# rimelabs/lambda-labs_distributed-training-guide

Hardware: AMD Instinct MI355X
Metric: tokens/sec/GPU (causal-LM pretrain) at 1/2/4/8 MI355X; FSDP peak-mem (higher is better)
Workload: dtype bf16; 1 GPU; model=meta-llama/Meta-Llama-3-8B, global_batch=16, seq_len=1024, parallelism=dp1-single

## Files before the change

csrc/kernels/flash_attn.hip:

```cpp
#include "flash_attn_plan.h"
#include "rope_common.h"

#include <ATen/hip/HIPGeneratorImpl.h>
#include <ATen/hip/PhiloxUtils.cuh>
#include <ATen/core/DistributionsHelper.h>

#include <climits>
#include <cstdlib>
#include <type_traits>

#include <cmath>

namespace dtg {

namespace fa {

typedef __attribute__((address_space(3))) i16x4 lds_i16x4;

constexpr float kLog2e = 1.4426950408889634f;
constexpr float kLn2 = 0.6931471805599453f;
constexpr float kRescaleThreshold = 8.f;

template <int W>
__device__ __forceinline__ int off(int row, int ch) {
  constexpr int NCH = W / 8;
  static_assert(NCH == 8 || NCH == 16, "head_dim 64 or 128");
  int sw;
  if constexpr (NCH == 16) sw = ((row & 3) << 2) | ((row >> 2) & 3);
  else sw = ((row & 1) << 2) | ((row >> 1) & 3);
  return row * (W * 2) + 16 * (ch ^ sw);
}

__device__ __forceinline__ i16x4 tr_read(const char* p) {
  return __builtin_amdgcn_ds_read_tr16_b64_v4i16((lds_i16x4*)(p));
}

__device__ __forceinline__ bf16x8 tr_frag_at(const char* pa, const char* pb) {
  const i16x4 a = tr_read(pa);
  const i16x4 b = tr_read(pb);
  typedef short i16x8 __attribute__((ext_vector_type(8)));
  const i16x8 ab = __builtin_shufflevector(a, b, 0, 1, 2, 3, 4, 5, 6, 7);
  return __builtin_bit_cast(bf16x8, ab);
}

template <int W>
__device__ __forceinline__ void tr_offsets(int d, int& oa, int& ob) {
  const int lane = threadIdx.x & 63;
  const int i = lane & 15, g = lane >> 4;
  const int q = i >> 2, p = i & 3;
  const int ch = ((32 * d + 16 * (g & 1)) >> 3) + (p >> 1);
  const int half = 8 * (p & 1);
  const int row = 4 * (g >> 1) + q;
  oa = off<W>(row, ch) + half;
  ob = off<W>(row + 8, ch) + half;
}

__device__ __forceinline__ f32x16 mfma(bf16x8 a, bf16x8 b, f32x16 c) {
  return __builtin_amdgcn_mfma_f32_32x32x16_bf16(a, b, c, 0, 0, 0);
}

__device__ __forceinline__ bf16x8 lds_frag(const char* p) { return *reinterpret_cast<const bf16x8*>(p); }

__device__ __forceinline__ bf16x8 pack8(const f32x16& x, int s) {
  bf16x8 r;
#pragma unroll
  for (int j = 0; j < 8; ++j) r[j] = static_cast<__bf16>(x[8 * s + j]);
  return r;
}

__device__ __forceinline__ float fexp2(float x) { return __builtin_amdgcn_exp2f(x); }

__device__ __forceinline__ float pair_max(float x) {
  const auto r = __builtin_amdgcn_permlane32_swap(__float_as_uint(x), __float_as_uint(x), false, false);
  return fmaxf(__uint_as_float(r[0]), __uint_as_float(r[1]));
}
__device__ __forceinline__ float pair_sum(float x) {
  const auto r = __builtin_amdgcn_permlane32_swap(__float_as_uint(x), __float_as_uint(x), false, false);
  return __uint_as_float(r[0]) + __uint_as_float(r[1]);
}

constexpr int kSchedMfma = 0x008, kSchedDsRead = 0x100;
template <int N, int RPM, int AHEAD>
__device__ __forceinline__ void pipeline_reads() {
  __builtin_amdgcn_sched_group_barrier(kSchedDsRead, AHEAD * RPM, 0);
#pragma unroll
  for (int i = 0; i < N - AHEAD; ++i) {
    __builtin_amdgcn_sched_group_barrier(kSchedMfma, 1, 0);
    __builtin_amdgcn_sched_group_barrier(kSchedDsRead, RPM, 0);
  }
  __builtin_amdgcn_sched_group_barrier(kSchedMfma, AHEAD, 0);
}

__device__ __forceinline__ void prio_hi() { __builtin_amdgcn_s_setprio(1); }
__device__ __forceinline__ void prio_lo() { __builtin_amdgcn_s_setprio(0); }

__device__ __forceinline__ int acc_row(int reg, int h) { return (reg & 3) + 8 * (reg >> 2) + 4 * h; }
constexpr int acc_row0(int reg) { return (reg & 3) + 8 * (reg >> 2); }

struct DropCfg {
  uint32_t k0, k1, off;
  int thr;
  float scale;
  const uint32_t* rng;
};

__device__ __forceinline__ DropCfg resolve_drop(const DropCfg& in) {
  DropCfg d = in;
  if (d.rng != nullptr) {
    d.k0 = d.rng[0];
    d.k1 = d.rng[1] ^ d.rng[3];
    d.off = d.rng[2];
  }
  return d;
}

__device__ __forceinline__ void philox4x32_10(uint32_t (&c)[4], uint32_t k0, uint32_t k1) {
#pragma unroll
  for (int r = 0; r < 10; ++r) {
    if (r) {
      k0 += 0x9E3779B9u;
      k1 += 0xBB67AE85u;
    }
    const uint32_t lo0 = 0xD2511F53u * c[0], hi0 = __umulhi(0xD2511F53u, c[0]);
    const uint32_t lo1 = 0xCD9E8D57u * c[2], hi1 = __umulhi(0xCD9E8D57u, c[2]);
    const uint32_t n0 = hi1 ^ c[1] ^ k0, n2 = hi0 ^ c[3] ^ k1;
    c[0] = n0;
    c[1] = lo1;
    c[2] = n2;
    c[3] = lo0;
  }
}

__device__ __forceinline__ void drop_row_half(const DropCfg& dc, int s0, int q, int head, int key0, int h,
                                              f32x16& x) {
#pragma unroll
  for (int g = 0; g < 4; ++g) {
    uint32_t c[4] = {(uint32_t)(key0 + 8 * g + 4 * h), (uint32_t)(s0 + (q & ~3)), (uint32_t)head, dc.off};
    philox4x32_10(c, dc.k0, dc.k1);
    const int ws = q & 3;
    const uint32_t wd = ws == 0 ? c[0] : ws == 1 ? c[1] : ws == 2 ? c[2] : c[3];
#pragma unroll
    for (int e = 0; e < 4; ++e) x[4 * g + e] = (int)((wd >> (8 * e)) & 255u) < dc.thr ? x[4 * g + e] : 0.f;
  }
}

__device__ __forceinline__ __amdgpu_buffer_rsrc_t make_rsrc(const void* p, int bytes) {
  const uint64_t a = reinterpret_cast<uint64_t>(p);
  const uint32_t lo = __builtin_amdgcn_readfirstlane(static_cast<uint32_t>(a));
  const uint32_t hi = __builtin_amdgcn_readfirstlane(static_cast<uint32_t>(a >> 32));
  const int n = __builtin_amdgcn_readfirstlane(bytes);
  return __builtin_amdgcn_make_buffer_rsrc(reinterpret_cast<void*>((static_cast<uint64_t>(hi) << 32) | lo),
                                           (short)0, n, 0x00020000);
}

template <int R, int W, int NT>
struct Stager {
  static constexpr int NCH = W / 8;
  static constexpr int PER = (R * NCH) / NT;
  static constexpr int RSTEP = NT / NCH;
  static_assert((R * NCH) % NT == 0 && NT % NCH == 0 && RSTEP % 16 == 0, "tile split");
  u16x8 regs[PER];
  __device__ __forceinline__ void load(const uint16_t* base, int64_t stride, int nvalid) {
    const int row0 = threadIdx.x / NCH, ch = threadIdx.x % NCH;
    const int bytes = nvalid > 0 ? static_cast<int>((nvalid - 1) * stride * 2 + W * 2) : 0;
    const __amdgpu_buffer_rsrc_t rs = make_rsrc(base, bytes);
    const int s2 = static_cast<int>(stride) * 2;
#pragma unroll
    for (int i = 0; i < PER; ++i) {
      const int voff = (row0 + i * RSTEP) * s2 + ch * 16;
      regs[i] = __builtin_bit_cast(u16x8, __builtin_amdgcn_raw_buffer_load_b128(rs, voff, 0, 0));
    }
  }
  __device__ __forceinline__ void store(char* tile) const {
    const int o = off<W>(threadIdx.x / NCH, threadIdx.x % NCH);
#pragma unroll
    for (int i = 0; i < PER; ++i) *reinterpret_cast<u16x8*>(tile + o + i * RSTEP * W * 2) = regs[i];
  }
};

template <int NC>
__device__ __forceinline__ void load_row_frags(const uint16_t* row, bool ok, int h, bf16x8* out) {
#pragma unroll
  for (int c = 0; c < NC; ++c) {
    const u16x8 z{0, 0, 0, 0, 0, 0, 0, 0};
    const u16x8 v = ok ? *reinterpret_cast<const u16x8*>(row + 16 * c + 8 * h) : z;
    out[c] = __builtin_bit_cast(bf16x8, v);
  }
}

__device__ __forceinline__ int grid_head(int x, int hq, int hkv) {
  const int group = hq / hkv;
  return (x % hkv) * group + x / hkv;
}

template <int ND>
__device__ __forceinline__ void store_rows_wide(const f32x16* acc, float scale, uint16_t* row, bool ok) {
  const int h = (threadIdx.x & 63) >> 5;
#pragma unroll
  for (int d = 0; d < ND; ++d) {
#pragma unroll
    for (int j = 0; j < 2; ++j) {
      uint32_t w[4];
#pragma unroll
      for (int u = 0; u < 2; ++u) {
        const int base = 4 * (2 * j + u);
        w[2 * u + 0] = (uint32_t)f2bf(acc[d][base + 0] * scale) | ((uint32_t)f2bf(acc[d][base + 1] * scale) << 16);
        w[2 * u + 1] = (uint32_t)f2bf(acc[d][base + 2] * scale) | ((uint32_t)f2bf(acc[d][base + 3] * scale) << 16);
      }
#pragma unroll
      for (int x = 0; x < 2; ++x) {
        const auto r = __builtin_amdgcn_permlane32_swap(w[x], w[2 + x], false, false);
        w[x] = r[0];
        w[2 + x] = r[1];
      }
      if (ok) *reinterpret_cast<uint4*>(row + 32 * d + 16 * j + 8 * h) = make_uint4(w[0], w[1], w[2], w[3]);
    }
  }
}

struct KeyRange {
  int start, len, off;
};
__device__ __forceinline__ KeyRange key_range(const int* kstart, const int* klen, int seq, int s0, int seqlen) {
  if (kstart == nullptr) return KeyRange{s0, seqlen, 0};
  const int n = klen[seq];
  return KeyRange{kstart[seq], n, n - seqlen};
}

struct FwdParams {
  const uint16_t *q, *k, *v;
  int64_t sq, sk, sv;
  uint16_t* o;
  float* lse;
  const int* cu;
  int64_t T;
  int hq, hkv;
  float c2;
  long long* stamps;
  const int *kstart, *klen;
  int window;
  DropCfg drop;
};

__device__ __forceinline__ void fa_stamp(long long* st, int slot, int k) {
  if (st != nullptr && threadIdx.x == 0) {
    st[slot * 6 + k] = (long long)__builtin_amdgcn_s_memrealtime();
    if (k == 0) {
      st[slot * 6 + 4] = (long long)__builtin_amdgcn_s_getreg(4 | (31 << 11));
      st[slot * 6 + 5] = (long long)__builtin_amdgcn_s_getreg(20 | (31 << 11));
    }
  }
}

template <int D, bool CAUSAL, bool WIN = false, bool DROP = false>
__global__ __launch_bounds__(256, 2) void fwd_kernel(FwdParams P) {
  [[maybe_unused]] const DropCfg dcfg = DROP ? resolve_drop(P.drop) : P.drop;
  constexpr int RB = 2 * D;
  constexpr int TILE = kFwdBK * RB;
  constexpr int NC = D / 16;
  constexpr int ND = D / 32;
  extern __shared__ __attribute__((aligned(16))) char smem[];

  fa_stamp(P.stamps, blockIdx.x + gridDim.x * (blockIdx.y + gridDim.y * blockIdx.z), 0);
  const int seq = blockIdx.y, head = grid_head(blockIdx.x, P.hq, P.hkv);
  const int s0 = P.cu[seq];
  const int seqlen = P.cu[seq + 1] - s0;
  const int qb = CAUSAL ? (gridDim.z - 1 - blockIdx.z) : blockIdx.z;
  const int q0 = qb * kFwdBQ;
  if (q0 >= seqlen) return;
  const KeyRange kr = key_range(P.kstart, P.klen, seq, s0, seqlen);
  const int klen = kr.len, koff_c = kr.off;
  const int kvh = head / (P.hq / P.hkv);
  const int lane = threadIdx.x & 63, w = __builtin_amdgcn_readfirstlane(threadIdx.x >> 6);
  const int r = lane & 31, h = lane >> 5;
  const int qrow = q0 + 32 * w + r;

  bf16x8 qf[NC];
  Stager<kFwdBQ, D, 256> sq;
  sq.load(P.q + (int64_t)(s0 + q0) * P.sq + (int64_t)head * D, P.sq, seqlen - q0);
  int koff[NC], toa[ND], tob[ND];
#pragma unroll
  for (int c = 0; c < NC; ++c) koff[c] = off<D>(r, 2 * c + h);
#pragma unroll
  for (int d = 0; d < ND; ++d) tr_offsets<D>(d, toa[d], tob[d]);

  const int kv_end = CAUSAL ? min(klen, q0 + kFwdBQ + koff_c) : klen;
  const int ntiles = (kv_end + kFwdBK - 1) / kFwdBK;
  const int win = (CAUSAL && WIN) ? P.window : 0;
  const int t_begin = win > 0 ? max(0, q0 + koff_c - win + 1) / kFwdBK : 0;
  const uint16_t* kbase = P.k + (int64_t)kr.start * P.sk + (int64_t)kvh * D;
  const uint16_t* vbase = P.v + (int64_t)kr.start * P.sv + (int64_t)kvh * D;

  f32x16 acc[ND];
#pragma unroll
  for (int i = 0; i < ND; ++i) acc[i] = f32x16{};
  float m = -INFINITY, l = 0.f;

  Stager<kFwdBK, D, 256> sk, sv;
  sk.load(kbase + (int64_t)t_begin * kFwdBK * P.sk, P.sk, klen - t_begin * kFwdBK);
  sv.load(vbase + (int64_t)t_begin * kFwdBK * P.sv, P.sv, klen - t_begin * kFwdBK);
  sq.store(smem + 2 * TILE);
  sk.store(smem);
  sv.store(smem + TILE);
  __syncthreads();
#pragma unroll
  for (int c = 0; c < NC; ++c) qf[c] = lds_frag(smem + 2 * TILE + 32 * w * RB + koff[c]);
  __syncthreads();
  fa_stamp(P.stamps, blockIdx.x + gridDim.x * (blockIdx.y + gridDim.y * blockIdx.z), 1);

  const int wave_q0 = q0 + 32 * w, wave_qmax = wave_q0 + 31;
  auto tile_step = [&](int t, auto buf) {
    constexpr int B = decltype(buf)::value;
    const int kt0 = t * kFwdBK;
    const bool more = t + 1 < ntiles;
    if (more) {
      const int nk = kt0 + kFwdBK;
      sk.load(kbase + (int64_t)nk * P.sk, P.sk, klen - nk);
      sv.load(vbase + (int64_t)nk * P.sv, P.sv, klen - nk);
    }
    const char* K = smem + B * 2 * TILE;
    const char* V = K + TILE;
    if ((!CAUSAL || kt0 <= wave_qmax + koff_c) && (win == 0 || kt0 + kFwdBK - 1 >= wave_q0 + koff_c - win + 1)) {
      f32x16 s[2];
      __builtin_amdgcn_sched_barrier(0);
      prio_hi();
#pragma unroll
      for (int kt = 0; kt < 2; ++kt) {
        bf16x8 kf[NC];
#pragma unroll
        for (int c = 0; c < NC; ++c) kf[c] = lds_frag(K + kt * 32 * RB + koff[c]);
        s[kt] = f32x16{};
#pragma unroll
        for (int c = 0; c < NC; ++c) s[kt] = mfma(kf[c], qf[c], s[kt]);
      }
      pipeline_reads<2 * NC, 1, 4>();
      __builtin_amdgcn_sched_barrier(0);
      prio_lo();
      if ((CAUSAL && kt0 + kFwdBK - 1 > wave_q0 + koff_c) || kt0 + kFwdBK > klen ||
          (win > 0 && kt0 < wave_qmax + koff_c - win + 1)) {
#pragma unroll
        for (int kt = 0; kt < 2; ++kt) {
          const int lim = (CAUSAL ? min(qrow + koff_c, klen - 1) : klen - 1) - (kt0 + 32 * kt + 4 * h);
          const int llim = win > 0 ? qrow + koff_c - win + 1 - (kt0 + 32 * kt + 4 * h) : INT_MIN;
#pragma unroll
          for (int i = 0; i < 16; ++i)
            s[kt][i] = (acc_row0(i) > lim || acc_row0(i) < llim) ? -INFINITY : s[kt][i];
        }
      }
      float mx = s[0][0];
#pragma unroll
      for (int kt = 0; kt < 2; ++kt) {
#pragma unroll
        for (int i = 0; i < 16; ++i) mx = fmaxf(mx, s[kt][i]);
      }
      mx = pair_max(mx) * P.c2;
      if (__builtin_amdgcn_ballot_w64(mx > m + kRescaleThreshold) != 0) {
        const float mn = fmaxf(m, mx);
        const float alpha = (mn == -INFINITY) ? 1.f : fexp2(m - mn);
        l *= alpha;
#pragma unroll
        for (int d = 0; d < ND; ++d) acc[d] *= alpha;
        m = mn;
      }
      const float mu = (m == -INFINITY) ? 0.f : m;
      float rs = 0.f;
#pragma unroll
      for (int kt = 0; kt < 2; ++kt) {
#pragma unroll
        for (int i = 0; i < 16; ++i) {
          const float p = fexp2(__builtin_fmaf(s[kt][i], P.c2, -mu));
          s[kt][i] = p;
          rs += p;
        }
      }
      l += rs;
      if constexpr (DROP) {
#pragma unroll
        for (int kt = 0; kt < 2; ++kt) drop_row_half(dcfg, s0, qrow, head, kt0 + 32 * kt, h, s[kt]);
      }
      bf16x8 pf[4];
#pragma unroll
      for (int j = 0; j < 4; ++j) pf[j] = pack8(s[j >> 1], j & 1);
      __builtin_amdgcn_sched_barrier(0);
      prio_hi();
#pragma unroll
      for (int j = 0; j < 4; ++j) {
        const char* vb = V + 16 * j * RB;
        bf16x8 vt[ND];
#pragma unroll
        for (int d = 0; d < ND; ++d) vt[d] = tr_frag_at(vb + toa[d], vb + tob[d]);
#pragma unroll
        for (int d = 0; d < ND; ++d) acc[d] = mfma(vt[d], pf[j], acc[d]);
      }
      pipeline_reads<4 * ND, 2, 3>();
      __builtin_amdgcn_sched_barrier(0);
      prio_lo();
    }
    if (more) {
      char* nb = smem + (1 - B) * 2 * TILE;
      sk.store(nb);
      sv.store(nb + TILE);
    }
    __syncthreads();
  };
  int t = t_begin;
  for (; t + 1 < ntiles; t += 2) {
    tile_step(t, std::integral_constant<int, 0>{});
    tile_step(t + 1, std::integral_constant<int, 1>{});
  }
  if (t < ntiles) tile_step(t, std::integral_constant<int, 0>{});
  fa_stamp(P.stamps, blockIdx.x + gridDim.x * (blockIdx.y + gridDim.y * blockIdx.z), 2);

  const float lt = pair_sum(l);
  const float inv = (lt > 0.f ? 1.f / lt : 0.f) * (DROP ? P.drop.scale : 1.f);
  uint16_t* op = P.o + ((int64_t)(s0 + min(qrow, seqlen - 1)) * P.hq + head) * D;
  store_rows_wide<ND>(acc, inv, op, qrow < seqlen);
  if (qrow < seqlen && h == 0)
    P.lse[(int64_t)head * P.T + s0 + qrow] = (lt > 0.f) ? (m + log2f(lt)) * kLn2 : -INFINITY;
  if (P.stamps != nullptr) {
    asm volatile("s_waitcnt vmcnt(0)" ::: "memory");
    __syncthreads();
    fa_stamp(P.stamps, blockIdx.x + gridDim.x * (blockIdx.y + gridDim.y * blockIdx.z), 3);
  }
}

struct BwdParams {
  const uint16_t *q, *k, *v, *dout, *o;
  int64_t sq, sk, sv;
  const float* lse;
  float* delta;
  uint16_t *dq, *dk, *dv;
  int64_t sdq, sdk, sdv;
  const int* cu;
  int64_t T;
  int hq, hkv;
  float scale, c2;
  const int *kstart, *klen;
  int window;
  float *dk_part, *dv_part;
  int nsplit;
  DropCfg drop;
  const float *rope_cos, *rope_sin;
  const int64_t* rope_pos;
};

template <int ND>
__device__ __forceinline__ void rope_inv_rows(f32x16* acc, const float* cos_t, const float* sin_t, int64_t p) {
  constexpr int HT = ND / 2;
  constexpr int HALF = 16 * ND;
  const int h = (threadIdx.x & 63) >> 5;
  const float* cp = cos_t + p * HALF;
  const float* sp = sin_t + p * HALF;
#pragma unroll
  for (int d = 0; d < HT; ++d) {
#pragma unroll
    for (int g = 0; g < 4; ++g) {
      const int i = 32 * d + 8 * g + 4 * h;
      const float4 c = *reinterpret_cast<const float4*>(cp + i);
      const float4 sn = *reinterpret_cast<const float4*>(sp + i);
      const float cc[4] = {c.x, c.y, c.z, c.w}, ss[4] = {sn.x, sn.y, sn.z, sn.w};
#pragma unroll
      for (int e = 0; e < 4; ++e) {
        const int r = 4 * g + e;
        const float x1 = acc[d][r], x2 = acc[d + HT][r];
        acc[d][r] = x1 * cc[e] + x2 * ss[e];
        acc[d + HT][r] = x2 * cc[e] - x1 * ss[e];
      }
    }
  }
}

template <int D, bool CAUSAL, int OCC, bool WIN = false, bool DROP = false>
__global__ __launch_bounds__(256, OCC) void bwd_dq_kernel(BwdParams P) {
  [[maybe_unused]] const DropCfg dcfg = DROP ? resolve_drop(P.drop) : P.drop;
  constexpr int RB = 2 * D;
  constexpr int TILE = kDqBK * RB;
  constexpr int NC = D / 16;
  constexpr int ND = D / 32;
  extern __shared__ __attribute__((aligned(16))) char smem[];

  const int seq = blockIdx.y, head = grid_head(blockIdx.x, P.hq, P.hkv);
  const int s0 = P.cu[seq];
  const int seqlen = P.cu[seq + 1] - s0;
  const int qb = CAUSAL ? (gridDim.z - 1 - blockIdx.z) : blockIdx.z;
  const int q0 = qb * kDqBQ;
  if (q0 >= seqlen) return;
  const KeyRange kr = key_range(P.kstart, P.klen, seq, s0, seqlen);
  const int klen = kr.len, koff_c = kr.off;
  const int kvh = head / (P.hq / P.hkv);
  const int lane = threadIdx.x & 63, w = __builtin_amdgcn_readfirstlane(threadIdx.x >> 6);
  const int r = lane & 31, h = lane >> 5;
  const int qrow = q0 + 32 * w + r;
  const bool qok = qrow < seqlen;
  const int64_t t_row = s0 + (qok ? qrow : seqlen - 1);

  int koff[NC], toa[ND], tob[ND];
#pragma unroll
  for (int c = 0; c < NC; ++c) koff[c] = off<D>(r, 2 * c + h);
#pragma unroll
  for (int d = 0; d < ND; ++d) tr_offsets<D>(d, toa[d], tob[d]);

  const int kv_end = CAUSAL ? min(klen, q0 + kDqBQ + koff_c) : klen;
  const int ntiles = (kv_end + kDqBK - 1) / kDqBK;
  const int win = (CAUSAL && WIN) ? P.window : 0;
  const int t_begin = win > 0 ? max(0, q0 + koff_c - win + 1) / kDqBK : 0;
  const uint16_t* kbase = P.k + (int64_t)kr.start * P.sk + (int64_t)kvh * D;
  const uint16_t* vbase = P.v + (int64_t)kr.start * P.sv + (int64_t)kvh * D;

  constexpr int QIMG = kDqBQ * RB;
  static_assert(2 * QIMG <= 4 * TILE, "Q + dO images must fit the K/V buffers");
  float* rowd = reinterpret_cast<float*>(smem + 4 * TILE);
  bf16x8 qf[NC], dof[NC];
  float delta;
  Stager<kDqBK, D, 256> sk, sv;
  {
    Stager<kDqBQ, D, 256> sq, sdo, so;
    const int64_t srow = (int64_t)(s0 + q0);
    sq.load(P.q + srow * P.sq + (int64_t)head * D, P.sq, seqlen - q0);
    sdo.load(P.dout + (srow * P.hq + head) * D, (int64_t)P.hq * D, seqlen - q0);
    so.load(P.o + (srow * P.hq + head) * D, (int64_t)P.hq * D, seqlen - q0);
    sk.load(kbase + (int64_t)t_begin * kDqBK * P.sk, P.sk, klen - t_begin * kDqBK);
    sv.load(vbase + (int64_t)t_begin * kDqBK * P.sv, P.sv, klen - t_begin * kDqBK);
    {
      constexpr int NCH = D / 8, RSTEP = 256 / NCH, PER = kDqBQ / RSTEP;
      const int row0 = threadIdx.x / NCH, ch = threadIdx.x % NCH;
#pragma unroll
      for (int i = 0; i < PER; ++i) {
        float part = 0.f;
#pragma unroll
        for (int j = 0; j < 8; ++j) part += bf2f(sdo.regs[i][j]) * bf2f(so.regs[i][j]);
#pragma unroll
        for (int x = 1; x < NCH; x <<= 1) part += __shfl_xor(part, x, 64);
        if (ch == 0) rowd[row0 + i * RSTEP] = part;
      }
    }
    sq.store(smem);
    sdo.store(smem + QIMG);
    __syncthreads();
#pragma unroll
    for (int c = 0; c < NC; ++c) {
      qf[c] = lds_frag(smem + 32 * w * RB + koff[c]);
      dof[c] = lds_frag(smem + QIMG + 32 * w * RB + koff[c]);
    }
    delta = rowd[32 * w + r];
    __syncthreads();
  }
  if (qok && h == 0) P.delta[(int64_t)head * P.T + s0 + qrow] = delta;
  const float lse2 = qok ? P.lse[(int64_t)head * P.T + s0 + qrow] * kLog2e : 0.f;

  f32x16 acc[ND];
#pragma unroll
  for (int i = 0; i < ND; ++i) acc[i] = f32x16{};

  sk.store(smem);
  sv.store(smem + TILE);
  __syncthreads();

  const int wave_q0 = q0 + 32 * w, wave_qmax = wave_q0 + 31;
  auto sd_mfma = [&](const char* K, const char* V, int kt, f32x16& s, f32x16& dp) {
    bf16x8 f[NC], g[NC];
#pragma unroll
    for (int c = 0; c < NC; ++c) f[c] = lds_frag(K + kt * 32 * RB + koff[c]);
#pragma unroll
    for (int c = 0; c < NC; ++c) s = mfma(f[c], qf[c], s);
#pragma unroll
    for (int c = 0; c < NC; ++c) g[c] = lds_frag(V + kt * 32 * RB + koff[c]);
#pragma unroll
    for (int c = 0; c < NC; ++c) dp = mfma(g[c], dof[c], dp);
  };
  auto half_masked = [&](int key0) {
    return (CAUSAL && key0 + 31 > wave_q0 + koff_c) || key0 + 32 > klen ||
           (win > 0 && key0 < wave_qmax + koff_c - win + 1);
  };
  auto softmax_ds = [&](int key0, f32x16& s, const f32x16& dp, bf16x8* dsf) {
#pragma unroll
    for (int i = 0; i < 16; ++i) s[i] = fexp2(__builtin_fmaf(s[i], P.c2, -lse2));
    if (half_masked(key0)) {
      const int lim = (CAUSAL ? min(qrow + koff_c, klen - 1) : klen - 1) - (key0 + 4 * h);
      const int llim = win > 0 ? qrow + koff_c - win + 1 - (key0 + 4 * h) : INT_MIN;
#pragma unroll
      for (int i = 0; i < 16; ++i) s[i] = (acc_row0(i) > lim || acc_row0(i) < llim) ? 0.f : s[i];
    }
    if constexpr (DROP) {
      f32x16 z = dp;
      drop_row_half(dcfg, s0, qrow, head, key0, h, z);
#pragma unroll
      for (int i = 0; i < 16; ++i) s[i] *= z[i] * dcfg.scale - delta;
    } else {
#pragma unroll
      for (int i = 0; i < 16; ++i) s[i] *= dp[i] - delta;
    }
    dsf[0] = pack8(s, 0);
    dsf[1] = pack8(s, 1);
  };
  auto dq_mfma = [&](const char* K, int kt, const bf16x8* dsf) {
#pragma unroll
    for (int st = 0; st < 2; ++st) {
      const char* kb = K + (32 * kt + 16 * st) * RB;
      bf16x8 kt_[ND];
#pragma unroll
      for (int d = 0; d < ND; ++d) kt_[d] = tr_frag_at(kb + toa[d], kb + tob[d]);
#pragma unroll
      for (int d = 0; d < ND; ++d) acc[d] = mfma(kt_[d], dsf[st], acc[d]);
    }
  };
  auto half_live = [&](int key0) {
    return !((CAUSAL && key0 > wave_qmax + koff_c) || key0 >= klen) &&
           !(win > 0 && key0 + 31 < wave_q0 + koff_c - win + 1);
  };
  auto tile_step = [&](int t, auto buf) {
    constexpr int B = decltype(buf)::value;
    const int kt0 = t * kDqBK;
    const bool more = t + 1 < ntiles;
    if (more) {
      const int nk = kt0 + kDqBK;
      sk.load(kbase + (int64_t)nk * P.sk, P.sk, klen - nk);
      sv.load(vbase + (int64_t)nk * P.sv, P.sv, klen - nk);
    }
    const char* K = smem + B * 2 * TILE;
    const char* V = K + TILE;
    const bool live0 = half_live(kt0), live1 = half_live(kt0 + 32);
    {
#pragma unroll
      for (int kt = 0; kt < 2; ++kt) {
        if (!(kt == 0 ? live0 : live1)) continue;
        f32x16 s = f32x16{}, dp = f32x16{};
        __builtin_amdgcn_sched_barrier(0);
        sd_mfma(K, V, kt, s, dp);
        pipeline_reads<2 * NC, 1, 4>();
        __builtin_amdgcn_sched_barrier(0);
        bf16x8 dsf[2];
        softmax_ds(kt0 + 32 * kt, s, dp, dsf);
        __builtin_amdgcn_sched_barrier(0);
        dq_mfma(K, kt, dsf);
        pipeline_reads<2 * ND, 2, 3>();
        __builtin_amdgcn_sched_barrier(0);
      }
    }
    if (more) {
      char* nb = smem + (1 - B) * 2 * TILE;
      sk.store(nb);
      sv.store(nb + TILE);
    }
    __syncthreads();
  };
  int t = t_begin;
  for (; t + 1 < ntiles; t += 2) {
    tile_step(t, std::integral_constant<int, 0>{});
    tile_step(t + 1, std::integral_constant<int, 1>{});
  }
  if (t < ntiles) tile_step(t, std::integral_constant<int, 0>{});

  if (P.rope_cos != nullptr) rope_inv_rows<ND>(acc, P.rope_cos, P.rope_sin, P.rope_pos[s0 + min(qrow, seqlen - 1)]);
  store_rows_wide<ND>(acc, P.scale, P.dq + (int64_t)(s0 + min(qrow, seqlen - 1)) * P.sdq + (int64_t)head * D, qok);
}

template <int D, bool CAUSAL, int PF, bool WIN = false, int QB = kKvBQ, bool DROP = false>
__global__ __launch_bounds__(256, D == 128 ? 1 : 2) void bwd_dkdv_kernel(BwdParams P) {
  [[maybe_unused]] const DropCfg dcfg = DROP ? resolve_drop(P.drop) : P.drop;
  static_assert(QB == 32 || QB == 64, "query rows per item");
  constexpr int RB = 2 * D;
  constexpr int NC = D / 16;
  constexpr int ND = D / 32;
  constexpr int SLICE = QB * RB;
  extern __shared__ __attribute__((aligned(16))) char smem[];
  char* qd = smem;
  float* rowc = reinterpret_cast<float*>(qd + 4 * SLICE);

  const int seq = blockIdx.y, kvh = blockIdx.x;
  const int s0 = P.cu[seq];
  const int seqlen = P.cu[seq + 1] - s0;
  const KeyRange kr = key_range(P.kstart, P.klen, seq, s0, seqlen);
  const int klen = kr.len, koff_c = kr.off;
  const int nsplit = P.nsplit > 1 ? P.nsplit : 1;
  const int split = blockIdx.z % nsplit;
  const int kb = (blockIdx.z / nsplit) * kKvBK;
  if (kb >= klen) return;
  const int group = P.hq / P.hkv;
  const int lane = threadIdx.x & 63, w = __builtin_amdgcn_readfirstlane(threadIdx.x >> 6);
  const int r = lane & 31, h = lane >> 5;
  const int wkey0 = kb + 32 * w;
  const int key = wkey0 + r;

  bf16x8 kf[NC], vf[NC];
  {
    const bool ok = key < klen;
    const int64_t t = kr.start + (ok ? key : klen - 1);
    load_row_frags<NC>(P.k + t * P.sk + (int64_t)kvh * D, ok, h, kf);
    load_row_frags<NC>(P.v + t * P.sv + (int64_t)kvh * D, ok, h, vf);
  }
  int roff[NC], toa[ND], tob[ND];
#pragma unroll
  for (int c = 0; c < NC; ++c) roff[c] = off<D>(r, 2 * c + h);
#pragma unroll
  for (int d = 0; d < ND; ++d) tr_offsets<D>(d, toa[d], tob[d]);

  f32x16 dk[ND], dv[ND];
#pragma unroll
  for (int i = 0; i < ND; ++i) {
    dk[i] = f32x16{};
    dv[i] = f32x16{};
  }

  const int first_slice = CAUSAL ? (max(0, kb - koff_c) / QB) : 0;
  const int win = (CAUSAL && WIN) ? P.window : 0;
  const int end_slice = win > 0 ? min((seqlen + QB - 1) / QB, (kb + kKvBK - 1 - koff_c + win - 1) / QB + 1)
                                : (seqlen + QB - 1) / QB;
  const int per_head = max(0, end_slice - first_slice);
  const int nitems = per_head * group;
  const float inv_scale = 1.f / P.scale;

  struct Item {
    Stager<QB, D, 256> q, dout;
    uint32_t lse, dlt;
  };
  Item ia, ib;
  auto load_item = [&](Item& X, int it) {
    const int hqi = kvh * group + it / per_head;
    const int qs = (first_slice + it % per_head) * QB;
    const int nv = seqlen - qs;
    X.q.load(P.q + (int64_t)(s0 + qs) * P.sq + (int64_t)hqi * D, P.sq, nv);
    X.dout.load(P.dout + ((int64_t)(s0 + qs) * P.hq + hqi) * D, (int64_t)P.hq * D, nv);
    const int nrow = min(QB, seqlen - qs);
    const int64_t ro = (int64_t)hqi * P.T + s0 + qs;
    const int vo = (threadIdx.x & (QB - 1)) * 4;
    X.lse = __builtin_amdgcn_raw_buffer_load_b32(make_rsrc(P.lse + ro, nrow * 4), vo, 0, (int)(1u << 31));
    X.dlt = __builtin_amdgcn_raw_buffer_load_b32(make_rsrc(P.delta + ro, nrow * 4), vo, 0, (int)(1u << 31));
  };
  auto store_item = [&](const Item& X, int buf) {
    X.q.store(qd + buf * 2 * SLICE);
    X.dout.store(qd + buf * 2 * SLICE + SLICE);
    if (threadIdx.x < 2 * QB) {
      const float l = __builtin_bit_cast(float, X.lse), dl = __builtin_bit_cast(float, X.dlt);
      rowc[buf * 2 * QB + threadIdx.x] = (threadIdx.x & QB) ? -dl : -l * inv_scale;
    }
  };
  auto drop_cols = [&](int qsu, int hqi, f32x16& s, f32x16& dp, const float* cnd) {
#pragma unroll
    for (int g = 0; g < 4; ++g) {
      uint32_t c[4] = {(uint32_t)(key & ~3), (uint32_t)(s0 + qsu + 8 * g + 4 * h), (uint32_t)hqi, dcfg.off};
      philox4x32_10(c, dcfg.k0, dcfg.k1);
      const int sh = 8 * (key & 3);
#pragma unroll
      for (int e = 0; e < 4; ++e) {
        const int i = 4 * g + e;
        const bool keep = (int)((c[e] >> sh) & 255u) < dcfg.thr;
        const float p = s[i];
        dp[i] = p * ((keep ? dp[i] * dcfg.scale : 0.f) + cnd[acc_row(i, h)]);
        s[i] = keep ? p * dcfg.scale : 0.f;
      }
    }
  };
  auto compute = [&](int it, int buf) {
    const int qs = (first_slice + it % per_head) * QB;
    {
      const char* Ql = qd + buf * 2 * SLICE;
      const char* dOl = Ql + SLICE;
      const float* c0 = rowc + buf * 2 * QB;
      f32x16 s, dp;
#pragma unroll
      for (int i = 0; i < 16; ++i) {
        s[i] = c0[acc_row(i, h)];
        dp[i] = DROP ? 0.f : c0[QB + acc_row(i, h)];
      }
      __builtin_amdgcn_sched_barrier(0);
      {
        bf16x8 f[NC], g[NC];
#pragma unroll
        for (int c = 0; c < NC; ++c) f[c] = lds_frag(Ql + roff[c]);
#pragma unroll
        for (int c = 0; c < NC; ++c) s = mfma(f[c], kf[c], s);
#pragma unroll
        for (int c = 0; c < NC; ++c) g[c] = lds_frag(dOl + roff[c]);
#pragma unroll
        for (int c = 0; c < NC; ++c) dp = mfma(g[c], vf[c], dp);
      }
      pipeline_reads<2 * NC, 1, 4>();
      __builtin_amdgcn_sched_barrier(0);
#pragma unroll
      for (int i = 0; i < 16; ++i) s[i] = fexp2(s[i] * P.c2);
      if ((CAUSAL && wkey0 + 31 > qs + koff_c) || (win > 0 && qs + kKvBQ - 1 > wkey0 - koff_c + win - 1)) {
        const int lim = key - koff_c - qs - 4 * h;
        const int ulim = win > 0 ? key - koff_c + win - 1 - qs - 4 * h : INT_MAX;
#pragma unroll
        for (int i = 0; i < 16; ++i) s[i] = (acc_row0(i) < lim || acc_row0(i) > ulim) ? 0.f : s[i];
      }
      if constexpr (DROP) {
        drop_cols(qs, kvh * group + it / per_head, s, dp, c0 + QB);
      } else {
#pragma unroll
        for (int i = 0; i < 16; ++i) dp[i] *= s[i];
      }
      const bf16x8 pf[2] = {pack8(s, 0), pack8(s, 1)};
      const bf16x8 dsf[2] = {pack8(dp, 0), pack8(dp, 1)};
      __builtin_amdgcn_sched_barrier(0);
#pragma unroll
      for (int st = 0; st < 2; ++st) {
        const char* ob = dOl + 16 * st * RB;
        const char* qb = Ql + 16 * st * RB;
        bf16x8 a[ND], b[ND];
#pragma unroll
        for (int d = 0; d < ND; ++d) a[d] = tr_frag_at(ob + toa[d], ob + tob[d]);
#pragma unroll
        for (int d = 0; d < ND; ++d) dv[d] = mfma(a[d], pf[st], dv[d]);
#pragma unroll
        for (int d = 0; d < ND; ++d) b[d] = tr_frag_at(qb + toa[d], qb + tob[d]);
#pragma unroll
        for (int d = 0; d < ND; ++d) dk[d] = mfma(b[d], dsf[st], dk[d]);
      }
      pipeline_reads<4 * ND, 2, 3>();
      __builtin_amdgcn_sched_barrier(0);
    }
  };

  auto sd_mfma = [&](const char* Ql, const char* dOl, f32x16& s, f32x16& dp) {
    bf16x8 f[NC], g[NC];
#pragma unroll
    for (int c = 0; c < NC; ++c) f[c] = lds_frag(Ql + roff[c]);
#pragma unroll
    for (int c = 0; c < NC; ++c) s = mfma(f[c], kf[c], s);
#pragma unroll
    for (int c = 0; c < NC; ++c) g[c] = lds_frag(dOl + roff[c]);
#pragma unroll
    for (int c = 0; c < NC; ++c) dp = mfma(g[c], vf[c], dp);
  };
  auto softmax_half = [&](int qsu, int hqi, const float* cnd, f32x16& s, f32x16& dp, bf16x8 (&pf)[2],
                          bf16x8 (&dsf)[2]) {
#pragma unroll
    for (int i = 0; i < 16; ++i) s[i] = fexp2(s[i] * P.c2);
    if constexpr (CAUSAL) {
      const int lim = key - koff_c - qsu - 4 * h;
#pragma unroll
      for (int i = 0; i < 16; ++i) s[i] = acc_row0(i) < lim ? 0.f : s[i];
    }
    if constexpr (DROP) {
      drop_cols(qsu, hqi, s, dp, cnd);
    } else {
#pragma unroll
      for (int i = 0; i < 16; ++i) dp[i] *= s[i];
    }
    pf[0] = pack8(s, 0);
    pf[1] = pack8(s, 1);
    dsf[0] = pack8(dp, 0);
    dsf[1] = pack8(dp, 1);
  };
  auto kv_mfma = [&](const char* Ql, const char* dOl, const bf16x8 (&pf)[2], const bf16x8 (&dsf)[2]) {
#pragma unroll
    for (int st = 0; st < 2; ++st) {
      const char* ob = dOl + 16 * st * RB;
      const char* qb = Ql + 16 * st * RB;
      bf16x8 a[ND], b[ND];
#pragma unroll
      for (int d = 0; d < ND; ++d) a[d] = tr_frag_at(ob + toa[d], ob + tob[d]);
#pragma unroll
      for (int d = 0; d < ND; ++d) dv[d] = mfma(a[d], pf[st], dv[d]);
#pragma unroll
      for (int d = 0; d < ND; ++d) b[d] = tr_frag_at(qb + toa[d], qb + tob[d]);
#pragma unroll
      for (int d = 0; d < ND; ++d) dk[d] = mfma(b[d], dsf[st], dk[d]);
    }
  };
  auto compute64 = [&](int it, int buf) {
    const int qs = (first_slice + it % per_head) * QB;
    const char* Ql = qd + buf * 2 * SLICE;
    const char* dOl = Ql + SLICE;
    const float* c0 = rowc + buf * 2 * QB;
    f32x16 s0, dp0, s1, dp1;
#pragma unroll
    for (int i = 0; i < 16; ++i) {
      s0[i] = c0[acc_row(i, h)];
      dp0[i] = DROP ? 0.f : c0[QB + acc_row(i, h)];
      s1[i] = c0[32 + acc_row(i, h)];
      dp1[i] = DROP ? 0.f : c0[QB + 32 + acc_row(i, h)];
    }
    __builtin_amdgcn_sched_barrier(0);
    sd_mfma(Ql, dOl, s0, dp0);
    pipeline_reads<2 * NC, 1, 4>();
    __builtin_amdgcn_sched_barrier(0);
    bf16x8 pf0[2], dsf0[2], pf1[2], dsf1[2];
    sd_mfma(Ql + 32 * RB, dOl + 32 * RB, s1, dp1);
    const int hqi = kvh * group + it / per_head;
    softmax_half(qs, hqi, c0 + QB, s0, dp0, pf0, dsf0);
    __builtin_amdgcn_sched_barrier(0);
    kv_mfma(Ql, dOl, pf0, dsf0);
    softmax_half(qs + 32, hqi, c0 + QB + 32, s1, dp1, pf1, dsf1);
    __builtin_amdgcn_sched_barrier(0);
    kv_mfma(Ql + 32 * RB, dOl + 32 * RB, pf1, dsf1);
    pipeline_reads<4 * ND, 2, 3>();
    __builtin_amdgcn_sched_barrier(0);
  };

  auto run_item = [&](int it, int buf) {
    if constexpr (QB == 64) compute64(it, buf);
    else compute(it, buf);
  };

  __builtin_amdgcn_s_waitcnt(0x0f70);

  static_assert(PF == 1 || QB == 32, "two-item prefetch only with 32-row items");
  if constexpr (PF == 2) {
    load_item(ia, 0);
    load_item(ib, min(1, nitems - 1));
    store_item(ia, 0);
    __syncthreads();
    auto step = [&](int it, auto par) {
      constexpr int S = decltype(par)::value;
      Item& cur = S == 0 ? ia : ib;
      Item& nxt = S == 0 ? ib : ia;
      load_item(cur, min(it + 2, nitems - 1));
      compute(it, S);
      if (it + 1 < nitems) store_item(nxt, S ^ 1);
      __syncthreads();
    };
    int it = 0;
    for (; it + 1 < nitems; it += 2) {
      step(it, std::integral_constant<int, 0>{});
      step(it + 1, std::integral_constant<int, 1>{});
    }
    if (it < nitems) step(it, std::integral_constant<int, 0>{});
  } else {
    const int it0 = (int)((int64_t)split * nitems / nsplit), it1 = (int)((int64_t)(split + 1) * nitems / nsplit);
    if (it0 < it1) {
      load_item(ia, it0);
      store_item(ia, it0 & 1);
    }
    __syncthreads();
    for (int it = it0; it < it1; ++it) {
      const int buf = it & 1;
      const bool more = it + 1 < it1;
      if (more) load_item(ia, it + 1);
      run_item(it, buf);
      if (more) store_item(ia, buf ^ 1);
      __syncthreads();
    }
  }

  const int64_t krow = kr.start + min(key, klen - 1);
  if (nsplit > 1) {
    if (key < klen) {
      const int64_t o = (((int64_t)split * P.T + krow) * P.hkv + kvh) * D + 4 * h;
      float* pk = P.dk_part + o;
      float* pv = P.dv_part + o;
#pragma unroll
      for (int d = 0; d < ND; ++d) {
#pragma unroll
        for (int g = 0; g < 4; ++g) {
          *reinterpret_cast<f32x4*>(pk + 32 * d + 8 * g) = f32x4{dk[d][4 * g], dk[d][4 * g + 1], dk[d][4 * g + 2], dk[d][4 * g + 3]};
          *reinterpret_cast<f32x4*>(pv + 32 * d + 8 * g) = f32x4{dv[d][4 * g], dv[d][4 * g + 1], dv[d][4 * g + 2], dv[d][4 * g + 3]};
        }
      }
    }
    return;
  }
  if (P.rope_cos != nullptr) rope_inv_rows<ND>(dk, P.rope_cos, P.rope_sin, P.rope_pos[krow]);
  store_rows_wide<ND>(dk, P.scale, P.dk + krow * P.sdk + (int64_t)kvh * D, key < klen);
  store_rows_wide<ND>(dv, 1.f, P.dv + krow * P.sdv + (int64_t)kvh * D, key < klen);
}

template <int D>
__global__ __launch_bounds__(256) void bwd_kv_combine_kernel(const float* __restrict__ dk_part,
                                                             const float* __restrict__ dv_part, int nsplit,
                                                             int64_t T, int hkv, float scale, uint16_t* __restrict__ dk,
                                                             int64_t sdk, uint16_t* __restrict__ dv, int64_t sdv) {
  constexpr int V = D / 8;
  const int64_t i = (int64_t)blockIdx.x * blockDim.x + threadIdx.x;
  const int64_t rows = T * hkv;
  if (i >= rows * V) return;
  const int64_t row = i / V;
  const int c = (int)(i % V) * 8;
  const int64_t t = row / hkv;
  const int hh = (int)(row % hkv);
  float a[8], b[8];
#pragma unroll
  for (int j = 0; j < 8; ++j) a[j] = b[j] = 0.f;
  for (int sp = 0; sp < nsplit; ++sp) {
    const int64_t o = ((int64_t)sp * rows + row) * D + c;
    const f32x4 k0 = *reinterpret_cast<const f32x4*>(dk_part + o), k1 = *reinterpret_cast<const f32x4*>(dk_part + o + 4);
    const f32x4 v0 = *reinterpret_cast<const f32x4*>(dv_part + o), v1 = *reinterpret_cast<const f32x4*>(dv_part + o + 4);
#pragma unroll
    for (int j = 0; j < 4; ++j) {
      a[j] += k0[j];
      a[4 + j] += k1[j];
      b[j] += v0[j];
      b[4 + j] += v1[j];
    }
  }
#pragma unroll
  for (int j = 0; j < 8; ++j) a[j] *= scale;
  store8(dk + t * sdk + (int64_t)hh * D + c, a);
  store8(dv + t * sdv + (int64_t)hh * D + c, b);
}

}

static int env_int(const char* name, int dflt) {
  const char* e = std::getenv(name);
  return (e != nullptr && e[0] != 0) ? std::atoi(e) : dflt;
}
static fa::Tuning& tuning() {
  static fa::Tuning t{std::max(0, env_int("DTG_FA_KV_SPLIT", 0)), env_int("DTG_FA_KV_QB", 64) == 32 ? 32 : 64,
                      env_int("DTG_FA_OCC", 1) == 2 ? 2 : 1, env_int("DTG_FA_KV_PF", 1) == 2 ? 2 : 1};
  return t;
}
[[maybe_unused]] static const bool kTuningLoaded = (tuning(), true);

std::vector<int64_t> flash_attn_tuning(const at::Tensor& , int64_t kv_split, int64_t kv_qb) {
  fa::Tuning& t = tuning();
  std::vector<int64_t> old{t.kv_split, t.kv_qb};
  if (kv_split >= 0) t.kv_split = (int)kv_split;
  DTG_CHECK(kv_qb < 0 || kv_qb == 32 || kv_qb == 64, "flash_attn_tuning: kv_qb must be 32 or 64");
  if (kv_qb >= 0) t.kv_qb = (int)kv_qb;
  return old;
}

template <typename Params>
static void launch(void (*kernel)(Params), const fa::Plan& pl, size_t lds, hipStream_t st, const Params& P) {
  TORCH_INTERNAL_ASSERT(lds == pl.lds, "flash_attn: launch plan and instantiation disagree");
  if (lds > 65536)
    C10_HIP_CHECK(hipFuncSetAttribute((const void*)kernel, hipFuncAttributeMaxDynamicSharedMemorySize, (int)lds));
  hipLaunchKernelGGL(kernel, dim3(pl.grid.x, pl.grid.y, pl.grid.z), dim3(256), lds, st, P);
  DTG_LAUNCH_CHECK();
}
template <int D, bool C, bool WIN = false, bool DROP = false>
static void fwd_launch(const fa::FwdPlan& pl, const fa::FwdParams& P, hipStream_t st) {
  launch(fa::fwd_kernel<D, C, WIN, DROP>, pl, fa::fwd_lds_bytes(D), st, P);
}
template <int D, bool C, int OCC, bool WIN = false, bool DROP = false>
static void dq_launch(const fa::DqPlan& pl, const fa::BwdParams& P, hipStream_t st) {
  TORCH_INTERNAL_ASSERT(pl.occ == OCC);
  launch(fa::bwd_dq_kernel<D, C, OCC, WIN, DROP>, pl, fa::dq_lds_bytes(D), st, P);
}
template <int D, bool C, int PF, bool WIN = false, int QB = fa::kKvBQ, bool DROP = false>
static void kv_launch(const fa::KvPlan& pl, const fa::BwdParams& P, hipStream_t st) {
  TORCH_INTERNAL_ASSERT(pl.pf == PF && pl.qb == QB);
  launch(fa::bwd_dkdv_kernel<D, C, PF, WIN, QB, DROP>, pl, fa::kv_lds_bytes(D, QB), st, P);
}

template <int D>
static void launch_fwd(const fa::FwdPlan& pl, const fa::FwdParams& P, hipStream_t st) {
  if (pl.var == fa::Variant::DROP)
    pl.causal ? fwd_launch<D, true, false, true>(pl, P, st) : fwd_launch<D, false, false, true>(pl, P, st);
  else if (pl.var == fa::Variant::WIN) fwd_launch<D, true, true>(pl, P, st);
  else pl.causal ? fwd_launch<D, true>(pl, P, st) : fwd_launch<D, false>(pl, P, st);
}
template <int D>
static void launch_bwd_dq(const fa::DqPlan& pl, const fa::BwdParams& P, hipStream_t st) {
  constexpr int kOcc = D == 64 ? 2 : 1;
  if (pl.var == fa::Variant::DROP)
    pl.causal ? dq_launch<D, true, kOcc, false, true>(pl, P, st) : dq_launch<D, false, kOcc, false, true>(pl, P, st);
  else if (pl.var == fa::Variant::WIN) dq_launch<D, true, kOcc, true>(pl, P, st);
  else if (pl.occ == 2) pl.causal ? dq_launch<D, true, 2>(pl, P, st) : dq_launch<D, false, 2>(pl, P, st);
  else pl.causal ? dq_launch<D, true, kOcc>(pl, P, st) : dq_launch<D, false, kOcc>(pl, P, st);
}
template <int D>
static void launch_bwd_dkdv(const fa::KvPlan& pl, fa::BwdParams P, hipStream_t st, const at::TensorOptions& opts) {
  at::Tensor dk_part, dv_part;
  P.nsplit = pl.nsplit;
  if (pl.nsplit > 1) {
    dk_part = at::empty({pl.nsplit, P.T, P.hkv, D}, opts.dtype(at::kFloat));
    dv_part = at::empty({pl.nsplit, P.T, P.hkv, D}, opts.dtype(at::kFloat));
    P.dk_part = dk_part.data_ptr<float>();
    P.dv_part = dv_part.data_ptr<float>();
  }
  if (pl.var == fa::Variant::DROP)
    pl.causal ? kv_launch<D, true, 1, false, 64, true>(pl, P, st) : kv_launch<D, false, 1, false, 64, true>(pl, P, st);
  else if (pl.var == fa::Variant::WIN) kv_launch<D, true, 1, true>(pl, P, st);
  else if (pl.pf == 2) pl.causal ? kv_launch<D, true, 2>(pl, P, st) : kv_launch<D, false, 2>(pl, P, st);
  else if (pl.qb == 64)
    pl.causal ? kv_launch<D, true, 1, false, 64>(pl, P, st) : kv_launch<D, false, 1, false, 64>(pl, P, st);
  else pl.causal ? kv_launch<D, true, 1>(pl, P, st) : kv_launch<D, false, 1>(pl, P, st);
  if (pl.nsplit > 1) {
    const int64_t nv = P.T * P.hkv * (D / 8);
    fa::bwd_kv_combine_kernel<D><<<(nv + 255) / 256, 256, 0, st>>>(P.dk_part, P.dv_part, pl.nsplit, P.T, P.hkv, P.scale,
                                                                  P.dk, P.sdk, P.dv, P.sdv);
    DTG_LAUNCH_CHECK();
    if (P.rope_cos != nullptr) rope_rows_launch(P.dk, P.sdk, P.hkv, D, P.rope_cos, P.rope_sin, P.rope_pos, P.T, true, st);
  }
}

struct AttnOpts {
  const at::Tensor *k_start = nullptr, *k_len = nullptr;
  int64_t max_seqlen_k = -1;
  int64_t window = 0;
  const fa::DropCfg* drop = nullptr;
  const at::Tensor *rope_cos = nullptr, *rope_sin = nullptr, *rope_pos = nullptr;
  at::Tensor* stamps = nullptr;
};

static void check_qkv(const at::Tensor& t, const char* name, int64_t heads, int64_t d) {
  DTG_CHECK_CUDA_BF16(t);
  DTG_CHECK(t.dim() == 3 && t.size(1) == heads && t.size(2) == d && t.stride(2) == 1 &&
                t.stride(1) == d && t.stride(0) % 8 == 0,
            name, " must be [T, H, D] with contiguous heads and 16-B aligned token stride");
}

static void check_inputs(const at::Tensor& q, const at::Tensor& k, const at::Tensor& v, const at::Tensor& cu_seqlens) {
  const int64_t D = q.size(2);
  check_qkv(q, "q", q.size(1), D);
  check_qkv(k, "k", k.size(1), D);
  check_qkv(v, "v", k.size(1), D);
  DTG_CHECK(D == 64 || D == 128, "flash_attn: head_dim must be 64 or 128");
  DTG_CHECK(cu_seqlens.scalar_type() == at::kInt && cu_seqlens.is_cuda() && cu_seqlens.is_contiguous(),
            "flash_attn: cu_seqlens must be int32 on the GPU");
}
static fa::Call checked_call(const at::Tensor& q, int64_t hkv, int nseq, int64_t max_seqlen, bool causal,
                             const AttnOpts& op, const int** ks, const int** kl) {
  DTG_CHECK(nseq <= 65535, "flash_attn: at most 65535 sequences per call");
  if (op.k_start != nullptr) {
    for (const at::Tensor* t : {op.k_start, op.k_len})
      DTG_CHECK(t->scalar_type() == at::kInt && t->is_cuda() && t->is_contiguous() && t->numel() == nseq,
                "flash_attn: k_start / k_len must be int32 [nseq] on the GPU");
    *ks = op.k_start->data_ptr<int>();
    *kl = op.k_len->data_ptr<int>();
  }
  DTG_CHECK(op.window >= 0 && op.window < (1ll << 30), "flash_attn: window must be >= 0 (0 = full causal)");
  return fa::Call{(int)q.size(2), causal, op.window, op.drop != nullptr, op.k_start != nullptr, op.rope_cos != nullptr,
                  (int)q.size(1), (int)hkv, nseq, max_seqlen, op.max_seqlen_k < 0 ? max_seqlen : op.max_seqlen_k};
}

static std::tuple<at::Tensor, at::Tensor> flash_attn_fwd_impl(
    const at::Tensor& q, const at::Tensor& k, const at::Tensor& v, const at::Tensor& cu_seqlens, int64_t max_seqlen,
    double scale, bool causal, const AttnOpts& op) {
  const int64_t T = q.size(0), hq = q.size(1), D = q.size(2), hkv = k.size(1);
  check_inputs(q, k, v, cu_seqlens);
  DTG_CHECK(v.size(0) == k.size(0) && (op.k_start != nullptr || k.size(0) == T), "flash_attn: q/k/v token counts differ");
  DTG_CHECK(hq % hkv == 0, "flash_attn: Hq must be a multiple of Hkv");
  const c10::DeviceGuard g(q.device());
  auto o = at::empty({T, hq, D}, q.options());
  auto lse = at::empty({hq, T}, q.options().dtype(at::kFloat));
  const int nseq = cu_seqlens.numel() - 1;
  if (T == 0 || nseq <= 0 || max_seqlen <= 0) return {o, lse};
  fa::FwdParams P{bf16_ptr(q), bf16_ptr(k), bf16_ptr(v), q.stride(0), k.stride(0), v.stride(0),
                  bf16_mut(o), lse.data_ptr<float>(), cu_seqlens.data_ptr<int>(), T, (int)hq, (int)hkv,
                  (float)(scale * fa::kLog2e), nullptr, nullptr, nullptr, 0};
  const fa::Call c = checked_call(q, hkv, nseq, max_seqlen, causal, op, &P.kstart, &P.klen);
  P.window = fa::window_eff(c);
  const fa::FwdPlan pl = fa::plan_fwd(c);
  if (op.stamps != nullptr) {
    *op.stamps = at::zeros({(int64_t)pl.grid.x * pl.grid.y * pl.grid.z, 6}, q.options().dtype(at::kLong));
    P.stamps = reinterpret_cast<long long*>(op.stamps->data_ptr<int64_t>());
  }
  if (const char* why = fa::conflict(c)) DTG_CHECK(false, why);
  if (op.drop != nullptr) P.drop = *op.drop;
  D == 128 ? launch_fwd<128>(pl, P, stream()) : launch_fwd<64>(pl, P, stream());
  return {o, lse};
}

std::tuple<at::Tensor, at::Tensor> flash_attn_fwd(const at::Tensor& q, const at::Tensor& k, const at::Tensor& v,
                                                  const at::Tensor& cu_seqlens, int64_t max_seqlen, double scale,
                                                  bool causal, int64_t window) {
  return flash_attn_fwd_impl(q, k, v, cu_seqlens, max_seqlen, scale, causal, {.window = window});
}

std::tuple<at::Tensor, at::Tensor, at::Tensor> flash_attn_fwd_stamped(
    const at::Tensor& q, const at::Tensor& k, const at::Tensor& v, const at::Tensor& cu_seqlens, int64_t max_seqlen,
    double scale, bool causal) {
  at::Tensor st;
  auto [o, lse] = flash_attn_fwd_impl(q, k, v, cu_seqlens, max_seqlen, scale, causal, {.stamps = &st});
  return {o, lse, st};
}

static void flash_attn_bwd_impl(const at::Tensor& dout_, const at::Tensor& q, const at::Tensor& k, const at::Tensor& v,
                                const at::Tensor& o, const at::Tensor& lse, const at::Tensor& cu_seqlens,
                                int64_t max_seqlen, double scale, bool causal, const at::Tensor& dq,
                                const at::Tensor& dk, const at::Tensor& dv, const AttnOpts& op) {
  auto dout = dout_.contiguous();
  const int64_t T = q.size(0), hq = q.size(1), D = q.size(2), hkv = k.size(1);
  check_inputs(q, k, v, cu_seqlens);
  check_qkv(dq, "dq", hq, D);
  check_qkv(dk, "dk", hkv, D);
  check_qkv(dv, "dv", hkv, D);
  DTG_CHECK_CUDA_BF16(dout);
  DTG_CHECK(o.is_contiguous() && dout.sizes() == o.sizes() && o.size(0) == T, "flash_attn_bwd: o/dout");
  DTG_CHECK(lse.scalar_type() == at::kFloat && lse.is_contiguous() && lse.size(0) == hq && lse.size(1) == T,
            "flash_attn_bwd: lse must be f32 [Hq, T]");
  const c10::DeviceGuard g(q.device());
  const int nseq = cu_seqlens.numel() - 1;
  if (T == 0 || nseq <= 0 || max_seqlen <= 0) {
    for (const at::Tensor& t : {dq, dk, dv}) t.zero_();
    return;
  }
  auto delta = at::empty({hq, T}, q.options().dtype(at::kFloat));
  fa::BwdParams P{bf16_ptr(q), bf16_ptr(k), bf16_ptr(v), bf16_ptr(dout), bf16_ptr(o), q.stride(0), k.stride(0),
                  v.stride(0), lse.data_ptr<float>(), delta.data_ptr<float>(), bf16_mut(dq), bf16_mut(dk),
                  bf16_mut(dv), dq.stride(0), dk.stride(0), dv.stride(0), cu_seqlens.data_ptr<int>(), T, (int)hq,
                  (int)hkv, (float)scale, (float)(scale * fa::kLog2e), nullptr, nullptr, 0};
  const fa::Call c = checked_call(q, hkv, nseq, max_seqlen, causal, op, &P.kstart, &P.klen);
  P.window = fa::window_eff(c);
  if (op.rope_cos != nullptr) {
    P.rope_cos = op.rope_cos->data_ptr<float>();
    P.rope_sin = op.rope_sin->data_ptr<float>();
    P.rope_pos = op.rope_pos->data_ptr<int64_t>();
  }
  if (const char* why = fa::conflict(c)) DTG_CHECK(false, why);
  if (op.drop != nullptr) P.drop = *op.drop;
  const fa::DqPlan dqp = fa::plan_dq(c, tuning());
  const fa::KvPlan kvp = fa::plan_kv(c, tuning());
  D == 128 ? launch_bwd_dq<128>(dqp, P, stream()) : launch_bwd_dq<64>(dqp, P, stream());
  D == 128 ? launch_bwd_dkdv<128>(kvp, P, stream(), q.options()) : launch_bwd_dkdv<64>(kvp, P, stream(), q.options());
}

static std::tuple<at::Tensor, at::Tensor, at::Tensor> flash_attn_bwd_alloc(
    const at::Tensor& dout, const at::Tensor& q, const at::Tensor& k, const at::Tensor& v, const at::Tensor& o,
    const at::Tensor& lse, const at::Tensor& cu_seqlens, int64_t max_seqlen, double scale, bool causal,
    const AttnOpts& op) {
  auto dq = at::empty(q.sizes(), q.options());
  auto dk = op.k_start != nullptr ? at::zeros(k.sizes(), k.options()) : at::empty(k.sizes(), k.options());
  auto dv = op.k_start != nullptr ? at::zeros(v.sizes(), v.options()) : at::empty(v.sizes(), v.options());
  flash_attn_bwd_impl(dout, q, k, v, o, lse, cu_seqlens, max_seqlen, scale, causal, dq, dk, dv, op);
  return {dq, dk, dv};
}

static at::Tensor flash_attn_bwd_fused(const char* name, const at::Tensor& dout, const at::Tensor& qkv, int64_t nq,
                                       int64_t nkv, int64_t D, const at::Tensor& o, const at::Tensor& lse,
                                       const at::Tensor& cu_seqlens, int64_t max_seqlen, double scale, bool causal,
                                       const AttnOpts& op) {
  rope::check_qkv(qkv, nq + 2 * nkv, D, name);
  const int64_t T = qkv.size(0);
  DTG_CHECK(qkv.size(1) == (nq + 2 * nkv) * D, name, ": qkv must be [T, (nq + 2 nkv) * D]");
  if (op.rope_cos != nullptr) {
    rope::check_tables(*op.rope_cos, *op.rope_sin, D, name);
    rope::check_pos(*op.rope_pos, T, name);
  }
  auto dqkv = at::empty({T, (nq + 2 * nkv) * D}, qkv.options());
  auto view3 = [&](const at::Tensor& t, int64_t h0, int64_t nh) {
    return t.as_strided({T, nh, D}, {t.stride(0), D, 1}, t.storage_offset() + h0 * D);
  };
  flash_attn_bwd_impl(dout, view3(qkv, 0, nq), view3(qkv, nq, nkv), view3(qkv, nq + nkv, nkv), o, lse, cu_seqlens,
                      max_seqlen, scale, causal, view3(dqkv, 0, nq), view3(dqkv, nq, nkv), view3(dqkv, nq + nkv, nkv), op);
  return dqkv;
}

std::tuple<at::Tensor, at::Tensor, at::Tensor> flash_attn_bwd(
    const at::Tensor& dout, const at::Tensor& q, const at::Tensor& k, const at::Tensor& v, const at::Tensor& o,
    const at::Tensor& lse, const at::Tensor& cu_seqlens, int64_t max_seqlen, double scale, bool causal, int64_t window) {
  return flash_attn_bwd_alloc(dout, q, k, v, o, lse, cu_seqlens, max_seqlen, scale, causal, {.window = window});
}

at::Tensor flash_attn_bwd_qkv(const at::Tensor& dout, const at::Tensor& qkv, int64_t nq, int64_t nkv, int64_t head_dim,
                              const at::Tensor& o, const at::Tensor& lse, const at::Tensor& cu_seqlens,
                              int64_t max_seqlen, double scale, bool causal, int64_t window) {
  return flash_attn_bwd_fused("flash_attn_bwd_qkv", dout, qkv, nq, nkv, head_dim, o, lse, cu_seqlens, max_seqlen, scale,
                              causal, {.window = window});
}

at::Tensor flash_attn_bwd_qkv_rope(const at::Tensor& dout, const at::Tensor& qkv, int64_t nq, int64_t nkv, int64_t head_dim,
                                   const at::Tensor& o, const at::Tensor& lse, const at::Tensor& cu_seqlens,
                                   int64_t max_seqlen, double scale, bool causal, const at::Tensor& cos_t,
                                   const at::Tensor& sin_t, const at::Tensor& pos, int64_t window) {
  return flash_attn_bwd_fused("flash_attn_bwd_qkv_rope", dout, qkv, nq, nkv, head_dim, o, lse, cu_seqlens, max_seqlen,
                              scale, causal, {.window = window, .rope_cos = &cos_t, .rope_sin = &sin_t, .rope_pos = &pos});
}

std::tuple<at::Tensor, at::Tensor> flash_attn_varlen_fwd(
    const at::Tensor& q, const at::Tensor& k, const at::Tensor& v, const at::Tensor& cu_seqlens_q,
    const at::Tensor& k_start, const at::Tensor& k_len, int64_t max_seqlen_q,
    int64_t , double scale, bool causal) {
  return flash_attn_fwd_impl(q, k, v, cu_seqlens_q, max_seqlen_q, scale, causal, {.k_start = &k_start, .k_len = &k_len});
}

std::tuple<at::Tensor, at::Tensor, at::Tensor> flash_attn_varlen_bwd(
    const at::Tensor& dout, const at::Tensor& q, const at::Tensor& k, const at::Tensor& v, const at::Tensor& o,
    const at::Tensor& lse, const at::Tensor& cu_seqlens_q, const at::Tensor& k_start, const at::Tensor& k_len,
    int64_t max_seqlen_q, int64_t max_seqlen_k, double scale, bool causal) {
  return flash_attn_bwd_alloc(dout, q, k, v, o, lse, cu_seqlens_q, max_seqlen_q, scale, causal,
                              {.k_start = &k_start, .k_len = &k_len, .max_seqlen_k = max_seqlen_k});
}

static fa::DropCfg make_drop_dev(double p, const at::Tensor& rng, const at::Tensor& like) {
  DTG_CHECK(p >= 0.0 && p < 1.0, "flash_attn dropout: p must be in [0, 1)");
  DTG_CHECK(rng.is_cuda() && rng.scalar_type() == at::kLong && rng.numel() == 2 && rng.is_contiguous() &&
                rng.device() == like.device(),
            "flash_attn dropout: rng must be a contiguous int64 [2] tensor {seed, offset} on the inputs' device");
  fa::DropCfg d{};
  d.thr = std::max(1, std::min(256, (int)std::lround((1.0 - p) * 256.0)));
  d.scale = 256.f / (float)d.thr;
  d.rng = reinterpret_cast<const uint32_t*>(rng.data_ptr<int64_t>());
  return d;
}

std::tuple<at::Tensor, at::Tensor> flash_attn_fwd_drop(const at::Tensor& q, const at::Tensor& k, const at::Tensor& v,
                                                       const at::Tensor& cu_seqlens, int64_t max_seqlen, double scale,
                                                       bool causal, double p, const at::Tensor& rng) {
  const fa::DropCfg d = make_drop_dev(p, rng, q);
  return flash_attn_fwd_impl(q, k, v, cu_seqlens, max_seqlen, scale, causal, {.drop = &d});
}

std::tuple<at::Tensor, at::Tensor, at::Tensor> flash_attn_bwd_drop(
    const at::Tensor& dout, const at::Tensor& q, const at::Tensor& k, const at::Tensor& v, const at::Tensor& o,
    const at::Tensor& lse, const at::Tensor& cu_seqlens, int64_t max_seqlen, double scale, bool causal, double p,
    const at::Tensor& rng) {
  const fa::DropCfg d = make_drop_dev(p, rng, q);
  return flash_attn_bwd_alloc(dout, q, k, v, o, lse, cu_seqlens, max_seqlen, scale, causal, {.drop = &d});
}

at::Tensor flash_attn_bwd_qkv_drop(const at::Tensor& dout, const at::Tensor& qkv, int64_t nq, int64_t nkv, int64_t head_dim,
                                   const at::Tensor& o, const at::Tensor& lse, const at::Tensor& cu_seqlens,
                                   int64_t max_seqlen, double scale, bool causal, double p, const at::Tensor& rng) {
  const fa::DropCfg d = make_drop_dev(p, rng, qkv);
  return flash_attn_bwd_fused("flash_attn_bwd_qkv_drop", dout, qkv, nq, nkv, head_dim, o, lse, cu_seqlens, max_seqlen,
                              scale, causal, {.drop = &d});
}

__global__ void philox_rng_kernel(at::PhiloxCudaState st, int64_t* out) {
  if (threadIdx.x == 0) {
    const auto so = at::cuda::philox::unpack(st);
    out[0] = static_cast<int64_t>(std::get<0>(so));
    out[1] = static_cast<int64_t>(std::get<1>(so));
  }
}

at::Tensor philox_rng(const at::Tensor& like, int64_t increment) {
  DTG_CHECK(like.is_cuda(), "philox_rng: needs a GPU tensor");
  const c10::DeviceGuard g(like.device());
  auto gen = at::get_generator_or_default<at::CUDAGeneratorImpl>(
      std::nullopt, at::cuda::detail::getDefaultCUDAGenerator(like.device().index()));
  at::PhiloxCudaState st;
  {
    std::lock_guard<std::mutex> lock(gen->mutex_);
    st = gen->philox_cuda_state(static_cast<uint64_t>(std::max<int64_t>(4, increment)));
  }
  auto out = at::empty({2}, like.options().dtype(at::kLong));
  philox_rng_kernel<<<1, 64, 0, stream()>>>(st, out.data_ptr<int64_t>());
  DTG_LAUNCH_CHECK();
  return out;
}

TORCH_LIBRARY_IMPL(dtg, CUDA, m) {
  m.impl("flash_attn_fwd_drop", &flash_attn_fwd_drop);
  m.impl("flash_attn_bwd_drop", &flash_attn_bwd_drop);
  m.impl("flash_attn_bwd_qkv_drop", &flash_attn_bwd_qkv_drop);
  m.impl("philox_rng", &philox_rng);
  m.impl("flash_attn_varlen_fwd", &flash_attn_varlen_fwd);
  m.impl("flash_attn_varlen_bwd", &flash_attn_varlen_bwd);
  m.impl("flash_attn_fwd", &flash_attn_fwd);
  m.impl("flash_attn_fwd_stamped", &flash_attn_fwd_stamped);
  m.impl("flash_attn_bwd", &flash_attn_bwd);
  m.impl("flash_attn_bwd_qkv", &flash_attn_bwd_qkv);
  m.impl("flash_attn_bwd_qkv_rope", &flash_attn_bwd_qkv_rope);
  m.impl("flash_attn_tuning", &flash_attn_tuning);
}

}
```

csrc/kernels/flash_attn_plan.h:

```cpp
#pragma once

#include <algorithm>
#include <cstddef>
#include <cstdint>

namespace dtg {
namespace fa {

constexpr int kFwdBQ = 128;
constexpr int kFwdBK = 64;
constexpr int kDqBQ = 128;
constexpr int kDqBK = 64;
constexpr int kKvBK = 128;
constexpr int kKvBQ = 32;

constexpr size_t fwd_lds_bytes(int D) { return 4 * (size_t)kFwdBK * D * 2; }
constexpr size_t dq_lds_bytes(int D) { return 4 * (size_t)kDqBK * D * 2 + kDqBQ * 4; }
constexpr size_t kv_lds_bytes(int D, int qb) { return 4 * (size_t)qb * D * 2 + 2 * 2 * qb * 4; }

struct Tuning {
  int kv_split, kv_qb, dq_occ, kv_pf;
};
struct Call {
  int D;
  bool causal;
  int64_t window;
  bool drop, key_ranges, rope;
  int hq, hkv, nseq;
  int64_t max_seqlen, max_seqlen_k;
};
enum class Variant { PLAIN, WIN, DROP };
struct Grid {
  unsigned x, y, z;
};
struct Plan {
  Variant var;
  bool causal;
  Grid grid;
  size_t lds;
};
using FwdPlan = Plan;
struct DqPlan : Plan {
  int occ;
};
struct KvPlan : Plan {
  int pf, qb, nsplit;
};

inline int window_eff(const Call& c) { return c.causal ? (int)c.window : 0; }
inline Variant variant(const Call& c) {
  return c.drop ? Variant::DROP : window_eff(c) > 0 ? Variant::WIN : Variant::PLAIN;
}
inline const char* conflict(const Call& c) {
  if (c.rope && (c.key_ranges || c.drop)) return "flash_attn rope: self-attention without dropout only";
  if (c.drop && (window_eff(c) != 0 || c.key_ranges)) return "flash_attn dropout: no sliding window / key ranges";
  return nullptr;
}
inline unsigned nblocks(int64_t n, int per) { return (unsigned)((n + per - 1) / per); }

inline FwdPlan plan_fwd(const Call& c) {
  return {variant(c), c.causal, {(unsigned)c.hq, (unsigned)c.nseq, nblocks(c.max_seqlen, kFwdBQ)}, fwd_lds_bytes(c.D)};
}
inline DqPlan plan_dq(const Call& c, const Tuning& t) {
  const Variant var = variant(c);
  const int occ = c.D == 64 || (var == Variant::PLAIN && t.dq_occ == 2) ? 2 : 1;
  return {{var, c.causal, {(unsigned)c.hq, (unsigned)c.nseq, nblocks(c.max_seqlen, kDqBQ)}, dq_lds_bytes(c.D)}, occ};
}

inline KvPlan plan_kv(const Call& c, const Tuning& t) {
  const Variant var = variant(c);
  const int pf = var == Variant::PLAIN ? t.kv_pf : 1;
  const int qb = c.drop || (t.kv_qb != 32 && window_eff(c) == 0 && t.kv_pf == 1) ? 64 : 32;
  const unsigned nkb = nblocks(c.max_seqlen_k, kKvBK);
  const int64_t wgs = (int64_t)c.hkv * c.nseq * nkb;
  int nsplit = 1;
  if (t.kv_split > 0) nsplit = std::min(8, t.kv_split);
  else if (wgs > 0 && wgs < 512) nsplit = (int)std::min<int64_t>(4, (512 + wgs - 1) / wgs);
  if (c.key_ranges || window_eff(c) != 0 || (c.drop ? 1 : t.kv_pf) != 1) nsplit = 1;
  return {{var, c.causal, {(unsigned)c.hkv, (unsigned)c.nseq, nkb * nsplit}, kv_lds_bytes(c.D, qb)}, pf, qb, nsplit};
}

}
}
```

lambda-labs_distributed-training-guide_amd/models/llama.py:

```python
from __future__ import annotations

import dataclasses
import weakref
from typing import Optional

import torch
import torch.distributed as dist
import torch.nn as nn

from .. import ops
from ..parallel import async_tp, tp_comm
from .config import LlamaConfig


@dataclasses.dataclass
class CausalLMOutput:
    loss: Optional[torch.Tensor] = None
    logits: Optional[torch.Tensor] = None


class Weight(nn.Module):

    _dtg_param_holder = True

    def __init__(self, *shape, device=None, dtype=torch.bfloat16):
        super().__init__()
        self.weight = nn.Parameter(torch.empty(*shape, device=device, dtype=dtype))


class TPInfo:
    def __init__(self, group=None):
        self.group = group
        self.size = dist.get_world_size(group) if group is not None else 1
        self.rank = dist.get_rank(group) if group is not None else 0
        self.overlap_chunks = async_tp.DEFAULT_CHUNKS
        self.sp_regather = False

    @property
    def enabled(self):
        return self.size > 1


class RunCtx:

    __slots__ = ("cos", "sin", "pos", "cu_seqlens", "max_seqlen", "cp_group", "rows", "sp_group", "cp_ranges")

    def __init__(self, cos, sin, pos, cu_seqlens, max_seqlen, cp_group=None, rows=0, sp_group=None, cp_ranges=None):
        self.cos, self.sin, self.pos, self.cu_seqlens, self.max_seqlen = cos, sin, pos, cu_seqlens, max_seqlen
        self.cp_group, self.rows, self.sp_group = cp_group, rows, sp_group
        self.cp_ranges = cp_ranges


class LlamaAttention(nn.Module):
    def __init__(self, cfg: LlamaConfig, tp: TPInfo, device=None, dtype=torch.bfloat16):
        super().__init__()
        assert cfg.num_attention_heads % tp.size == 0 and cfg.num_key_value_heads % tp.size == 0, \
            "tensor-parallel degree must divide the number of query and key/value heads"
        self.nq = cfg.num_attention_heads // tp.size
        self.nkv = cfg.num_key_value_heads // tp.size
        self.d = cfg.head_dim
        h = cfg.hidden_size
        self.qkv_proj = Weight((self.nq + 2 * self.nkv) * self.d, h, device=device, dtype=dtype)
        if cfg.attention_bias:
            self.qkv_proj.bias = nn.Parameter(torch.empty((self.nq + 2 * self.nkv) * self.d, 1, device=device,
                                                          dtype=dtype))
        self.o_proj = Weight(h, self.nq * self.d, device=device, dtype=dtype)
        self.window = int(cfg.sliding_window or 0)
        self.qk_norm = bool(cfg.qk_norm)
        if self.qk_norm:
            self.eps = cfg.rms_norm_eps
            self.q_norm = Weight(self.d, device=device, dtype=dtype)
            self.k_norm = Weight(self.d, device=device, dtype=dtype)
            for p in (self.q_norm.weight, self.k_norm.weight):
                p._dtg_sequence_parallel = tp.enabled

    def _forward_qk_norm(self, qkv, rc: RunCtx):
        wq, wk, d = self.q_norm.weight, self.k_norm.weight, self.d
        if rc.cp_group is not None:
            from ..parallel.context_parallel import cp_attention

            T = qkv.shape[0]
            qkv = ops.qk_norm_rope(qkv, wq, wk, self.eps, self.nq, self.nkv, d, rc.cos, rc.sin, rc.pos)
            q = qkv[:, :self.nq * d].reshape(T, self.nq, d)
            k = qkv[:, self.nq * d:(self.nq + self.nkv) * d].reshape(T, self.nkv, d)
            v = qkv[:, (self.nq + self.nkv) * d:].reshape(T, self.nkv, d)
            return cp_attention(q, k, v, rc.cp_group, rc.rows, ranges=rc.cp_ranges).reshape(T, self.nq * d)
        if rc.sp_group is not None:
            from ..parallel.ulysses import ulysses_attention

            qkv = ops.qk_norm_rope(qkv, wq, wk, self.eps, self.nq, self.nkv, d)
            return ulysses_attention(qkv, self.nq, self.nkv, d, rc.sp_group, rc.rows, rc.cu_seqlens,
                                     rc.max_seqlen, rc.cos, rc.sin, rc.pos)
        qkv = ops.qk_norm_rope(qkv, wq, wk, self.eps, self.nq, self.nkv, d, rc.cos, rc.sin, rc.pos,
                               grad_inplace=True)
        return ops.attention(qkv, self.nq, self.nkv, d, rc.cu_seqlens, rc.max_seqlen, window=self.window)

    def forward(self, x, rc: RunCtx, out=None):
        b = getattr(self.qkv_proj, "bias", None)
        qkv = ops.linear(x, self.qkv_proj.weight, None if b is None else b.view(-1))
        if self.qk_norm:
            return ops.linear(self._forward_qk_norm(qkv, rc), self.o_proj.weight, out=out)
        if rc.cp_group is not None:
            from ..parallel.context_parallel import cp_attention

            T, d = qkv.shape[0], self.d
            qkv = ops.rope(qkv, rc.cos, rc.sin, rc.pos, self.nq + self.nkv, d)
            q = qkv[:, :self.nq * d].reshape(T, self.nq, d)
            k = qkv[:, self.nq * d:(self.nq + self.nkv) * d].reshape(T, self.nkv, d)
            v = qkv[:, (self.nq + self.nkv) * d:].reshape(T, self.nkv, d)
            o = cp_attention(q, k, v, rc.cp_group, rc.rows, ranges=rc.cp_ranges).reshape(T, self.nq * d)
        elif rc.sp_group is not None:
            from ..parallel.ulysses import ulysses_attention

            o = ulysses_attention(qkv, self.nq, self.nkv, self.d, rc.sp_group, rc.rows, rc.cu_seqlens,
                                  rc.max_seqlen, rc.cos, rc.sin, rc.pos)
        else:
            o = ops.attention(qkv, self.nq, self.nkv, self.d, rc.cu_seqlens, rc.max_seqlen, rc.cos, rc.sin, rc.pos,
                              window=self.window)
        return ops.linear(o, self.o_proj.weight, out=out)


class LlamaMLP(nn.Module):
    def __init__(self, cfg: LlamaConfig, tp: TPInfo, device=None, dtype=torch.bfloat16):
        super().__init__()
        assert cfg.intermediate_size % tp.size == 0
        self.inter = cfg.intermediate_size // tp.size
        self.gate_up_proj = Weight(2 * self.inter, cfg.hidden_size, device=device, dtype=dtype)
        self.down_proj = Weight(cfg.hidden_size, self.inter, device=device, dtype=dtype)

    def forward(self, x, out=None):
        return ops.swiglu_mlp(x, self.gate_up_proj.weight, self.down_proj.weight, out=out)


class LlamaDecoderLayer(nn.Module):
    def __init__(self, cfg: LlamaConfig, tp: TPInfo, device=None, dtype=torch.bfloat16):
        super().__init__()
        self.eps = cfg.rms_norm_eps
        self.tp = tp
        self.input_layernorm = Weight(cfg.hidden_size, device=device, dtype=dtype)
        self.post_attention_layernorm = Weight(cfg.hidden_size, device=device, dtype=dtype)
        self.self_attn = LlamaAttention(cfg, tp, device, dtype)
        self.mlp = LlamaMLP(cfg, tp, device, dtype)
        for p in (self.input_layernorm.weight, self.post_attention_layernorm.weight):
            p._dtg_sequence_parallel = tp.enabled

    def forward(self, x, res, rc: RunCtx):
        g = self.tp.group if self.tp.enabled else None
        if res is None:
            n, res = ops.rms_norm(x, self.input_layernorm.weight, self.eps), x
        else:
            n, res = ops.add_rms_norm(x, res, self.input_layernorm.weight, self.eps)
        ka, km = self._overlap_chunks(n.shape[0], rc) if g is not None else (1, 1)
        regather = g is not None and self._regather()
        if ka > 1:
            a = async_tp.sp_region(n, lambda xg, j, out=None: self.self_attn(xg, _chunk_ctx(rc, xg.shape[0]), out=out), g, ka,
                                   tuple(p for p in self.self_attn.parameters()), regather=regather)
        elif g is not None:
            a = self._sp_block(n, lambda xg: self.self_attn(xg, rc), g, regather)
        else:
            a = self.self_attn(n, rc)
        n2, res = ops.add_rms_norm(a, res, self.post_attention_layernorm.weight, self.eps)
        if km > 1:
            m = async_tp.sp_region(n2, lambda xg, j, out=None: self.mlp(xg, out=out), g, km,
                                   (self.mlp.gate_up_proj.weight, self.mlp.down_proj.weight), regather=regather)
        elif g is not None:
            m = self._sp_block(n2, self.mlp, g, regather)
        else:
            m = self.mlp(n2)
        return m, res

    def _regather(self):
        return self.tp.sp_regather and torch.is_grad_enabled() and not getattr(self, "_dtg_checkpointed", False)

    @staticmethod
    def _sp_block(n, fn, g, regather):
        full = tp_comm.gather_seq(n, g)
        if not regather:
            return tp_comm.scatter_seq(fn(full), g)
        with async_tp.regathered(full, n, g) as h:
            y = fn(full)
        if y.requires_grad:
            ref = weakref.ref(h)
            y.register_hook(lambda grad: None if ref() is None else ref().prefetch())
        return tp_comm.scatter_seq(y, g)

    def _overlap_chunks(self, rows_local, rc: RunCtx):
        k = self.tp.overlap_chunks
        if k <= 1 or getattr(self, "_dtg_checkpointed", False) or not torch.is_grad_enabled():
            return 1, 1
        km = async_tp.region_chunks(rows_local, k)
        dense = (rc.cp_group is None and rc.sp_group is None and rc.cu_seqlens is not None
                 and rc.cu_seqlens.numel() == rc.rows + 1 and rc.max_seqlen > 0)
        ka = async_tp.region_chunks(rows_local, k, rc.max_seqlen) if dense else 1
        return ka, km


def tp_seed_offset(tp_rank: int) -> int:
    return 1_000_003 * int(tp_rank)


def _chunk_ctx(rc: RunCtx, rows: int) -> RunCtx:
    S = rc.max_seqlen
    b = rows // S
    return RunCtx(rc.cos, rc.sin, rc.pos[:rows], rc.cu_seqlens[:b + 1], S, None, b, None)


class _VocabParallelEmbedding(torch.autograd.Function):
    @staticmethod
    def forward(ctx, ids, w, vstart):
        from ..utils.comm import _FAKE

        local = ids - vstart
        if _FAKE:
            local = torch.remainder(local, w.shape[0])
        mask = (local < 0) | (local >= w.shape[0])
        local = local.masked_fill(mask, 0)
        out = torch.nn.functional.embedding(local, w)
        out.masked_fill_(mask[:, None], 0)
        ctx.save_for_backward(local, mask)
        ctx.w = w
        return out

    @staticmethod
    def backward(ctx, dy):
        local, mask = ctx.saved_tensors
        from ..ops.grad_routing import route_embedding_grad

        return None, route_embedding_grad(ctx.w, local.masked_fill(mask, -1), dy.contiguous(), ctx.w.shape[0]), None


class LlamaForCausalLM(nn.Module):
    def __init__(self, cfg: LlamaConfig, tp_group=None, device=None, dtype=torch.bfloat16, cp_group=None,
                 sp_group=None):
        super().__init__()
        self.config = cfg
        self.tp = TPInfo(tp_group)
        self.cp_group = cp_group
        self.sp_group = sp_group
        assert sum(g is not None for g in (cp_group, tp_group, sp_group)) <= 1, \
            "context, Ulysses and tensor parallelism are not combined"
        tp = self.tp
        assert cfg.vocab_size % tp.size == 0 or not tp.enabled, "vocab must divide by the TP degree"
        self.vocab_local = cfg.vocab_size // tp.size
        self.vocab_start = tp.rank * self.vocab_local
        self.embed_tokens = Weight(self.vocab_local, cfg.hidden_size, device=device, dtype=dtype)
        self.layers = nn.ModuleList([LlamaDecoderLayer(cfg, tp, device, dtype) for _ in range(cfg.num_hidden_layers)])
        self.norm = Weight(cfg.hidden_size, device=device, dtype=dtype)
        self.norm.weight._dtg_sequence_parallel = tp.enabled
        self.lm_head = None if cfg.tie_word_embeddings else Weight(self.vocab_local, cfg.hidden_size, device=device, dtype=dtype)
        if cfg.tie_word_embeddings:
            self.embed_tokens.weight._dtg_uses = 2
        self._rope = None
        self._dense_cache = {}

    @torch.no_grad()
    def init_param(self, name: str, t: torch.Tensor):
        if name.endswith("layernorm.weight") or name == "norm.weight" or name.endswith(("q_norm.weight", "k_norm.weight")):
            t.fill_(1.0)
        elif name.endswith(".bias"):
            t.zero_()
        else:
            t.normal_(0.0, self.config.initializer_range)

    @torch.no_grad()
    def init_weights(self):
        off = tp_seed_offset(self.tp.rank) if self.tp.enabled else 0
        for name, p in self.named_parameters():
            if p.device.type == "meta":
                continue
            if off:
                state = torch.random.get_rng_state()
                torch.manual_seed((int(torch.randint(0, 2**62, (1,)).item()) + off) % 2**63)
                self.init_param(name, p)
                torch.random.set_rng_state(state)
                torch.randint(0, 2**62, (1,))
            else:
                self.init_param(name, p)

    def lm_head_weight(self):
        return self.embed_tokens.weight if self.lm_head is None else self.lm_head.weight

    def _rope_tables(self, need: int, device):
        if self._rope is None or self._rope[0].shape[0] < need or self._rope[0].device != device:
            n = max(need, 4096)
            n = (n + 4095) // 4096 * 4096
            c = self.config
            self._rope = ops.rope_tables(c.head_dim, c.rope_theta, n, c.rope_scaling, device=device)
        return self._rope

    def _dense_meta(self, B, S, device):
        key = (B, S, str(device))
        v = self._dense_cache.get(key)
        if v is None:
            pos = torch.arange(S, device=device, dtype=torch.long).repeat(B)
            cu = torch.arange(0, (B + 1) * S, S, device=device, dtype=torch.int32)
            v = (pos, cu)
            self._dense_cache = {key: v}
        return v

    def forward(self, input_ids, labels=None, position_ids=None, cu_seqlens=None, max_seqlen=None,
                num_valid=None, return_logits=False, attention_mask=None):
        rc = self.run_context(input_ids, position_ids, cu_seqlens, max_seqlen)
        x, res = self.embed(input_ids), None
        for layer in self.layers:
            x, res = layer(x, res, rc)
        return self.head(x, res, labels, num_valid, return_logits, input_ids.shape[0])

    def run_context(self, input_ids, position_ids=None, cu_seqlens=None, max_seqlen=None) -> RunCtx:
        B, S = input_ids.shape
        T = B * S
        dev = input_ids.device
        sw = self.config.sliding_window
        if sw is not None and (self.cp_group is not None or self.sp_group is not None) and S > sw:
            raise ValueError(f"{self.config.model_type}: context / Ulysses parallelism with rows longer than the "
                             f"sliding window ({sw}) is not supported; the single-rank and TP paths are")
        sp = self.sp_group is not None
        if sp:
            from ..parallel.ulysses import sp_world

            n = sp_world(self.sp_group)
            if position_ids is not None:
                from ..utils import comm

                loc = position_ids.to(device=dev, dtype=torch.long).contiguous()
                position_ids = comm.all_gather_dim0(loc.t().contiguous(), self.sp_group).t()
                cu_seqlens = None
            S = S * n
            T = B * S
        cp_ranges = None
        if self.cp_group is not None:
            if cu_seqlens is not None:
                from ..parallel.context_parallel import cp_ranges as _cp_ranges
                from ..utils import comm

                n = comm.world(self.cp_group)
                cp_ranges = _cp_ranges(comm.rank(self.cp_group), n, B, S // 2, dev, cu_seqlens=cu_seqlens)
            pos, cu, max_seqlen = position_ids.reshape(-1).to(torch.long), None, 0
        elif position_ids is None:
            pos, cu = self._dense_meta(B, S, dev)
            max_seqlen = S
        else:
            pos = position_ids.reshape(-1).to(torch.long)
            if cu_seqlens is None:
                starts = torch.nonzero(pos == 0).flatten()
                row_starts = torch.arange(0, T, S, device=dev)
                starts = torch.unique(torch.cat([starts, row_starts]))
                cu = torch.cat([starts, torch.tensor([T], device=dev)]).to(torch.int32)
                max_seqlen = int((cu[1:] - cu[:-1]).max().item())
            else:
                cu = cu_seqlens.to(device=dev, dtype=torch.int32)
                if max_seqlen is None:
                    max_seqlen = int((cu[1:] - cu[:-1]).max().item())
        cp = self.cp_group is not None
        if cp:
            assert position_ids is not None, "context parallel needs the global position_ids (cp_batch)"
            cos, sin = self._rope_tables(int(position_ids.max()) + 1, dev)
        else:
            cos, sin = self._rope_tables(S, dev)
        return RunCtx(cos, sin, pos, cu, int(max_seqlen), self.cp_group if cp else None, B,
                      self.sp_group if sp else None, cp_ranges)

    def embed(self, input_ids):
        ids = input_ids.reshape(-1)
        tp = self.tp
        if tp.enabled:
            x = _VocabParallelEmbedding.apply(ids, self.embed_tokens.weight, self.vocab_start)
            return tp_comm.scatter_seq(x, tp.group)
        return ops.embedding(ids, self.embed_tokens.weight)

    def head(self, x, res, labels=None, num_valid=None, return_logits=False, batch_rows=1):
        tp = self.tp
        h, _ = ops.add_rms_norm(x, res, self.norm.weight, self.config.rms_norm_eps)
        if tp.enabled:
            h = tp_comm.gather_seq(h, tp.group)
        out = CausalLMOutput()
        w = self.lm_head_weight()
        if labels is not None:
            cp, sp = self.cp_group is not None, self.sp_group is not None
            if cp or sp:
                shifted = labels.reshape(-1)
            else:
                shifted = torch.full_like(labels, -100)
                shifted[:, :-1] = labels[:, 1:]
                shifted = shifted.reshape(-1)
            if num_valid is None:
                num_valid = int((shifted != -100).sum().item())
                if cp or sp:
                    import torch.distributed as dist

                    t = torch.tensor([num_valid], device=h.device)
                    dist.all_reduce(t, group=self.cp_group if cp else self.sp_group)
                    num_valid = int(t.item())
            if tp.enabled:
                out.loss = ops.vocab_parallel_fused_linear_cross_entropy(
                    h, w, shifted, self.vocab_start, tp.group, num_valid=num_valid)
            else:
                out.loss = ops.fused_linear_cross_entropy(h, w, shifted, num_valid=num_valid)
        if return_logits or labels is None:
            logits = ops.linear(h, w)
            if tp.enabled:
                logits = tp_comm.gather_seq(logits.t().contiguous(), tp.group).t()
            out.logits = logits.view(batch_rows, -1, logits.shape[-1])
        return out


def count_valid_labels(labels: torch.Tensor, ignore_index: int = -100) -> int:
    return int((labels[:, 1:] != ignore_index).sum())
```

lambda-labs_distributed-training-guide_amd/ops/__init__.py:

```python
from . import _schema
from . import _cpu
from . import _native

_native.load()
if not _native.LOADED:
    _schema.LIB.impl("adamw_cpu_", lambda p, g, m, v, lr, b1, b2, eps, wd, step, gs: _cpu.adamw_(
        p, None, g, m, v, lr, b1, b2, eps, wd, step, gs), "CPU")

from .functional import (
    add_rms_norm,
    attention,
    check_sample_scalar,
    decode_attention,
    dropout_add_layer_norm,
    embedding,
    fused_linear_cross_entropy,
    gelu_mlp,
    kv_cache_append,
    layer_norm,
    linear,
    qk_norm_rope,
    rms_norm,
    rope,
    rope_tables,
    sample_logits,
    skinny_linear,
    swiglu,
    swiglu_mlp,
    vocab_parallel_fused_linear_cross_entropy,
)
from .grad_routing import route_param_grad
from .adamw import adamw_step

import contextlib as _contextlib

import torch as _torch


@_contextlib.contextmanager
def fa_tuning(device="cuda", kv_split: int = -1, kv_qb: int = -1):
    like = _torch.empty(0, device=device)
    old = _torch.ops.dtg.flash_attn_tuning(like, kv_split, kv_qb)
    try:
        yield
    finally:
        _torch.ops.dtg.flash_attn_tuning(like, old[0], old[1])

__all__ = [
    "add_rms_norm", "attention", "rope", "embedding", "fused_linear_cross_entropy", "linear", "rms_norm",
    "rope_tables", "swiglu", "swiglu_mlp", "vocab_parallel_fused_linear_cross_entropy", "route_param_grad", "adamw_step",
    "fa_tuning", "layer_norm", "dropout_add_layer_norm", "gelu_mlp", "qk_norm_rope", "kv_cache_append", "decode_attention",
    "sample_logits", "skinny_linear",
]
```

lambda-labs_distributed-training-guide_amd/ops/_cpu.py:

```python
import math

import torch
import torch.nn.functional as F

from ._schema import LIB

_LOG2E = 1.4426950408889634


def rmsnorm_fwd(x, w, eps):
    xf = x.float()
    rstd = torch.rsqrt(xf.pow(2).mean(-1) + eps)
    n = (xf * rstd[:, None]).to(x.dtype)
    y = (w.float() * n.float()).to(x.dtype)
    return y, rstd


def add_rmsnorm_fwd(x, res, w, eps):
    h = (x.float() + res.float()).to(x.dtype)
    y, rstd = rmsnorm_fwd(h, w, eps)
    return y, h, rstd


def rmsnorm_bwd(dy, x, w, rstd, dres):
    xf, dyf, wf = x.float(), dy.float(), w.float()
    n = xf * rstd[:, None]
    g = dyf * wf
    dot = (g * n).mean(-1, keepdim=True)
    dx = rstd[:, None] * (g - n * dot)
    if dres is not None:
        dx = dx + dres.float()
    dw = (dyf * n.to(x.dtype).float()).sum(0)
    return dx.to(x.dtype), dw.to(w.dtype)


def rope_(qkv, cos, sin, pos, nheads, head_dim, inverse):
    T = qkv.shape[0]
    half = head_dim // 2
    view = qkv[:, : nheads * head_dim].reshape(T, nheads, head_dim)
    x1 = view[..., :half].float()
    x2 = view[..., half:].float()
    c = cos[pos][:, None, :]
    s = sin[pos][:, None, :]
    if inverse:
        s = -s
    o1 = x1 * c - x2 * s
    o2 = x2 * c + x1 * s
    qkv[:, : nheads * head_dim] = torch.cat([o1, o2], dim=-1).to(qkv.dtype).reshape(T, nheads * head_dim)


def _qk_weights(wq, wk, nq, nkv):
    return torch.cat([wq.float()[None].expand(nq, -1), wk.float()[None].expand(nkv, -1)], 0)


def _qk_rotate(y, cos, sin, pos, inverse):
    if cos.numel() == 0:
        return y
    half = y.shape[-1] // 2
    c = cos[pos][:, None, :]
    s = sin[pos][:, None, :]
    if inverse:
        s = -s
    y1, y2 = y[..., :half], y[..., half:]
    return torch.cat([y1 * c - y2 * s, y2 * c + y1 * s], -1)


def qk_norm_rope_fwd_(qkv, wq, wk, cos, sin, pos, nq, nkv, head_dim, eps):
    T, nh, d = qkv.shape[0], nq + nkv, head_dim
    xqk = qkv[:, : nh * d].clone()
    x = xqk.float().reshape(T, nh, d)
    rstd = torch.rsqrt(x.pow(2).mean(-1) + eps)
    y = _qk_weights(wq, wk, nq, nkv) * (x * rstd[..., None])
    qkv[:, : nh * d] = _qk_rotate(y, cos, sin, pos, False).reshape(T, nh * d).to(qkv.dtype)
    return xqk, rstd


def qk_norm_rope_bwd_(dqkv, xqk, rstd, wq, wk, cos, sin, pos, nq, nkv, head_dim):
    T, nh, d = dqkv.shape[0], nq + nkv, head_dim
    dy = _qk_rotate(dqkv[:, : nh * d].float().reshape(T, nh, d), cos, sin, pos, True)
    xh = xqk.float().reshape(T, nh, d) * rstd.reshape(T, nh, 1)
    g = _qk_weights(wq, wk, nq, nkv) * dy
    dx = rstd.reshape(T, nh, 1) * (g - xh * (g * xh).mean(-1, keepdim=True))
    dw = dy * xh
    dqkv[:, : nh * d] = dx.reshape(T, nh * d).to(dqkv.dtype)
    return dw[:, :nq].sum((0, 1)).to(wq.dtype), dw[:, nq:].sum((0, 1)).to(wk.dtype)


def kv_cache_append_(qkv, k_cache, v_cache, cos, sin, pos, rows, nq, nkv, head_dim):
    T, d = qkv.shape[0], head_dim
    if not (k_cache.dim() == 4 and k_cache.shape == v_cache.shape and k_cache.shape[1] == nkv and k_cache.shape[3] == d):
        raise RuntimeError("dtg: kv_cache_append_: caches must be contiguous bf16 [rows_max, nkv, S_max, head_dim]")
    if not (qkv.dim() == 2 and qkv.shape[1] >= (nq + 2 * nkv) * d and pos.numel() == T and rows.numel() == T):
        raise RuntimeError("dtg: kv_cache_append_: qkv must be [T, (nq + 2 nkv) * head_dim] with one pos and row per token")
    pos, rows = pos.long(), rows.long()
    ok = (pos >= 0) & (pos < k_cache.shape[2]) & (rows >= 0) & (rows < k_cache.shape[0])
    if cos.numel():
        ok &= pos < cos.shape[0]
        sel = qkv[ok]
        rope_(sel, cos, sin, pos[ok], nq + nkv, d, False)
        qkv[ok] = sel
    k = qkv[:, nq * d:(nq + nkv) * d].reshape(T, nkv, d)
    v = qkv[:, (nq + nkv) * d:(nq + 2 * nkv) * d].reshape(T, nkv, d)
    k_cache[rows[ok], :, pos[ok]] = k[ok]
    v_cache[rows[ok], :, pos[ok]] = v[ok]


def decode_attn(qkv, k_cache, v_cache, rows, lens, nq, nkv, head_dim, scale, max_len, window=0, splits=0):
    B, d, g = qkv.shape[0], head_dim, nq // nkv
    if nq % nkv or not (k_cache.dim() == 4 and k_cache.shape == v_cache.shape and k_cache.shape[1] == nkv
                        and k_cache.shape[3] == d):
        raise RuntimeError("dtg: decode_attn: caches must be contiguous bf16 [rows_max, nkv, S_max, head_dim]")
    if not 0 <= max_len <= k_cache.shape[2]:
        raise RuntimeError("dtg: decode_attn: max_len must lie in [0, S_max]")
    out = torch.zeros(B, nq * d, dtype=qkv.dtype)
    for b in range(B):
        n, r = int(lens[b]), int(rows[b])
        if not 0 <= r < k_cache.shape[0]:
            continue
        n = min(n, k_cache.shape[2])
        lo = max(0, n - window) if window > 0 else 0
        if n <= lo:
            continue
        q = qkv[b, : nq * d].float().reshape(nkv, g, d)
        k, v = k_cache[r, :, lo:n].float(), v_cache[r, :, lo:n].float()
        p = torch.softmax(torch.einsum("hgd,hsd->hgs", q, k) * scale, -1)
        out[b] = torch.einsum("hgs,hsd->hgd", p, v).reshape(nq * d).to(qkv.dtype)
    return out


def swiglu_fwd(gu):
    inter = gu.shape[1] // 2
    g, u = gu[:, :inter].float(), gu[:, inter:].float()
    return (F.silu(g) * u).to(gu.dtype)


SKINNY_MAX_M = 16


def skinny_linear(x, w, bias, act=0):
    name = "dtg: skinny_linear"
    if x.dtype != torch.bfloat16 or w.dtype != torch.bfloat16:
        raise RuntimeError(f"{name}: x and w must be bf16 tensors")
    if act not in (0, 1):
        raise RuntimeError(f"{name}: act must be 0 (none) or 1 (SwiGLU)")
    if x.dim() != 2 or not 1 <= x.shape[0] <= SKINNY_MAX_M:
        raise RuntimeError(f"{name}: x must be [M, K] with 1 <= M <= {SKINNY_MAX_M}")
    K = x.shape[1]
    if K % 8:
        raise RuntimeError(f"{name}: K must be a multiple of 8")
    if x.stride(1) != 1 or x.stride(0) % 8 or x.data_ptr() % 16:
        raise RuntimeError(f"{name}: x must have unit inner stride and 16-B aligned rows")
    if w.dim() != 2 or w.shape[1] != K or w.shape[0] < 1 or not w.is_contiguous():
        raise RuntimeError(f"{name}: w must be a contiguous [N, K] on x's device")
    N = w.shape[0]
    if act and N % 2:
        raise RuntimeError(f"{name}: the SwiGLU epilogue needs an even N (gate rows, then up rows)")
    y = x.float() @ w.float().t()
    if bias is not None:
        if bias.dtype != torch.bfloat16 or bias.dim() != 1 or bias.shape[0] != N or not bias.is_contiguous():
            raise RuntimeError(f"{name}: bias must be a contiguous bf16 [N]")
        y = y + bias.float()
    y = y.to(x.dtype)
    return swiglu_fwd(y) if act else y


def swiglu_bwd(dh, gu):
    inter = gu.shape[1] // 2
    g, u, d = gu[:, :inter].float(), gu[:, inter:].float(), dh.float()
    s = torch.sigmoid(g)
    du = d * g * s
    dg = d * u * s * (1 + g * (1 - s))
    return torch.cat([dg, du], dim=1).to(gu.dtype)


def ce_fwd_bwd_(logits, labels, ignore_index, grad_scale, compute_grad):
    x = logits.float()
    lse = torch.logsumexp(x, dim=-1)
    valid = labels != ignore_index
    safe = torch.where(valid, labels, torch.zeros_like(labels))
    xl = x.gather(1, safe[:, None])[:, 0]
    loss = torch.where(valid, lse - xl, torch.zeros_like(lse))
    if compute_grad:
        g = torch.exp(x - lse[:, None])
        g.scatter_add_(1, safe[:, None], -torch.ones_like(g[:, :1]))
        g = g * grad_scale
        g[~valid] = 0
        logits.copy_(g.to(logits.dtype))
    return loss


def ce_stats(logits, labels, vocab_start):
    x = logits.float()
    m = x.max(-1).values
    s = torch.exp(x - m[:, None]).sum(-1)
    local = labels - vocab_start
    inside = (local >= 0) & (local < x.shape[1])
    xl = x.gather(1, local.clamp(0, x.shape[1] - 1)[:, None])[:, 0]
    return m, s, torch.where(inside, xl, torch.zeros_like(xl))


def ce_grad_(logits, labels, lse, vocab_start, ignore_index, grad_scale):
    x = logits.float()
    g = torch.exp(x - lse[:, None])
    local = labels - vocab_start
    inside = (local >= 0) & (local < x.shape[1])
    onehot = torch.zeros_like(g)
    rows = torch.nonzero(inside).flatten()
    onehot[rows, local[rows]] = 1.0
    g = (g - onehot) * grad_scale
    g[labels == ignore_index] = 0
    logits.copy_(g.to(logits.dtype))


def adamw_t_(p, master, g, m, v, pt, mats, ntiles, lr, beta1, beta2, eps, wd, step, grad_scale, hyper=None,
             tile_cols=64, gscale=None):
    for off, rows, cols, toff, _ in mats.tolist():
        n = rows * cols
        sl = slice(off, off + n)
        adamw_(p[sl], None if master is None else master[sl], g[sl], m[sl], v[sl], lr, beta1, beta2, eps, wd,
               step, grad_scale, hyper, gscale)
        if toff >= 0:
            pt[toff:toff + n].copy_(p[sl].view(rows, cols).t().reshape(-1))


def adamw_(p, master, g, m, v, lr, beta1, beta2, eps, wd, step, grad_scale, hyper=None, gscale=None):
    bc1 = 1 - beta1**step
    bc2 = math.sqrt(1 - beta2**step)
    if hyper is not None:
        lr, bc1, bc2 = (float(x) for x in hyper[:3].tolist())
    if gscale is not None:
        grad_scale = float(torch.tensor(grad_scale, dtype=torch.float32) * gscale.float().reshape(-1)[0])
    pf = master if master is not None else p.float()
    gf = g.float() * grad_scale
    mf, vf = m.float(), v.float()
    pf = pf * (1 - lr * wd)
    mf = mf + (gf - mf) * (1 - beta1)
    vf = vf * beta2 + (1 - beta2) * gf * gf
    pf = pf - (lr / bc1) * mf / (vf.sqrt() / bc2 + eps)
    m.copy_(mf)
    v.copy_(vf)
    if master is not None:
        master.copy_(pf)
    p.copy_(pf)


_SUMSQ_CHUNK = 1 << 20


def grad_sumsq_(g, acc, slot):
    assert g.dim() == 1 and acc.dtype == torch.float32
    for i in range(0, g.numel(), _SUMSQ_CHUNK):
        acc[slot] += g[i:i + _SUMSQ_CHUNK].float().square().sum()


def _key_ranges(cu_seqlens, k_start=None, k_len=None):
    cu = cu_seqlens.tolist()
    out = []
    for i in range(len(cu) - 1):
        a, b = cu[i], cu[i + 1]
        if k_start is None:
            out.append((a, b, a, b))
        else:
            ks, kl = int(k_start[i]), int(k_len[i])
            out.append((a, b, ks, ks + kl))
    return out


def _mask(nq, nk, window=0):
    i = torch.arange(nq)[:, None]
    j = torch.arange(nk)[None, :]
    m = j > i + (nk - nq)
    if window > 0:
        m = m | (j <= i + (nk - nq) - window)
    return m


def _attn_ref(q, k, v, cu_seqlens, scale, causal, k_start=None, k_len=None, window=0):
    T, hq, d = q.shape
    hkv = k.shape[1]
    rep = hq // hkv
    o = torch.zeros(T, hq, d, dtype=torch.float32)
    lse = torch.full((hq, T), float("-inf"), dtype=torch.float32)
    for a, b, ka, kb in _key_ranges(cu_seqlens, k_start, k_len):
        if b <= a:
            continue
        qs = q[a:b].float().transpose(0, 1)
        ks = k[ka:kb].float().transpose(0, 1).repeat_interleave(rep, 0)
        vs = v[ka:kb].float().transpose(0, 1).repeat_interleave(rep, 0)
        sc = qs @ ks.transpose(1, 2) * scale
        if causal:
            sc = sc.masked_fill(_mask(b - a, kb - ka, window), float("-inf"))
        l_ = torch.logsumexp(sc, -1)
        p = torch.exp(sc - l_[..., None])
        o[a:b] = (p @ vs).transpose(0, 1)
        lse[:, a:b] = l_
    return o, lse


def _check_qkv(t, name, heads, d):
    if not (t.dim() == 3 and t.shape[1] == heads and t.shape[2] == d and t.stride(2) == 1 and t.stride(1) == d
            and t.stride(0) % 8 == 0):
        raise RuntimeError(f"dtg: {name} must be [T, H, D] with contiguous heads and 16-B aligned token stride")


def _check_attn_inputs(q, k, v):
    _check_qkv(q, "q", q.shape[1], q.shape[2])
    _check_qkv(k, "k", k.shape[1], q.shape[2])
    _check_qkv(v, "v", k.shape[1], q.shape[2])


def flash_attn_fwd(q, k, v, cu_seqlens, max_seqlen, scale, causal, window=0):
    _check_attn_inputs(q, k, v)
    o, lse = _attn_ref(q, k, v, cu_seqlens, scale, causal, window=window)
    return o.to(q.dtype), lse


_PHILOX_M = (0xD2511F53, 0xCD9E8D57)
_PHILOX_W = (0x9E3779B9, 0xBB67AE85)


def philox4x32_10(c0, c1, c2, c3, k0, k1):
    import numpy as np

    m32 = np.uint64(0xFFFFFFFF)
    c = [np.asarray(x, dtype=np.uint64) & m32 for x in (c0, c1, c2, c3)]
    k0, k1 = np.uint64(k0) & m32, np.uint64(k1) & m32
    for r in range(10):
        if r:
            k0 = (k0 + np.uint64(_PHILOX_W[0])) & m32
            k1 = (k1 + np.uint64(_PHILOX_W[1])) & m32
        p0 = np.uint64(_PHILOX_M[0]) * c[0]
        p1 = np.uint64(_PHILOX_M[1]) * c[2]
        c = [(p1 >> np.uint64(32)) ^ c[1] ^ k0, p1 & m32, (p0 >> np.uint64(32)) ^ c[3] ^ k1, p0 & m32]
    return c


def dropout_threshold(p):
    thr = max(1, min(256, int(round((1.0 - p) * 256.0))))
    return thr, 256.0 / thr


def dropout_keep(seed, offset, head, s0, nq, nk, p):
    import numpy as np

    thr, _ = dropout_threshold(p)
    q = np.arange(nq, dtype=np.uint64)[:, None]
    k = np.arange(nk, dtype=np.uint64)[None, :]
    seed = int(seed) & 0xFFFFFFFFFFFFFFFF
    offset = int(offset) & 0xFFFFFFFFFFFFFFFF
    w = philox4x32_10(k & ~np.uint64(3), np.uint64(s0) + (q & ~np.uint64(3)), np.full_like(q, head),
                      np.full_like(q, offset & 0xFFFFFFFF), seed & 0xFFFFFFFF, (seed >> 32) ^ (offset >> 32))
    sel = (q & np.uint64(3)).astype(np.int64)
    word = np.choose(np.broadcast_to(sel, (nq, nk)), [np.broadcast_to(x, (nq, nk)) for x in w])
    byte = (word >> (np.uint64(8) * (k & np.uint64(3)))) & np.uint64(255)
    return torch.from_numpy(byte.astype(np.int64) < thr)


def _drop_masks(cu_seqlens, hq, p, seed, offset):
    out = []
    for a, b, _, _ in _key_ranges(cu_seqlens):
        out.append(torch.stack([dropout_keep(seed, offset, h, a, b - a, b - a, p) for h in range(hq)]) if b > a else None)
    return out


def _rng_pair(rng):
    seed, offset = (int(x) for x in rng.reshape(-1).tolist())
    return seed, offset


def philox_rng(like, increment):
    r = torch.randint(0, 2**62, (2,))
    return torch.tensor([int(r[0]), int(r[1] % (2**31))], dtype=torch.int64)


def flash_attn_fwd_drop(q, k, v, cu_seqlens, max_seqlen, scale, causal, p, rng):
    seed, offset = _rng_pair(rng)
    _check_attn_inputs(q, k, v)
    T, hq, d = q.shape
    rep = hq // k.shape[1]
    _, sc_keep = dropout_threshold(p)
    o = torch.zeros(T, hq, d, dtype=torch.float32)
    lse = torch.full((hq, T), float("-inf"), dtype=torch.float32)
    for (a, b, _, _), m in zip(_key_ranges(cu_seqlens), _drop_masks(cu_seqlens, hq, p, seed, offset)):
        if b <= a:
            continue
        qs = q[a:b].float().transpose(0, 1)
        ks = k[a:b].float().transpose(0, 1).repeat_interleave(rep, 0)
        vs = v[a:b].float().transpose(0, 1).repeat_interleave(rep, 0)
        s = qs @ ks.transpose(1, 2) * scale
        if causal:
            s = s.masked_fill(_mask(b - a, b - a), float("-inf"))
        l_ = torch.logsumexp(s, -1)
        pr = torch.exp(s - l_[..., None]) * m * sc_keep
        o[a:b] = (pr @ vs).transpose(0, 1)
        lse[:, a:b] = l_
    return o.to(q.dtype), lse


def flash_attn_bwd_drop(dout, q, k, v, o, lse, cu_seqlens, max_seqlen, scale, causal, p, rng):
    seed, offset = _rng_pair(rng)
    _check_attn_inputs(q, k, v)
    T, hq, d = q.shape
    hkv = k.shape[1]
    rep = hq // hkv
    _, sc_keep = dropout_threshold(p)
    dq = torch.zeros(T, hq, d, dtype=torch.float32)
    dk = torch.zeros(T, hkv, d, dtype=torch.float32)
    dv = torch.zeros(T, hkv, d, dtype=torch.float32)
    for (a, b, _, _), m in zip(_key_ranges(cu_seqlens), _drop_masks(cu_seqlens, hq, p, seed, offset)):
        if b <= a:
            continue
        qs = q[a:b].float().transpose(0, 1)
        ks = k[a:b].float().transpose(0, 1).repeat_interleave(rep, 0)
        vs = v[a:b].float().transpose(0, 1).repeat_interleave(rep, 0)
        dos = dout[a:b].float().transpose(0, 1)
        os_ = o[a:b].float().transpose(0, 1)
        s = qs @ ks.transpose(1, 2) * scale
        if causal:
            s = s.masked_fill(_mask(b - a, b - a), float("-inf"))
        pr = torch.exp(s - lse[:, a:b].float()[..., None])
        z = pr * m * sc_keep
        dvh = z.transpose(1, 2) @ dos
        dpr = (dos @ vs.transpose(1, 2)) * m * sc_keep
        delta = (dos * os_).sum(-1, keepdim=True)
        ds = pr * (dpr - delta)
        dq[a:b] = (ds @ ks * scale).transpose(0, 1)
        dk[a:b] += (ds.transpose(1, 2) @ qs * scale).view(hkv, rep, b - a, d).sum(1).transpose(0, 1)
        dv[a:b] += dvh.view(hkv, rep, b - a, d).sum(1).transpose(0, 1)
    return dq.to(q.dtype), dk.to(k.dtype), dv.to(v.dtype)


_LN_STREAM_TAG = 0x4C4E4452


def ln_dropout_keep(seed, offset, T, H, p):
    import numpy as np

    thr, _ = dropout_threshold(p)
    seed = int(seed) & 0xFFFFFFFFFFFFFFFF
    offset = int(offset) & 0xFFFFFFFFFFFFFFFF
    rows = np.arange(T, dtype=np.uint64)[:, None]
    chunks = np.arange(H // 8, dtype=np.uint64)[None, :]
    shape = (T, H // 8)
    w = philox4x32_10(np.broadcast_to(chunks, shape), np.broadcast_to(rows, shape),
                      np.full(shape, offset & 0xFFFFFFFF, dtype=np.uint64),
                      np.full(shape, _LN_STREAM_TAG, dtype=np.uint64), seed & 0xFFFFFFFF, (seed >> 32) ^ (offset >> 32))
    byte = np.stack([(w[j >> 2] >> np.uint64(8 * (j & 3))) & np.uint64(255) for j in range(8)], axis=-1)
    return torch.from_numpy((byte.astype(np.int64) < thr).reshape(T, H))


def _ln_check_rows(t, name):
    if not (t.dim() == 2 and t.stride(1) == 1 and t.stride(0) % 8 == 0):
        raise RuntimeError(f"dtg: {name} must be 2-D with unit inner stride and 16-byte aligned rows")
    if t.shape[1] % 8:
        raise RuntimeError("dtg: layernorm: bad weight/hidden")
    if t.shape[1] > 16384:
        raise RuntimeError("dtg: layernorm: unsupported hidden size")


def _ln_drop(p, rng):
    if not 0.0 <= p < 1.0:
        raise RuntimeError("dtg: layernorm dropout: p must be in [0, 1)")
    if p == 0.0:
        if rng is not None:
            raise RuntimeError("dtg: layernorm dropout: rng given with p == 0")
        return None
    if rng is None:
        raise RuntimeError("dtg: layernorm dropout: rng must be a contiguous int64 [2] tensor {seed, offset}")
    return _rng_pair(rng)


def _ln_stats(h, eps):
    hf = h.float()
    mean = hf.mean(-1)
    d = hf - mean[:, None]
    return mean, torch.rsqrt((d * d).mean(-1) + eps)


def layernorm_fwd(x, w, b, eps):
    _ln_check_rows(x, "x")
    mean, rstd = _ln_stats(x, eps)
    return F.layer_norm(x, (x.shape[1],), w, b, eps), mean, rstd


def dropout_add_layernorm_fwd(x, res, w, b, eps, p, rng):
    _ln_check_rows(x, "x")
    _ln_check_rows(res, "residual")
    so = _ln_drop(p, rng)
    xf = x.float()
    if so is not None:
        keep = ln_dropout_keep(so[0], so[1], x.shape[0], x.shape[1], p)
        xf = torch.where(keep, xf * dropout_threshold(p)[1], torch.zeros_like(xf))
    h = (res.float() + xf).to(x.dtype)
    y, mean, rstd = layernorm_fwd(h, w, b, eps)
    return y, h, mean, rstd


def layernorm_bwd(dy, h, w, mean, rstd, dres, p, rng):
    _ln_check_rows(h, "h")
    so = _ln_drop(p, rng)
    dyf, wf, r = dy.float(), w.float(), rstd[:, None]
    n = (h.float() - mean[:, None]) * r
    g = dyf * wf
    dhf = r * (g - g.mean(-1, keepdim=True) - n * (g * n).mean(-1, keepdim=True))
    if dres is not None:
        dhf = dhf + dres.float()
    dh = dhf.to(h.dtype)
    dx = dh
    if so is not None:
        keep = ln_dropout_keep(so[0], so[1], h.shape[0], h.shape[1], p)
        dx = torch.where(keep, dhf * dropout_threshold(p)[1], torch.zeros_like(dhf)).to(h.dtype)
    return dh, dx, (dyf * n).sum(0).to(w.dtype), dyf.sum(0).to(w.dtype)


_GELU_C = math.sqrt(2.0 / math.pi)
_GELU_A = 0.044715


def _gelu_check(x, name):
    if not (x.dim() == 2 and x.stride(1) == 1 and x.stride(0) % 8 == 0 and x.shape[1] % 8 == 0):
        raise RuntimeError(f"dtg: {name}: x must be [T, I] with unit inner stride, 16-byte aligned rows and I % 8 == 0")


def gelu_fwd(x):
    _gelu_check(x, "gelu_fwd")
    return F.gelu(x, approximate="tanh").contiguous()


def gelu_bwd(dh, x):
    _gelu_check(x, "gelu_bwd")
    xf = x.float()
    s = torch.sigmoid(2 * _GELU_C * (xf + _GELU_A * xf * xf * xf))
    du2 = 2 * _GELU_C * (1 + 3 * _GELU_A * xf * xf)
    return (dh.float() * (s + xf * s * (1 - s) * du2)).to(x.dtype)


def gelu_bwd_t(dh, x):
    if x.shape[0] % 8:
        raise RuntimeError("dtg: gelu_bwd_t: T must be a multiple of 8")
    dx = gelu_bwd(dh, x)
    return dx, dx.t().contiguous(), gelu_fwd(x).t().contiguous()


def _qkv_heads(qkv, nq, nkv, d):
    T = qkv.shape[0]
    q = qkv[:, : nq * d].reshape(T, nq, d)
    k = qkv[:, nq * d : (nq + nkv) * d].reshape(T, nkv, d)
    v = qkv[:, (nq + nkv) * d :].reshape(T, nkv, d)
    return q, k, v


def flash_attn_bwd_qkv_drop(dout, qkv, nq, nkv, head_dim, o, lse, cu_seqlens, max_seqlen, scale, causal, p, rng):
    T = qkv.shape[0]
    q, k, v = _qkv_heads(qkv, nq, nkv, head_dim)
    dq, dk, dv = flash_attn_bwd_drop(dout, q, k, v, o, lse, cu_seqlens, max_seqlen, scale, causal, p, rng)
    return torch.cat([dq.reshape(T, -1), dk.reshape(T, -1), dv.reshape(T, -1)], dim=1)


def flash_attn_varlen_fwd(q, k, v, cu_seqlens_q, k_start, k_len, max_seqlen_q, max_seqlen_k, scale, causal):
    _check_attn_inputs(q, k, v)
    o, lse = _attn_ref(q, k, v, cu_seqlens_q, scale, causal, k_start, k_len)
    return o.to(q.dtype), lse


def flash_attn_bwd(dout, q, k, v, o, lse, cu_seqlens, max_seqlen, scale, causal, window=0, k_start=None, k_len=None):
    T, hq, d = q.shape
    _check_attn_inputs(q, k, v)
    if not (lse.dtype == torch.float32 and lse.is_contiguous() and tuple(lse.shape) == (hq, T)):
        raise RuntimeError("dtg: flash_attn_bwd: lse must be f32 [Hq, T]")
    if not (o.is_contiguous() and dout.shape == o.shape and o.shape[0] == T):
        raise RuntimeError("dtg: flash_attn_bwd: o/dout")
    hkv = k.shape[1]
    rep = hq // hkv
    dq = torch.zeros(T, hq, d, dtype=torch.float32)
    dk = torch.zeros(k.shape[0], hkv, d, dtype=torch.float32)
    dv = torch.zeros(k.shape[0], hkv, d, dtype=torch.float32)
    for a, b, ka, kb in _key_ranges(cu_seqlens, k_start, k_len):
        if b <= a:
            continue
        qs = q[a:b].float().transpose(0, 1)
        ks = k[ka:kb].float().transpose(0, 1).repeat_interleave(rep, 0)
        vs = v[ka:kb].float().transpose(0, 1).repeat_interleave(rep, 0)
        dos = dout[a:b].float().transpose(0, 1)
        os_ = o[a:b].float().transpose(0, 1)
        sc = qs @ ks.transpose(1, 2) * scale
        if causal:
            sc = sc.masked_fill(_mask(b - a, kb - ka, window), float("-inf"))
        p = torch.exp(sc - lse[:, a:b].float()[..., None])
        dvh = p.transpose(1, 2) @ dos
        dp = dos @ vs.transpose(1, 2)
        delta = (dos * os_).sum(-1, keepdim=True)
        ds = p * (dp - delta)
        dqh = ds @ ks * scale
        dkh = ds.transpose(1, 2) @ qs * scale
        dq[a:b] = dqh.transpose(0, 1)
        dk[ka:kb] += dkh.view(hkv, rep, kb - ka, d).sum(1).transpose(0, 1)
        dv[ka:kb] += dvh.view(hkv, rep, kb - ka, d).sum(1).transpose(0, 1)
    return dq.to(q.dtype), dk.to(k.dtype), dv.to(v.dtype)


def flash_attn_varlen_bwd(dout, q, k, v, o, lse, cu_seqlens_q, k_start, k_len, max_seqlen_q, max_seqlen_k, scale,
                          causal):
    return flash_attn_bwd(dout, q, k, v, o, lse, cu_seqlens_q, max_seqlen_q, scale, causal, 0, k_start, k_len)


def flash_attn_bwd_qkv(dout, qkv, nq, nkv, head_dim, o, lse, cu_seqlens, max_seqlen, scale, causal, window=0):
    T = qkv.shape[0]
    q, k, v = _qkv_heads(qkv, nq, nkv, head_dim)
    dq, dk, dv = flash_attn_bwd(dout, q, k, v, o, lse, cu_seqlens, max_seqlen, scale, causal, window)
    return torch.cat([dq.reshape(T, -1), dk.reshape(T, -1), dv.reshape(T, -1)], dim=1)


def flash_attn_bwd_qkv_rope(dout, qkv, nq, nkv, head_dim, o, lse, cu_seqlens, max_seqlen, scale, causal, cos, sin,
                            pos, window=0):
    dqkv = flash_attn_bwd_qkv(dout, qkv, nq, nkv, head_dim, o, lse, cu_seqlens, max_seqlen, scale, causal, window)
    rope_(dqkv, cos, sin, pos, nq + nkv, head_dim, True)
    return dqkv


def swiglu_bwd_t(dh, gu):
    if not (gu.dim() == 2 and gu.stride(1) == 1 and gu.stride(0) % 8 == 0 and gu.shape[1] % 16 == 0):
        raise RuntimeError("dtg: swiglu_bwd_t: the pre-activation must be [T, 2 * I] with unit inner stride, "
                           "16-byte aligned rows and I % 8 == 0")
    if not (dh.dim() == 2 and dh.shape[0] == gu.shape[0] and dh.shape[1] == gu.shape[1] // 2):
        raise RuntimeError("dtg: swiglu_bwd_t: shape mismatch")
    dgu = swiglu_bwd(dh, gu)
    return dgu, dgu.t().contiguous(), swiglu_fwd(gu).t().contiguous()


def transpose2d(x):
    return x.t().contiguous()


def transpose_mats_(x, out, mats, mats_host, ntiles):
    for so, r, c, do, _t0 in mats_host.tolist():
        out[do:do + r * c].copy_(x[so:so + r * c].view(r, c).t().reshape(-1))


def embedding_bwd_(out, ids, dy):
    acc = torch.zeros(out.shape, dtype=torch.float32)
    ids = ids.reshape(-1)
    keep = (ids >= 0) & (ids < out.shape[0])
    acc.index_add_(0, ids[keep], dy.reshape(-1, dy.shape[-1])[keep].float())
    out.copy_((out.float() + acc).to(out.dtype))


def sample_u(rng):
    import numpy as np

    g = rng.detach().cpu().numpy().astype(np.int64).view(np.uint64).reshape(-1, 3)
    lo, hi = g & np.uint64(0xFFFFFFFF), g >> np.uint64(32)
    w0 = philox4x32_10(lo[:, 2], hi[:, 2], lo[:, 1], hi[:, 1], lo[:, 0], hi[:, 0])[0]
    u = (w0 >> np.uint64(8)).astype(np.float32) * np.float32(2.0 ** -24)
    return torch.from_numpy(u).to(rng.device)


def sample_logits(logits, params, top_k, rng, u=None):
    n, V = logits.shape
    dev = logits.device
    if n == 0:
        return torch.empty(0, dtype=torch.int64, device=dev), torch.empty(0, dtype=torch.int32, device=dev)
    ninf = float("-inf")
    x = logits.to(torch.float64)
    x = torch.where(torch.isnan(x), torch.full_like(x, ninf), x)
    T, top_p, min_p = (params[:, i].to(torch.float64) for i in range(3))
    k = top_k.to(torch.int64)
    idx = torch.arange(V, device=dev)
    M = x.max(1).values
    first_max = torch.where(x == M[:, None], idx, V).min(1).values
    n_max = (x == M[:, None]).sum(1)
    dead, hot = M == ninf, M == float("inf")
    greedy = ~(T > 0)
    special = dead | hot | greedy
    Ms = torch.where(special, torch.zeros_like(M), M)[:, None]
    Ts = torch.where(special, torch.ones_like(T), T)[:, None]
    xs = torch.where(special[:, None], torch.zeros_like(x), x)
    w = torch.where(xs == Ms, torch.ones_like(xs), torch.exp((xs - Ms) / Ts))
    w = torch.where(xs == ninf, torch.zeros_like(w), w)

    desc, order = xs.sort(1, descending=True)
    asc = desc.flip(1).contiguous()
    kth = desc.gather(1, (k - 1).clamp(0, V - 1)[:, None])[:, 0]
    t_k = torch.where((k > 0) & (k < V), kth, torch.full_like(kth, ninf))
    in_a = xs >= t_k[:, None]
    wa = w * in_a
    z_a = wa.sum(1)
    cs = wa.gather(1, order).cumsum(1)
    n_ge = V - torch.searchsorted(asc, desc.contiguous(), right=False)
    mass_ge = cs.gather(1, n_ge - 1)
    ok = (desc >= t_k[:, None]) & (mass_ge >= (top_p * z_a)[:, None])
    t_p = torch.where(ok, desc, torch.full_like(desc, ninf)).max(1).values
    t_p = torch.where((top_p > 0) & (top_p < 1), t_p, torch.where(top_p <= 0, Ms[:, 0], torch.full_like(t_p, ninf)))
    t_m = torch.where(min_p > 0, Ms[:, 0] + Ts[:, 0] * torch.log(min_p.clamp_min(1e-300)), torch.full_like(M, ninf))
    t_m = torch.where(torch.isnan(t_m), torch.full_like(t_m, ninf), t_m)
    thr = torch.minimum(torch.maximum(torch.maximum(t_k, t_p), t_m), Ms[:, 0])
    in_k = xs >= thr[:, None]
    c = (w * in_k).cumsum(1)
    z_k = c[:, -1]
    if u is None:
        u = sample_u(rng)
    u = u.to(torch.float64)
    u = torch.where(u >= 0, u.clamp(max=1.0), torch.zeros_like(u))
    ids = torch.searchsorted(c, (u * z_k)[:, None], right=True)[:, 0]
    last = torch.where(in_k, idx, -1).max(1).values
    ids = torch.where(ids >= V, last, ids)
    kept = in_k.sum(1)

    ids = torch.where(greedy | hot, first_max, ids)
    kept = torch.where(greedy, torch.ones_like(kept), kept)
    kept = torch.where(hot, n_max, kept)
    ids = torch.where(dead, torch.full_like(ids, -1), ids)
    kept = torch.where(dead, torch.zeros_like(kept), kept)
    return ids.to(torch.int64), kept.to(torch.int32)


_TUNING = [0, 64]


def flash_attn_tuning(like, kv_split, kv_qb):
    old = list(_TUNING)
    if kv_split >= 0:
        _TUNING[0] = int(kv_split)
    if kv_qb >= 0:
        _TUNING[1] = int(kv_qb)
    return old


for _name, _fn in list(globals().items()):
    if _name in (
        "rmsnorm_fwd", "add_rmsnorm_fwd", "rmsnorm_bwd", "rope_", "swiglu_fwd", "swiglu_bwd",
        "ce_fwd_bwd_", "ce_stats", "ce_grad_", "adamw_", "adamw_t_", "grad_sumsq_", "flash_attn_fwd", "flash_attn_bwd",
        "flash_attn_bwd_qkv", "transpose2d", "transpose_mats_", "swiglu_bwd_t", "embedding_bwd_", "flash_attn_varlen_fwd",
        "flash_attn_varlen_bwd", "flash_attn_fwd_drop", "flash_attn_bwd_drop", "flash_attn_bwd_qkv_drop", "philox_rng",
        "flash_attn_bwd_qkv_rope", "flash_attn_tuning", "layernorm_fwd", "dropout_add_layernorm_fwd", "layernorm_bwd",
        "gelu_fwd", "gelu_bwd", "gelu_bwd_t", "qk_norm_rope_fwd_", "qk_norm_rope_bwd_", "kv_cache_append_", "decode_attn",
        "sample_logits", "skinny_linear",
    ):
        LIB.impl(_name, _fn, "CPU")
```

lambda-labs_distributed-training-guide_amd/ops/_schema.py:

```python
import torch

LIB = torch.library.Library("dtg", "DEF")

_DEFS = [
    "rmsnorm_fwd(Tensor x, Tensor w, float eps) -> (Tensor, Tensor)",
    "add_rmsnorm_fwd(Tensor x, Tensor residual, Tensor w, float eps) -> (Tensor, Tensor, Tensor)",
    "rmsnorm_bwd(Tensor dy, Tensor x, Tensor w, Tensor rstd, Tensor? dres) -> (Tensor, Tensor)",
    "layernorm_fwd(Tensor x, Tensor w, Tensor b, float eps) -> (Tensor, Tensor, Tensor)",
    "dropout_add_layernorm_fwd(Tensor x, Tensor residual, Tensor w, Tensor b, float eps, float p, Tensor? rng) "
    "-> (Tensor, Tensor, Tensor, Tensor)",
    "layernorm_bwd(Tensor dy, Tensor h, Tensor w, Tensor mean, Tensor rstd, Tensor? dres, float p, Tensor? rng) "
    "-> (Tensor, Tensor, Tensor, Tensor)",
    "gelu_fwd(Tensor x) -> Tensor",
    "gelu_bwd(Tensor dh, Tensor x) -> Tensor",
    "gelu_bwd_t(Tensor dh, Tensor x) -> (Tensor, Tensor, Tensor)",
    "rope_(Tensor(a!) qkv, Tensor cos, Tensor sin, Tensor pos, int nheads, int head_dim, bool inverse) -> ()",
    "qk_norm_rope_fwd_(Tensor(a!) qkv, Tensor wq, Tensor wk, Tensor cos, Tensor sin, Tensor pos, int nq, int nkv, "
    "int head_dim, float eps) -> (Tensor, Tensor)",
    "qk_norm_rope_bwd_(Tensor(a!) dqkv, Tensor xqk, Tensor rstd, Tensor wq, Tensor wk, Tensor cos, Tensor sin, "
    "Tensor pos, int nq, int nkv, int head_dim) -> (Tensor, Tensor)",
    "kv_cache_append_(Tensor(a!) qkv, Tensor(b!) k_cache, Tensor(c!) v_cache, Tensor cos, Tensor sin, Tensor pos, "
    "Tensor rows, int nq, int nkv, int head_dim) -> ()",
    "decode_attn(Tensor qkv, Tensor k_cache, Tensor v_cache, Tensor rows, Tensor lens, int nq, int nkv, int head_dim, "
    "float scale, int max_len, int window=0, int splits=0) -> Tensor",
    "sample_logits(Tensor logits, Tensor params, Tensor top_k, Tensor rng, Tensor? u=None) -> (Tensor, Tensor)",
    "skinny_linear(Tensor x, Tensor w, Tensor? bias, int act=0) -> Tensor",
    "swiglu_fwd(Tensor gu) -> Tensor",
    "swiglu_bwd(Tensor dh, Tensor gu) -> Tensor",
    "swiglu_bwd_t(Tensor dh, Tensor gu) -> (Tensor, Tensor, Tensor)",
    "ce_fwd_bwd_(Tensor(a!) logits, Tensor labels, int ignore_index, float grad_scale, bool compute_grad) -> Tensor",
    "ce_stats(Tensor logits, Tensor labels, int vocab_start) -> (Tensor, Tensor, Tensor)",
    "ce_grad_(Tensor(a!) logits, Tensor labels, Tensor lse, int vocab_start, int ignore_index, float grad_scale) -> ()",
    "adamw_(Tensor(a!) p, Tensor(b!)? master, Tensor g, Tensor(c!) m, Tensor(d!) v, float lr, float beta1, "
    "float beta2, float eps, float wd, int step, float grad_scale, Tensor? hyper=None, Tensor? gscale=None) -> ()",
    "adamw_t_(Tensor(a!) p, Tensor(b!)? master, Tensor g, Tensor(c!) m, Tensor(d!) v, Tensor(e!) pt, Tensor mats, "
    "int ntiles, float lr, float beta1, float beta2, float eps, float wd, int step, float grad_scale, "
    "Tensor? hyper=None, int tile_cols=64, Tensor? gscale=None) -> ()",
    "grad_sumsq_(Tensor g, Tensor(a!) acc, int slot) -> ()",
    "adamw_cpu_(Tensor(a!) p, Tensor g, Tensor(b!) m, Tensor(c!) v, float lr, float beta1, float beta2, "
    "float eps, float wd, int step, float grad_scale) -> ()",
    "flash_attn_fwd(Tensor q, Tensor k, Tensor v, Tensor cu_seqlens, int max_seqlen, float scale, bool causal, "
    "int window=0) -> (Tensor, Tensor)",
    "flash_attn_bwd(Tensor dout, Tensor q, Tensor k, Tensor v, Tensor o, Tensor lse, Tensor cu_seqlens, "
    "int max_seqlen, float scale, bool causal, int window=0) -> (Tensor, Tensor, Tensor)",
    "flash_attn_bwd_qkv(Tensor dout, Tensor qkv, int nq, int nkv, int head_dim, Tensor o, Tensor lse, "
    "Tensor cu_seqlens, int max_seqlen, float scale, bool causal, int window=0) -> Tensor",
    "flash_attn_bwd_qkv_rope(Tensor dout, Tensor qkv, int nq, int nkv, int head_dim, Tensor o, Tensor lse, "
    "Tensor cu_seqlens, int max_seqlen, float scale, bool causal, Tensor cos, Tensor sin, Tensor pos, "
    "int window=0) -> Tensor",
    "flash_attn_fwd_drop(Tensor q, Tensor k, Tensor v, Tensor cu_seqlens, int max_seqlen, float scale, bool causal, "
    "float p, Tensor rng) -> (Tensor, Tensor)",
    "flash_attn_bwd_drop(Tensor dout, Tensor q, Tensor k, Tensor v, Tensor o, Tensor lse, Tensor cu_seqlens, "
    "int max_seqlen, float scale, bool causal, float p, Tensor rng) -> (Tensor, Tensor, Tensor)",
    "flash_attn_bwd_qkv_drop(Tensor dout, Tensor qkv, int nq, int nkv, int head_dim, Tensor o, Tensor lse, "
    "Tensor cu_seqlens, int max_seqlen, float scale, bool causal, float p, Tensor rng) -> Tensor",
    "philox_rng(Tensor like, int increment) -> Tensor",
    "transpose2d(Tensor x) -> Tensor",
    "transpose_mats_(Tensor x, Tensor(a!) out, Tensor mats, Tensor mats_host, int ntiles) -> ()",
    "embedding_bwd_(Tensor(a!) out, Tensor ids, Tensor dy) -> ()",
    "flash_attn_varlen_fwd(Tensor q, Tensor k, Tensor v, Tensor cu_seqlens_q, Tensor k_start, Tensor k_len, "
    "int max_seqlen_q, int max_seqlen_k, float scale, bool causal) -> (Tensor, Tensor)",
    "flash_attn_varlen_bwd(Tensor dout, Tensor q, Tensor k, Tensor v, Tensor o, Tensor lse, Tensor cu_seqlens_q, "
    "Tensor k_start, Tensor k_len, int max_seqlen_q, int max_seqlen_k, float scale, bool causal) "
    "-> (Tensor, Tensor, Tensor)",
    "flash_attn_fwd_stamped(Tensor q, Tensor k, Tensor v, Tensor cu_seqlens, int max_seqlen, float scale, "
    "bool causal) -> (Tensor, Tensor, Tensor)",
    "flash_attn_tuning(Tensor like, int kv_split, int kv_qb) -> int[]",
]

for _d in _DEFS:
    LIB.define(_d)
```

lambda-labs_distributed-training-guide_amd/ops/functional.py:

```python
import math
import os

import torch
import torch.distributed as dist
import torch.nn.functional as F

from . import grad_routing as _gr
from .grad_routing import route_embedding_grad, route_param_grad, route_weight_grad_mm

ops = torch.ops.dtg


_LINEAR_BWD = os.environ.get("DTG_LINEAR_BWD", "tn")
_TN_MIN_TOKENS = 4096


def _tn_ok(*ts):
    return all(t.is_cuda and t.dtype == torch.bfloat16 and t.shape[0] % 8 == 0 and t.shape[1] % 8 == 0
               and t.stride(1) == 1 for t in ts)


def _wt(w):
    ref = getattr(w, "_dtg_wt", None)
    if ref is not None:
        t = ref[0].weight_t(ref[1])
        if t is not None:
            return t
    return ops.transpose2d(w)


def _bwd_layout(x, w):
    mode = _LINEAR_BWD
    if mode == "native" or x.shape[0] < _TN_MIN_TOKENS or not _tn_ok(x, w):
        return False, False
    if mode == "tn":
        return True, True
    return True, w.shape[0] >= w.shape[1]


def _bias_grad(b, dy):
    return route_param_grad(b, dy.sum(0, dtype=torch.float32).to(dy.dtype))


def _dx_mm(dy, w, tn):
    return torch.mm(dy, _wt(w).t()) if tn else torch.mm(dy, w)


def _dw_mm(w, dy, x, tn, dy_t=None, x_t=None):
    if not (tn and _tn_ok(dy)):
        return route_weight_grad_mm(w, dy, x)
    return route_weight_grad_mm(w, dy, x, a_t=ops.transpose2d(dy) if dy_t is None else dy_t,
                                b_t=ops.transpose2d(x) if x_t is None else x_t)


def _linear_backward(ctx, dy, x, w):
    dx_tn, dw_tn = _bwd_layout(x, w)
    dx = _dx_mm(dy, w, dx_tn) if ctx.needs_input_grad[0] else None
    dw = _dw_mm(w, dy, x, dw_tn) if ctx.needs_input_grad[1] else None
    return dx, dw


class _Linear(torch.autograd.Function):
    @staticmethod
    def forward(ctx, x, w, out=None):
        ctx.save_for_backward(x, w)
        if out is not None:
            return torch.mm(x, w.t(), out=out[0])
        return torch.mm(x, w.t())

    @staticmethod
    def backward(ctx, dy):
        x, w = ctx.saved_tensors
        return (*_linear_backward(ctx, dy, x, w), None)


def linear(x, w, b=None, out=None):
    if b is None:
        return _Linear.apply(x, w, None if out is None else (out,))
    assert out is None, "linear: out= is for the bias-free projections"
    return _LinearBias.apply(x, w, b)


class _LinearBias(torch.autograd.Function):
    @staticmethod
    def forward(ctx, x, w, b):
        ctx.save_for_backward(x, w, b)
        return torch.addmm(b, x, w.t())

    @staticmethod
    def backward(ctx, dy):
        x, w, b = ctx.saved_tensors
        dx, dw = _linear_backward(ctx, dy, x, w)
        return dx, dw, _bias_grad(b, dy) if ctx.needs_input_grad[2] else None


class _RMSNorm(torch.autograd.Function):
    @staticmethod
    def forward(ctx, x, w, eps):
        y, rstd = ops.rmsnorm_fwd(x, w, eps)
        ctx.save_for_backward(x, w, rstd)
        return y

    @staticmethod
    def backward(ctx, dy):
        x, w, rstd = ctx.saved_tensors
        dx, dw = ops.rmsnorm_bwd(dy, x, w, rstd, None)
        return dx, route_param_grad(w, dw), None


class _AddRMSNorm(torch.autograd.Function):
    @staticmethod
    def forward(ctx, x, res, w, eps):
        y, h, rstd = ops.add_rmsnorm_fwd(x, res, w, eps)
        ctx.save_for_backward(h, w, rstd)
        return y, h

    @staticmethod
    def backward(ctx, dy, dh):
        h, w, rstd = ctx.saved_tensors
        if dy is None:
            dy = torch.zeros_like(h)
        dx, dw = ops.rmsnorm_bwd(dy, h, w, rstd, dh)
        return dx, dx, route_param_grad(w, dw), None


def rms_norm(x, w, eps):
    return _RMSNorm.apply(x, w, eps)


def add_rms_norm(x, res, w, eps):
    return _AddRMSNorm.apply(x, res, w, eps)


class _LayerNorm(torch.autograd.Function):
    @staticmethod
    def forward(ctx, x, w, b, eps):
        y, mean, rstd = ops.layernorm_fwd(x, w, b, eps)
        ctx.save_for_backward(x, w, b, mean, rstd)
        return y

    @staticmethod
    def backward(ctx, dy):
        x, w, b, mean, rstd = ctx.saved_tensors
        dx, _, dw, db = ops.layernorm_bwd(dy, x, w, mean, rstd, None, 0.0, None)
        return dx, route_param_grad(w, dw), route_param_grad(b, db), None


class _DropoutAddLayerNorm(torch.autograd.Function):

    @staticmethod
    def forward(ctx, x, res, w, b, eps, p, rng):
        y, h, mean, rstd = ops.dropout_add_layernorm_fwd(x, res, w, b, eps, p, rng)
        saved = (h, w, b, mean, rstd) if rng is None else (h, w, b, mean, rstd, rng)
        ctx.save_for_backward(*saved)
        ctx.p = p
        return y, h

    @staticmethod
    def backward(ctx, dy, dh_in):
        h, w, b, mean, rstd, *rng = ctx.saved_tensors
        if dy is None:
            dy = torch.zeros_like(h)
        dh, dx, dw, db = ops.layernorm_bwd(dy, h, w, mean, rstd, dh_in, ctx.p, rng[0] if rng else None)
        return dx, dh, route_param_grad(w, dw), route_param_grad(b, db), None, None, None


def layer_norm(x, w, b, eps):
    return _LayerNorm.apply(x, w, b, eps)


def dropout_add_layer_norm(x, res, w, b, eps, p=0.0):
    p = float(p)
    return _DropoutAddLayerNorm.apply(x, res, w, b, eps, p, dropout_rng(x) if p > 0.0 else None)


def _llama3_inv_freq(inv_freq, scaling):
    factor = scaling["factor"]
    low = scaling.get("low_freq_factor", 1.0)
    high = scaling.get("high_freq_factor", 4.0)
    old_ctx = scaling["original_max_position_embeddings"]
    low_wl = old_ctx / low
    high_wl = old_ctx / high
    wavelen = 2 * math.pi / inv_freq
    out = torch.where(wavelen > low_wl, inv_freq / factor, inv_freq)
    smooth = (old_ctx / wavelen - low) / (high - low)
    smoothed = (1 - smooth) * out / factor + smooth * out
    is_medium = (wavelen >= high_wl) & (wavelen <= low_wl)
    return torch.where(is_medium, smoothed, out)


def rope_tables(head_dim, theta, max_pos, scaling=None, device=None):
    inv_freq = 1.0 / (theta ** (torch.arange(0, head_dim, 2, dtype=torch.int64).float() / head_dim))
    attn_factor = 1.0
    if scaling is not None:
        kind = scaling.get("rope_type", scaling.get("type"))
        if kind == "llama3":
            inv_freq = _llama3_inv_freq(inv_freq, scaling)
        elif kind in (None, "default"):
            pass
        else:
            raise NotImplementedError(f"rope scaling {kind}")
    t = torch.arange(max_pos, dtype=torch.float32)
    freqs = torch.outer(t, inv_freq)
    cos = (freqs.cos() * attn_factor).contiguous()
    sin = (freqs.sin() * attn_factor).contiguous()
    if device is not None:
        cos, sin = cos.to(device), sin.to(device)
    return cos, sin


_FA_ROPE_FUSED = os.environ.get("DTG_FA_ROPE_FUSED", "1") == "1"


def _qkv_head_views(qkv, nq, nkv, d):
    T = qkv.shape[0]

    def view(h0, nh):
        return qkv.as_strided((T, nh, d), (qkv.stride(0), d, 1), qkv.storage_offset() + h0 * d)

    return view(0, nq), view(nq, nkv), view(nq + nkv, nkv)


class _AttentionQKV(torch.autograd.Function):
    @staticmethod
    def forward(ctx, qkv, cos, sin, pos, cu_seqlens, max_seqlen, nq, nkv, head_dim, scale, causal, rope, window):
        T = qkv.shape[0]
        d = head_dim
        if rope:
            ops.rope_(qkv, cos, sin, pos, nq + nkv, d, False)
        q, k, v = _qkv_head_views(qkv, nq, nkv, d)
        o, lse = ops.flash_attn_fwd(q, k, v, cu_seqlens, max_seqlen, scale, causal, window)
        ctx.save_for_backward(qkv, o, lse, cu_seqlens, cos, sin, pos)
        ctx.meta = (max_seqlen, nq, nkv, d, scale, causal, rope, window)
        return o.view(T, nq * d)

    @staticmethod
    def backward(ctx, do):
        qkv, o, lse, cu, cos, sin, pos = ctx.saved_tensors
        max_seqlen, nq, nkv, d, scale, causal, rope, window = ctx.meta
        T = qkv.shape[0]
        if rope and _FA_ROPE_FUSED:
            dqkv = ops.flash_attn_bwd_qkv_rope(do.contiguous().view(T, nq, d), qkv, nq, nkv, d, o, lse, cu, max_seqlen,
                                               scale, causal, cos, sin, pos, window)
        else:
            dqkv = ops.flash_attn_bwd_qkv(do.contiguous().view(T, nq, d), qkv, nq, nkv, d, o, lse, cu, max_seqlen,
                                          scale, causal, window)
            if rope:
                ops.rope_(dqkv, cos, sin, pos, nq + nkv, d, True)
        return dqkv, None, None, None, None, None, None, None, None, None, None, None, None


class _AttentionQKVDrop(torch.autograd.Function):

    @staticmethod
    def forward(ctx, qkv, cu_seqlens, max_seqlen, nq, nkv, head_dim, scale, causal, p, rng):
        T = qkv.shape[0]
        d = head_dim
        q, k, v = _qkv_head_views(qkv, nq, nkv, d)
        o, lse = ops.flash_attn_fwd_drop(q, k, v, cu_seqlens, max_seqlen, scale, causal, p, rng)
        ctx.save_for_backward(qkv, o, lse, cu_seqlens, rng)
        ctx.meta = (max_seqlen, nq, nkv, d, scale, causal, p)
        return o.view(T, nq * d)

    @staticmethod
    def backward(ctx, do):
        qkv, o, lse, cu, rng = ctx.saved_tensors
        max_seqlen, nq, nkv, d, scale, causal, p = ctx.meta
        T = qkv.shape[0]
        dqkv = ops.flash_attn_bwd_qkv_drop(do.contiguous().view(T, nq, d), qkv, nq, nkv, d, o, lse, cu, max_seqlen,
                                           scale, causal, p, rng)
        return dqkv, None, None, None, None, None, None, None, None, None


def dropout_rng(like):
    return ops.philox_rng(like, 4)


class _Rope(torch.autograd.Function):

    @staticmethod
    def forward(ctx, qkv, cos, sin, pos, nheads, head_dim):
        y = qkv.contiguous().clone()
        ops.rope_(y, cos, sin, pos, nheads, head_dim, False)
        ctx.save_for_backward(cos, sin, pos)
        ctx.meta = (nheads, head_dim)
        return y

    @staticmethod
    def backward(ctx, dy):
        cos, sin, pos = ctx.saved_tensors
        dx = dy.contiguous().clone()
        ops.rope_(dx, cos, sin, pos, ctx.meta[0], ctx.meta[1], True)
        return dx, None, None, None, None, None


def rope(qkv, cos, sin, pos, nheads, head_dim):
    return _Rope.apply(qkv, cos, sin, pos, int(nheads), int(head_dim))


FA_HEAD_DIMS = (64, 128)


_QKNORM_FUSED = os.environ.get("DTG_QKNORM_FUSED", "1") == "1"


class _QKNormRope(torch.autograd.Function):

    @staticmethod
    def forward(ctx, qkv, wq, wk, cos, sin, pos, nq, nkv, head_dim, eps, grad_inplace):
        xqk, rstd = ops.qk_norm_rope_fwd_(qkv, wq, wk, cos, sin, pos, nq, nkv, head_dim, eps)
        ctx.mark_dirty(qkv)
        ctx.save_for_backward(xqk, rstd, wq, wk, cos, sin, pos)
        ctx.meta = (nq, nkv, head_dim, grad_inplace)
        return qkv

    @staticmethod
    def backward(ctx, dqkv):
        xqk, rstd, wq, wk, cos, sin, pos = ctx.saved_tensors
        nq, nkv, d, grad_inplace = ctx.meta
        dense = dqkv.dim() == 2 and dqkv.stride(1) == 1 and dqkv.stride(0) >= dqkv.shape[1] and dqkv.stride(0) % 8 == 0
        if not (grad_inplace and dense):
            dqkv = dqkv.contiguous().clone() if dense else dqkv.contiguous()
        dwq, dwk = ops.qk_norm_rope_bwd_(dqkv, xqk, rstd, wq, wk, cos, sin, pos, nq, nkv, d)
        return (dqkv, route_param_grad(wq, dwq), route_param_grad(wk, dwk), None, None, None, None, None, None, None,
                None)


class _RoutedParam(torch.autograd.Function):

    @staticmethod
    def forward(ctx, w):
        ctx.w = w
        return w.view_as(w)

    @staticmethod
    def backward(ctx, g):
        return route_param_grad(ctx.w, g.to(ctx.w.dtype))


def _qk_norm_rope_composed(qkv, wq, wk, eps, nq, nkv, d, cos, sin, pos):
    T, nh = qkv.shape[0], nq + nkv
    xf = qkv[:, : nh * d].reshape(T, nh, d).float()
    n = xf * torch.rsqrt(xf.pow(2).mean(-1, keepdim=True) + eps)
    wq, wk = _RoutedParam.apply(wq).float(), _RoutedParam.apply(wk).float()
    y = torch.cat([wq * n[:, :nq], wk * n[:, nq:]], 1)
    if cos is not None:
        h = d // 2
        c, s = cos[pos][:, None, :], sin[pos][:, None, :]
        y1, y2 = y[..., :h], y[..., h:]
        y = torch.cat([y1 * c - y2 * s, y2 * c + y1 * s], -1)
    return torch.cat([y.reshape(T, nh * d).to(qkv.dtype), qkv[:, nh * d:]], 1)


def qk_norm_rope(qkv, wq, wk, eps, nq, nkv, head_dim, cos=None, sin=None, pos=None, grad_inplace=False):
    nq, nkv, d = int(nq), int(nkv), int(head_dim)
    if not _QKNORM_FUSED or (qkv.is_cuda and d not in FA_HEAD_DIMS):
        return _qk_norm_rope_composed(qkv, wq, wk, float(eps), nq, nkv, d, cos, sin, pos)
    if cos is None:
        cos = sin = torch.empty(0, device=qkv.device)
        pos = torch.empty(0, dtype=torch.long, device=qkv.device)
    if qkv.is_leaf and qkv.requires_grad:
        qkv = qkv.clone()
    return _QKNormRope.apply(qkv, wq, wk, cos, sin, pos, nq, nkv, d, float(eps), bool(grad_inplace))


def _attention_padded(qkv, nq, nkv, d, cu_seqlens, max_seqlen, cos, sin, pos, causal, scale, window):
    dp = next((x for x in FA_HEAD_DIMS if x >= d), None)
    if dp is None or d % 2:
        raise ValueError(f"attention: head_dim {d} unsupported (kernels: {FA_HEAD_DIMS}; smaller even dims are padded)")
    T = qkv.shape[0]
    x = qkv.reshape(T, nq + 2 * nkv, d)
    if cos is not None:
        h = d // 2
        qk = x[:, : nq + nkv].float()
        c, s = cos[pos][:, None, :], sin[pos][:, None, :]
        x1, x2 = qk[..., :h], qk[..., h:]
        rot = torch.cat([x1 * c - x2 * s, x2 * c + x1 * s], -1).to(x.dtype)
        x = torch.cat([rot, x[:, nq + nkv:]], 1)
    xp = F.pad(x, (0, dp - d)).reshape(T, (nq + 2 * nkv) * dp)
    e = torch.empty(0, device=qkv.device)
    o = _AttentionQKV.apply(xp, e, e, torch.empty(0, dtype=torch.long, device=qkv.device), cu_seqlens, int(max_seqlen),
                            nq, nkv, dp, float(scale), causal, False, int(window or 0))
    return o.view(T, nq, dp)[..., :d].reshape(T, nq * d)


def attention(qkv, nq, nkv, head_dim, cu_seqlens, max_seqlen, cos=None, sin=None, pos=None, causal=True, scale=None,
              window=0, dropout_p=0.0):
    if scale is None:
        scale = 1.0 / math.sqrt(head_dim)
    if dropout_p > 0.0:
        if cos is not None or window:
            raise ValueError("attention dropout is supported without RoPE / sliding windows (GPT-2)")
        if qkv.is_cuda and head_dim not in FA_HEAD_DIMS:
            raise ValueError(f"attention dropout: head_dim {head_dim} needs a kernel instantiation {FA_HEAD_DIMS}")
        return _AttentionQKVDrop.apply(qkv, cu_seqlens, int(max_seqlen), nq, nkv, head_dim, float(scale), causal,
                                       float(dropout_p), dropout_rng(qkv))
    if qkv.is_cuda and head_dim not in FA_HEAD_DIMS:
        return _attention_padded(qkv, nq, nkv, head_dim, cu_seqlens, max_seqlen, cos, sin, pos, causal, scale, window)
    rope = cos is not None
    if not rope:
        cos = sin = torch.empty(0, device=qkv.device)
        pos = torch.empty(0, dtype=torch.long, device=qkv.device)
    return _AttentionQKV.apply(qkv, cos, sin, pos, cu_seqlens, int(max_seqlen), nq, nkv, head_dim, float(scale), causal, rope,
                               int(window or 0))


_DECODE_FUSED = os.environ.get("DTG_DECODE_FUSED", "1") == "1"
DECODE_GROUPS = (1, 2, 3, 4, 7, 8, 16)


def _decode_kernels(qkv, nq, nkv, d):
    if not _DECODE_FUSED:
        return False
    return not qkv.is_cuda or (qkv.dtype == torch.bfloat16 and d in FA_HEAD_DIMS and nq // nkv in DECODE_GROUPS)


def _check_cache_args(name, qkv, k_cache, v_cache, nq, nkv, d, index):
    if nq < 1 or nkv < 1 or nq % nkv:
        raise ValueError(f"{name}: nq ({nq}) must be a positive multiple of nkv ({nkv})")
    if qkv.dim() != 2 or qkv.shape[1] != (nq + 2 * nkv) * d:
        raise ValueError(f"{name}: qkv must be [T, (nq + 2 nkv) * head_dim], got {tuple(qkv.shape)}")
    if k_cache.dim() != 4 or k_cache.shape != v_cache.shape or k_cache.shape[1] != nkv or k_cache.shape[3] != d:
        raise ValueError(f"{name}: caches must be [rows_max, {nkv}, S_max, {d}], got {tuple(k_cache.shape)} / "
                         f"{tuple(v_cache.shape)}")
    if k_cache.dtype != qkv.dtype or v_cache.dtype != qkv.dtype or not (k_cache.is_contiguous() and v_cache.is_contiguous()):
        raise ValueError(f"{name}: caches must be contiguous and of qkv's dtype")
    for what, t in index.items():
        if t.dim() != 1 or t.numel() != qkv.shape[0] or t.dtype not in (torch.int32, torch.int64):
            raise ValueError(f"{name}: {what} must be an integer tensor [{qkv.shape[0]}], got {t.dtype} {tuple(t.shape)}")


@torch.no_grad()
def kv_cache_append(qkv, k_cache, v_cache, pos, rows, nq, nkv, head_dim, cos=None, sin=None, pos_max=None,
                    row_max=None):
    nq, nkv, d = int(nq), int(nkv), int(head_dim)
    _check_cache_args("kv_cache_append", qkv, k_cache, v_cache, nq, nkv, d, {"pos": pos, "rows": rows})
    if (cos is None) != (sin is None):
        raise ValueError("kv_cache_append: pass both cos and sin, or neither")
    if cos is not None and (cos.dim() != 2 or cos.shape[1] != d // 2 or cos.shape != sin.shape):
        raise ValueError(f"kv_cache_append: tables must be [max_pos, {d // 2}]")
    if pos_max is not None and not 0 <= int(pos_max) < min(k_cache.shape[2], cos.shape[0] if cos is not None else 1 << 62):
        raise ValueError(f"kv_cache_append: position {int(pos_max)} outside the cache (S_max = {k_cache.shape[2]}) or the "
                         f"RoPE tables")
    if row_max is not None and not 0 <= int(row_max) < k_cache.shape[0]:
        raise ValueError(f"kv_cache_append: cache row {int(row_max)} outside [0, {k_cache.shape[0]})")
    pos, rows = pos.long(), rows.to(torch.int32)
    if _decode_kernels(qkv, nq, nq, d):
        e = torch.empty(0, device=qkv.device)
        ops.kv_cache_append_(qkv, k_cache, v_cache, e if cos is None else cos, e if sin is None else sin,
                             pos.contiguous(), rows.contiguous(), nq, nkv, d)
        return qkv
    T, h = qkv.shape[0], d // 2
    ok = (pos >= 0) & (pos < k_cache.shape[2]) & (rows >= 0) & (rows < k_cache.shape[0])
    if cos is not None:
        ok &= pos < cos.shape[0]
        p = pos.clamp(0, cos.shape[0] - 1)
        x = qkv[:, : (nq + nkv) * d].reshape(T, nq + nkv, d).float()
        c, s = cos[p][:, None, :], sin[p][:, None, :]
        x1, x2 = x[..., :h], x[..., h:]
        rot = torch.cat([x1 * c - x2 * s, x2 * c + x1 * s], -1).reshape(T, (nq + nkv) * d).to(qkv.dtype)
        qkv[:, : (nq + nkv) * d] = torch.where(ok[:, None], rot, qkv[:, : (nq + nkv) * d])
    r, p = rows.long()[ok], pos[ok]
    k_cache[r, :, p] = qkv[:, nq * d:(nq + nkv) * d].reshape(T, nkv, d)[ok]
    v_cache[r, :, p] = qkv[:, (nq + nkv) * d:].reshape(T, nkv, d)[ok]
    return qkv


@torch.no_grad()
def decode_attention(qkv, k_cache, v_cache, rows, lens, nq, nkv, head_dim, max_len, scale=None, window=0, splits=0):
    nq, nkv, d = int(nq), int(nkv), int(head_dim)
    _check_cache_args("decode_attention", qkv, k_cache, v_cache, nq, nkv, d, {"rows": rows, "lens": lens})
    max_len, window, splits = int(max_len), int(window or 0), int(splits)
    if not 0 <= max_len <= k_cache.shape[2]:
        raise ValueError(f"decode_attention: max_len {max_len} outside [0, S_max = {k_cache.shape[2]}]")
    if window < 0 or splits < 0:
        raise ValueError("decode_attention: window and splits must not be negative")
    if scale is None:
        scale = 1.0 / math.sqrt(d)
    if _decode_kernels(qkv, nq, nkv, d):
        return ops.decode_attn(qkv, k_cache, v_cache, rows.to(torch.int32).contiguous(), lens.to(torch.int32).contiguous(),
                               nq, nkv, d, float(scale), max_len, window, splits)
    B, g = qkv.shape[0], nq // nkv
    n = lens.long().clamp(0, max_len)
    r = rows.long()
    n = torch.where((r >= 0) & (r < k_cache.shape[0]), n, torch.zeros_like(n))
    r = r.clamp(0, k_cache.shape[0] - 1)
    j = torch.arange(max_len, device=qkv.device)
    keep = j[None] < n[:, None]
    if window > 0:
        keep &= j[None] >= (n - window)[:, None]
    q = qkv[:, : nq * d].reshape(B, nkv, g, d).float()
    k = torch.where(keep[:, None, :, None], k_cache[r, :, :max_len].float(), torch.zeros((), device=qkv.device))
    v = torch.where(keep[:, None, :, None], v_cache[r, :, :max_len].float(), torch.zeros((), device=qkv.device))
    s = torch.einsum("bhgd,bhsd->bhgs", q, k) * float(scale)
    s = s.masked_fill(~keep[:, None, None, :], float("-inf"))
    p = torch.softmax(s, -1).masked_fill(~keep[:, None, None, :], 0.0)
    return torch.einsum("bhgs,bhsd->bhgd", p, v).reshape(B, nq * d).to(qkv.dtype)


_SAMPLE_FUSED = os.environ.get("DTG_SAMPLE_FUSED", "1") == "1"

_SAMPLE_RULES = {
    "temperature": (lambda v: v >= 0.0, "temperature >= 0"),
    "top_k": (lambda v: v >= 0, "top_k >= 0"),
    "top_p": (lambda v: 0.0 < v <= 1.0, "0 < top_p <= 1"),
    "min_p": (lambda v: 0.0 <= v <= 1.0, "0 <= min_p <= 1"),
}


def check_sample_scalar(name, v):
    ok, text = _SAMPLE_RULES[name]
    if not ok(v):
        raise ValueError(f"sample_logits: need {text}, got {name} = {v!r}")


def _sample_column(name, v, n, dtype, device):
    if isinstance(v, torch.Tensor):
        if v.dim() != 1 or v.shape[0] != n or v.device != device:
            raise ValueError(f"sample_logits: a tensor {name} must be [{n}] on the logits' device, got "
                             f"{tuple(v.shape)} on {v.device}")
        return v.to(dtype)
    if name in _SAMPLE_RULES:
        check_sample_scalar(name, v)
    if dtype == torch.int64:
        v = (int(v) + 2**63) % 2**64 - 2**63
    return torch.full((n,), v, dtype=dtype, device=device)


@torch.no_grad()
def sample_logits(logits, temperature=0.0, top_k=0, top_p=1.0, min_p=0.0, seed=0, stream=None, step=0, u=None):
    if logits.dim() != 2 or logits.shape[1] < 1:
        raise ValueError(f"sample_logits: logits must be [n, V] with V >= 1, got {tuple(logits.shape)}")
    n, V = logits.shape
    dev = logits.device
    col = lambda name, v, dt: _sample_column(name, v, n, dt, dev)
    params = torch.stack([col("temperature", temperature, torch.float32), col("top_p", top_p, torch.float32),
                          col("min_p", min_p, torch.float32)], 1)
    k = col("top_k", top_k, torch.int32)
    if stream is None:
        stream = torch.arange(n, dtype=torch.int64, device=dev)
    rng = torch.stack([col("seed", seed, torch.int64), col("stream", stream, torch.int64),
                       col("step", step, torch.int64)], 1)
    if u is not None:
        u = col("u", u, torch.float32)
    if n and (logits.stride(1) != 1 or (n > 1 and logits.stride(0) < V)):
        logits = logits.contiguous()
    if logits.is_cuda and not (_SAMPLE_FUSED and logits.dtype in (torch.bfloat16, torch.float32)):
        from . import _cpu

        return _cpu.sample_logits(logits, params, k, rng, u)
    return ops.sample_logits(logits, params, k, rng, u)


class _SwiGLU(torch.autograd.Function):
    @staticmethod
    def forward(ctx, gu):
        ctx.save_for_backward(gu)
        return ops.swiglu_fwd(gu)

    @staticmethod
    def backward(ctx, dh):
        (gu,) = ctx.saved_tensors
        return ops.swiglu_bwd(dh.contiguous(), gu)


def swiglu(gu):
    return _SwiGLU.apply(gu)


_SKINNY_FUSED = os.environ.get("DTG_SKINNY_FUSED", "1") == "1"
SKINNY_MAX_M = 16


@torch.no_grad()
def skinny_linear(x, w, b=None, act=None):
    if act not in (None, 0, 1, "swiglu"):
        raise ValueError(f"skinny_linear: act must be None or 'swiglu', got {act!r}")
    act = 1 if act in (1, "swiglu") else 0
    if x.dim() != 2 or w.dim() != 2 or x.shape[1] != w.shape[1]:
        raise ValueError(f"skinny_linear: x [M, K] and w [N, K] do not match: {tuple(x.shape)}, {tuple(w.shape)}")
    if x.shape[0] > SKINNY_MAX_M:
        raise ValueError(f"skinny_linear: M = {x.shape[0]} rows exceed the kernel's limit of {SKINNY_MAX_M}")
    if act and w.shape[0] % 2:
        raise ValueError(f"skinny_linear: the SwiGLU epilogue needs an even N, got {w.shape[0]}")
    if b is not None:
        b = b.reshape(-1)
    if x.is_cuda and not (_SKINNY_FUSED and x.dtype == torch.bfloat16 and w.dtype == torch.bfloat16):
        y = torch.mm(x, w.t()) if b is None else torch.addmm(b, x, w.t())
        if not act:
            return y
        inter = w.shape[0] // 2
        if inter % 8 == 0:
            return ops.swiglu_fwd(y)
        g, u = y[:, :inter].float(), y[:, inter:].float()
        return (F.silu(g) * u).to(y.dtype)
    return ops.skinny_linear(x, w, b, act)


def _mlp_backward(act, x, w1, w2, a, dy, b1=None, b2=None):
    dy = dy.contiguous()
    dx_tn, dw_tn = _bwd_layout(x, w1)
    fused = dw_tn and _tn_ok(dy, a) and a.stride(0) == a.shape[1]
    db2 = None if b2 is None else _bias_grad(b2, dy)
    dh = _dx_mm(dy, w2, dx_tn)
    if fused:
        da, da_t, h_t = getattr(ops, act + "_bwd_t")(dh, a)
        del dh
        dw2 = _dw_mm(w2, dy, None, True, x_t=h_t)
        del h_t
    else:
        da_t = None
        h = getattr(ops, act + "_fwd")(a)
        da = getattr(ops, act + "_bwd")(dh, a)
        del dh
        dw2 = _dw_mm(w2, dy, h, False)
        del h
    db1 = None if b1 is None else _bias_grad(b1, da)
    dx = _dx_mm(da, w1, dx_tn)
    dw1 = _dw_mm(w1, da, x, fused, dy_t=da_t)
    return dx, dw1, dw2, db1, db2


class _SwiGLUMLP(torch.autograd.Function):

    @staticmethod
    def forward(ctx, x, w_gu, w_down, out=None):
        gu = torch.mm(x, w_gu.t())
        h = ops.swiglu_fwd(gu)
        ctx.save_for_backward(x, w_gu, w_down, gu)
        if out is not None:
            return torch.mm(h, w_down.t(), out=out[0])
        return torch.mm(h, w_down.t())

    @staticmethod
    def backward(ctx, dy):
        x, w_gu, w_down, gu = ctx.saved_tensors
        dx, dw_gu, dw_down, _, _ = _mlp_backward("swiglu", x, w_gu, w_down, gu, dy)
        return dx, dw_gu, dw_down, None


def swiglu_mlp(x, w_gu, w_down, out=None):
    return _SwiGLUMLP.apply(x, w_gu, w_down, None if out is None else (out,))


class _GeluMLP(torch.autograd.Function):

    @staticmethod
    def forward(ctx, x, w_fc, b_fc, w_proj, b_proj):
        a = torch.addmm(b_fc, x, w_fc.t())
        h = ops.gelu_fwd(a)
        ctx.save_for_backward(x, w_fc, b_fc, w_proj, b_proj, a)
        return torch.addmm(b_proj, h, w_proj.t())

    @staticmethod
    def backward(ctx, dy):
        x, w_fc, b_fc, w_proj, b_proj, a = ctx.saved_tensors
        dx, dw_fc, dw_proj, db_fc, db_proj = _mlp_backward("gelu", x, w_fc, w_proj, a, dy, b_fc, b_proj)
        return dx, dw_fc, db_fc, dw_proj, db_proj


def gelu_mlp(x, w_fc, b_fc, w_proj, b_proj):
    return _GeluMLP.apply(x, w_fc, b_fc, w_proj, b_proj)


class _Embedding(torch.autograd.Function):
    @staticmethod
    def forward(ctx, ids, w):
        ctx.save_for_backward(ids)
        ctx.w = w
        return F.embedding(ids, w)

    @staticmethod
    def backward(ctx, dy):
        (ids,) = ctx.saved_tensors
        w = ctx.w
        return None, route_embedding_grad(w, ids, dy.contiguous(), w.shape[0])


def embedding(ids, w):
    return _Embedding.apply(ids, w)


def _default_chunk(vocab, hidden_rows):
    gib = float(os.environ.get("DTG_CE_CHUNK_GIB", "1"))
    n = max(1, -(-hidden_rows * max(vocab, 1) // max(1, int(gib * (1 << 29)))))
    per = -(-hidden_rows // n)
    return max(1024, min(hidden_rows, -(-per // 64) * 64))


def _ce_tn(h, w):
    return _LINEAR_BWD != "native" and _tn_ok(h, w)


def _ce_dx(logits, w, w_t, out):
    if w_t is not None:
        torch.mm(logits, w_t.t(), out=out)
    else:
        torch.mm(logits, w, out=out)


class _FusedLinearCE(torch.autograd.Function):
    @staticmethod
    def forward(ctx, h, w, labels, ignore_index, num_valid, chunk):
        T = h.shape[0]
        need = ctx.needs_input_grad[0] or ctx.needs_input_grad[1]
        scale = 1.0 / max(num_valid, 1)
        loss_sum = torch.zeros((), dtype=torch.float32, device=h.device)
        dh = torch.empty_like(h) if need else None
        want_dw = need and ctx.needs_input_grad[1]
        direct = want_dw and _gr.direct_loss_grad() and getattr(w, "main_grad", None) is not None
        dw = torch.empty(w.shape, dtype=w.dtype, device=h.device) if (want_dw and not direct) else None
        V = w.shape[0]
        pad = (-V) % 8 if (need and h.is_cuda and _LINEAR_BWD != "native" and chunk % 8 == 0
                           and _tn_ok(h)) else 0
        wp = w
        if pad:
            wp = torch.zeros((V + pad, w.shape[1]), dtype=w.dtype, device=w.device)
            wp[:V].copy_(w.detach())
        tn = need and _ce_tn(h, wp) and chunk % 8 == 0
        w_t = (_wt(w) if wp is w else ops.transpose2d(wp)) if (tn and ctx.needs_input_grad[0]) else None
        for s in range(0, T, chunk):
            e = min(T, s + chunk)
            lp = torch.mm(h[s:e], wp.t())
            logits = lp[:, :V] if pad else lp
            rows = ops.ce_fwd_bwd_(logits, labels[s:e], ignore_index, scale, need)
            loss_sum += rows.sum()
            if need:
                _ce_dx(lp, wp, w_t, dh[s:e])
                if direct and tn:
                    _gr.accumulate_mm_into_main_grad(w, logits, h[s:e], a_t=ops.transpose2d(lp)[:V],
                                                     b_t=ops.transpose2d(h[s:e]))
                elif direct:
                    _gr.accumulate_mm_into_main_grad(w, logits, h[s:e])
                elif dw is not None:
                    if s == 0:
                        torch.mm(logits.t(), h[s:e], out=dw)
                    else:
                        dw.addmm_(logits.t(), h[s:e])
        ctx.save_for_backward(dh, dw)
        ctx.w = w
        ctx.direct = direct
        return loss_sum * scale

    @staticmethod
    def backward(ctx, go):
        dh, dw = ctx.saved_tensors
        w = ctx.w
        if ctx.direct:
            _gr.notify_param(w)
            return dh, None, None, None, None, None
        gdh = (dh * go.to(dh.dtype)) if ctx.needs_input_grad[0] else None
        gdw = route_param_grad(w, dw * go.to(dw.dtype)) if dw is not None else None
        return gdh, gdw, None, None, None, None


def fused_linear_cross_entropy(h, w, labels, ignore_index=-100, num_valid=None, chunk=None):
    if num_valid is None:
        num_valid = int((labels != ignore_index).sum().item())
    if chunk is None:
        chunk = _default_chunk(w.shape[0], h.shape[0])
    return _FusedLinearCE.apply(h, w, labels, ignore_index, int(num_valid), int(chunk))


class _VocabParallelFusedLinearCE(torch.autograd.Function):

    @staticmethod
    def forward(ctx, h, w, labels, ignore_index, num_valid, chunk, vocab_start, group):
        from ..utils import comm as _comm

        T = h.shape[0]
        need = ctx.needs_input_grad[0] or ctx.needs_input_grad[1]
        scale = 1.0 / max(num_valid, 1)
        loss_sum = torch.zeros((), dtype=torch.float32, device=h.device)
        dh = torch.empty_like(h) if need else None
        want_dw = need and ctx.needs_input_grad[1]
        direct = want_dw and _gr.direct_loss_grad() and getattr(w, "main_grad", None) is not None
        dw = torch.empty(w.shape, dtype=w.dtype, device=h.device) if (want_dw and not direct) else None
        tn = need and _ce_tn(h, w) and chunk % 8 == 0 and w.shape[0] % 8 == 0
        w_t = _wt(w) if (tn and ctx.needs_input_grad[0]) else None

        def issue(s, e):
            logits = torch.mm(h[s:e], w.t())
            m, sx, xl = ops.ce_stats(logits, labels[s:e], vocab_start)
            stats, work = _comm.all_gather_stack_async(torch.stack([m, sx, xl]), group)
            return s, e, logits, stats, work

        def finish(s, e, logits, stats, work):
            nonlocal loss_sum
            work.wait()
            gm = stats[:, 0].amax(0)
            sx = (stats[:, 1] * torch.exp(stats[:, 0] - gm)).sum(0)
            lse = gm + torch.log(sx)
            lab = labels[s:e]
            valid = lab != ignore_index
            loss_sum += torch.where(valid, lse - stats[:, 2].sum(0), torch.zeros_like(lse)).sum()
            if not need:
                return
            ops.ce_grad_(logits, lab, lse.contiguous(), vocab_start, ignore_index, scale)
            _ce_dx(logits, w, w_t, dh[s:e])
            if not want_dw:
                return
            a_t = ops.transpose2d(logits) if tn else None
            b_t = ops.transpose2d(h[s:e]) if tn else None
            if direct:
                _gr.accumulate_mm_into_main_grad(w, logits, h[s:e], a_t=a_t, b_t=b_t)
            else:
                lhs, rhs = (a_t, b_t.t()) if tn else (logits.t(), h[s:e])
                if s == 0:
                    torch.mm(lhs, rhs, out=dw)
                else:
                    dw.addmm_(lhs, rhs)

        pend = None
        for s in range(0, T, chunk):
            cur = issue(s, min(T, s + chunk))
            if pend is not None:
                finish(*pend)
            pend = cur
        if pend is not None:
            finish(*pend)
        ctx.save_for_backward(dh, dw)
        ctx.w = w
        ctx.direct = direct
        return loss_sum * scale

    @staticmethod
    def backward(ctx, go):
        dh, dw = ctx.saved_tensors
        if ctx.direct:
            _gr.notify_param(ctx.w)
            return dh, None, None, None, None, None, None, None
        gdh = dh * go.to(dh.dtype) if ctx.needs_input_grad[0] else None
        gdw = route_param_grad(ctx.w, dw * go.to(dw.dtype)) if dw is not None else None
        return gdh, gdw, None, None, None, None, None, None


def vocab_parallel_fused_linear_cross_entropy(h, w_local, labels, vocab_start, group, ignore_index=-100,
                                              num_valid=None, chunk=None):
    if num_valid is None:
        num_valid = int((labels != ignore_index).sum().item())
    if chunk is None:
        chunk = _default_chunk(w_local.shape[0], h.shape[0])
    return _VocabParallelFusedLinearCE.apply(h, w_local, labels, ignore_index, int(num_valid), int(chunk),
                                             int(vocab_start), group)
```

Measured before the change: 27590 tokens/s (whole job).

## Emit transposed attention outputs from flash-attention kernels for weight-gradient GEMMs

Forward and backward flash-attention kernels can now also write a feature-major transposed copy of O and of dQKV, using DPP quad shuffles so lanes store packed columns. A new fused attention-block autograd function (QKV projection, RoPE, attention, output projection) passes these transposed tensors to the weight-gradient matmuls, so the TN path does not need its own transpose pass. The cost is an extra strided global write per kernel and extra saved memory for O transposed, and the fused block replaces the layer's old forward path when its eligibility checks pass.

Result: no change. 27650 tokens/s (whole job), median of 4 (+0.2%).

```diff
diff --git a/csrc/kernels/flash_attn.hip b/csrc/kernels/flash_attn.hip
--- a/csrc/kernels/flash_attn.hip
+++ b/csrc/kernels/flash_attn.hip
@@ -214,6 +214,46 @@
         w[2 + x] = r[1];
       }
       if (ok) *reinterpret_cast<uint4*>(row + 32 * d + 16 * j + 8 * h) = make_uint4(w[0], w[1], w[2], w[3]);
+    }
+  }
+}
+
+__device__ __forceinline__ uint32_t quad_xor1(uint32_t x) {
+  return (uint32_t)__builtin_amdgcn_mov_dpp((int)x, 0xB1, 0xF, 0xF, true);
+}
+__device__ __forceinline__ uint32_t quad_xor2(uint32_t x) {
+  return (uint32_t)__builtin_amdgcn_mov_dpp((int)x, 0x4E, 0xF, 0xF, true);
+}
+
+template <int ND>
+__device__ __forceinline__ void store_cols_t(const f32x16* acc, float scale, uint16_t* col0, int64_t ld, bool ok,
+                                             bool wide) {
+  const int lane = threadIdx.x & 63;
+  const int h = lane >> 5, j = lane & 3;
+  if (!wide) {
+    if (ok) {
+#pragma unroll
+      for (int d = 0; d < ND; ++d) {
+#pragma unroll
+        for (int i = 0; i < 16; ++i) col0[(int64_t)(32 * d + 8 * (i >> 2) + 4 * h + (i & 3)) * ld] = f2bf(acc[d][i] * scale);
+      }
+    }
+    return;
+  }
+  const bool odd = (j & 1) != 0, up = (j & 2) != 0;
+  uint16_t* p = col0 + (int64_t)(4 * h + j) * ld - j;
+#pragma unroll
+  for (int d = 0; d < ND; ++d) {
+#pragma unroll
+    for (int g = 0; g < 4; ++g) {
+      const uint32_t w0 = (uint32_t)f2bf(acc[d][4 * g + 0] * scale) | ((uint32_t)f2bf(acc[d][4 * g + 1] * scale) << 16);
+      const uint32_t w1 = (uint32_t)f2bf(acc[d][4 * g + 2] * scale) | ((uint32_t)f2bf(acc[d][4 * g + 3] * scale) << 16);
+      const uint32_t r0 = quad_xor1(w0), r1 = quad_xor1(w1);
+      const uint32_t x = odd ? (r0 >> 16) | (w0 & 0xffff0000u) : (w0 & 0xffffu) | (r0 << 16);
+      const uint32_t y = odd ? (r1 >> 16) | (w1 & 0xffff0000u) : (w1 & 0xffffu) | (r1 << 16);
+      const uint32_t got = quad_xor2(up ? x : y);
+      const uint2 out = up ? make_uint2(got, y) : make_uint2(x, got);
+      if (ok) *reinterpret_cast<uint2*>(p + (int64_t)(32 * d + 8 * g) * ld) = out;
     }
   }
 }
@@ -240,6 +280,7 @@
   const int *kstart, *klen;
   int window;
   DropCfg drop;
+  uint16_t* o_t = nullptr;
 };
 
 __device__ __forceinline__ void fa_stamp(long long* st, int slot, int k) {
@@ -252,7 +293,7 @@
   }
 }
 
-template <int D, bool CAUSAL, bool WIN = false, bool DROP = false>
+template <int D, bool CAUSAL, bool WIN = false, bool DROP = false, bool EMIT_T = false>
 __global__ __launch_bounds__(256, 2) void fwd_kernel(FwdParams P) {
   [[maybe_unused]] const DropCfg dcfg = DROP ? resolve_drop(P.drop) : P.drop;
   constexpr int RB = 2 * D;
@@ -415,6 +456,8 @@
   const float inv = (lt > 0.f ? 1.f / lt : 0.f) * (DROP ? P.drop.scale : 1.f);
   uint16_t* op = P.o + ((int64_t)(s0 + min(qrow, seqlen - 1)) * P.hq + head) * D;
   store_rows_wide<ND>(acc, inv, op, qrow < seqlen);
+  if constexpr (EMIT_T)
+    store_cols_t<ND>(acc, inv, P.o_t + (int64_t)head * D * P.T + s0 + qrow, P.T, qrow < seqlen, ((s0 | seqlen) & 3) == 0);
   if (qrow < seqlen && h == 0)
     P.lse[(int64_t)head * P.T + s0 + qrow] = (lt > 0.f) ? (m + log2f(lt)) * kLn2 : -INFINITY;
   if (P.stamps != nullptr) {
@@ -442,6 +485,7 @@
   DropCfg drop;
   const float *rope_cos, *rope_sin;
   const int64_t* rope_pos;
+  uint16_t* dqkv_t = nullptr;
 };
 
 template <int ND>
@@ -470,7 +514,7 @@
   }
 }
 
-template <int D, bool CAUSAL, int OCC, bool WIN = false, bool DROP = false>
+template <int D, bool CAUSAL, int OCC, bool WIN = false, bool DROP = false, bool EMIT_T = false>
 __global__ __launch_bounds__(256, OCC) void bwd_dq_kernel(BwdParams P) {
   [[maybe_unused]] const DropCfg dcfg = DROP ? resolve_drop(P.drop) : P.drop;
   constexpr int RB = 2 * D;
@@ -653,9 +697,11 @@
 
   if (P.rope_cos != nullptr) rope_inv_rows<ND>(acc, P.rope_cos, P.rope_sin, P.rope_pos[s0 + min(qrow, seqlen - 1)]);
   store_rows_wide<ND>(acc, P.scale, P.dq + (int64_t)(s0 + min(qrow, seqlen - 1)) * P.sdq + (int64_t)head * D, qok);
-}
-
-template <int D, bool CAUSAL, int PF, bool WIN = false, int QB = kKvBQ, bool DROP = false>
+  if constexpr (EMIT_T)
+    store_cols_t<ND>(acc, P.scale, P.dqkv_t + (int64_t)head * D * P.T + s0 + qrow, P.T, qok, ((s0 | seqlen) & 3) == 0);
+}
+
+template <int D, bool CAUSAL, int PF, bool WIN = false, int QB = kKvBQ, bool DROP = false, bool EMIT_T = false>
 __global__ __launch_bounds__(256, D == 128 ? 1 : 2) void bwd_dkdv_kernel(BwdParams P) {
   [[maybe_unused]] const DropCfg dcfg = DROP ? resolve_drop(P.drop) : P.drop;
   static_assert(QB == 32 || QB == 64, "query rows per item");
@@ -955,6 +1001,12 @@
   if (P.rope_cos != nullptr) rope_inv_rows<ND>(dk, P.rope_cos, P.rope_sin, P.rope_pos[krow]);
   store_rows_wide<ND>(dk, P.scale, P.dk + krow * P.sdk + (int64_t)kvh * D, key < klen);
   store_rows_wide<ND>(dv, 1.f, P.dv + krow * P.sdv + (int64_t)kvh * D, key < klen);
+  if constexpr (EMIT_T) {
+    const bool wide = ((s0 | seqlen) & 3) == 0;
+    uint16_t* kt = P.dqkv_t + (int64_t)(P.hq + kvh) * D * P.T + s0 + key;
+    store_cols_t<ND>(dk, P.scale, kt, P.T, key < klen, wide);
+    store_cols_t<ND>(dv, 1.f, kt + (int64_t)P.hkv * D * P.T, P.T, key < klen, wide);
+  }
 }
 
 template <int D>
@@ -1021,24 +1073,27 @@
   hipLaunchKernelGGL(kernel, dim3(pl.grid.x, pl.grid.y, pl.grid.z), dim3(256), lds, st, P);
   DTG_LAUNCH_CHECK();
 }
-template <int D, bool C, bool WIN = false, bool DROP = false>
+template <int D, bool C, bool WIN = false, bool DROP = false, bool EMIT_T = false>
 static void fwd_launch(const fa::FwdPlan& pl, const fa::FwdParams& P, hipStream_t st) {
-  launch(fa::fwd_kernel<D, C, WIN, DROP>, pl, fa::fwd_lds_bytes(D), st, P);
-}
-template <int D, bool C, int OCC, bool WIN = false, bool DROP = false>
+  launch(fa::fwd_kernel<D, C, WIN, DROP, EMIT_T>, pl, fa::fwd_lds_bytes(D), st, P);
+}
+template <int D, bool C, int OCC, bool WIN = false, bool DROP = false, bool EMIT_T = false>
 static void dq_launch(const fa::DqPlan& pl, const fa::BwdParams& P, hipStream_t st) {
   TORCH_INTERNAL_ASSERT(pl.occ == OCC);
-  launch(fa::bwd_dq_kernel<D, C, OCC, WIN, DROP>, pl, fa::dq_lds_bytes(D), st, P);
-}
-template <int D, bool C, int PF, bool WIN = false, int QB = fa::kKvBQ, bool DROP = false>
+  launch(fa::bwd_dq_kernel<D, C, OCC, WIN, DROP, EMIT_T>, pl, fa::dq_lds_bytes(D), st, P);
+}
+template <int D, bool C, int PF, bool WIN = false, int QB = fa::kKvBQ, bool DROP = false, bool EMIT_T = false>
 static void kv_launch(const fa::KvPlan& pl, const fa::BwdParams& P, hipStream_t st) {
   TORCH_INTERNAL_ASSERT(pl.pf == PF && pl.qb == QB);
-  launch(fa::bwd_dkdv_kernel<D, C, PF, WIN, QB, DROP>, pl, fa::kv_lds_bytes(D, QB), st, P);
+  launch(fa::bwd_dkdv_kernel<D, C, PF, WIN, QB, DROP, EMIT_T>, pl, fa::kv_lds_bytes(D, QB), st, P);
 }
 
 template <int D>
 static void launch_fwd(const fa::FwdPlan& pl, const fa::FwdParams& P, hipStream_t st) {
-  if (pl.var == fa::Variant::DROP)
+  if (P.o_t != nullptr) {
+    TORCH_INTERNAL_ASSERT(pl.var == fa::Variant::PLAIN);
+    pl.causal ? fwd_launch<D, true, false, false, true>(pl, P, st) : fwd_launch<D, false, false, false, true>(pl, P, st);
+  } else if (pl.var == fa::Variant::DROP)
     pl.causal ? fwd_launch<D, true, false, true>(pl, P, st) : fwd_launch<D, false, false, true>(pl, P, st);
   else if (pl.var == fa::Variant::WIN) fwd_launch<D, true, true>(pl, P, st);
   else pl.causal ? fwd_launch<D, true>(pl, P, st) : fwd_launch<D, false>(pl, P, st);
@@ -1046,7 +1101,11 @@
 template <int D>
 static void launch_bwd_dq(const fa::DqPlan& pl, const fa::BwdParams& P, hipStream_t st) {
   constexpr int kOcc = D == 64 ? 2 : 1;
-  if (pl.var == fa::Variant::DROP)
+  if (P.dqkv_t != nullptr) {
+    TORCH_INTERNAL_ASSERT(pl.var == fa::Variant::PLAIN && pl.occ == kOcc);
+    pl.causal ? dq_launch<D, true, kOcc, false, false, true>(pl, P, st)
+              : dq_launch<D, false, kOcc, false, false, true>(pl, P, st);
+  } else if (pl.var == fa::Variant::DROP)
     pl.causal ? dq_launch<D, true, kOcc, false, true>(pl, P, st) : dq_launch<D, false, kOcc, false, true>(pl, P, st);
   else if (pl.var == fa::Variant::WIN) dq_launch<D, true, kOcc, true>(pl, P, st);
   else if (pl.occ == 2) pl.causal ? dq_launch<D, true, 2>(pl, P, st) : dq_launch<D, false, 2>(pl, P, st);
@@ -1062,7 +1121,15 @@
     P.dk_part = dk_part.data_ptr<float>();
     P.dv_part = dv_part.data_ptr<float>();
   }
-  if (pl.var == fa::Variant::DROP)
+  if (P.dqkv_t != nullptr) {
+    TORCH_INTERNAL_ASSERT(pl.var == fa::Variant::PLAIN && pl.pf == 1 && pl.nsplit == 1);
+    if (pl.qb == 64)
+      pl.causal ? kv_launch<D, true, 1, false, 64, false, true>(pl, P, st)
+                : kv_launch<D, false, 1, false, 64, false, true>(pl, P, st);
+    else
+      pl.causal ? kv_launch<D, true, 1, false, 32, false, true>(pl, P, st)
+                : kv_launch<D, false, 1, false, 32, false, true>(pl, P, st);
+  } else if (pl.var == fa::Variant::DROP)
     pl.causal ? kv_launch<D, true, 1, false, 64, true>(pl, P, st) : kv_launch<D, false, 1, false, 64, true>(pl, P, st);
   else if (pl.var == fa::Variant::WIN) kv_launch<D, true, 1, true>(pl, P, st);
   else if (pl.pf == 2) pl.causal ? kv_launch<D, true, 2>(pl, P, st) : kv_launch<D, false, 2>(pl, P, st);
@@ -1085,7 +1152,14 @@
   const fa::DropCfg* drop = nullptr;
   const at::Tensor *rope_cos = nullptr, *rope_sin = nullptr, *rope_pos = nullptr;
   at::Tensor* stamps = nullptr;
+  at::Tensor* o_t = nullptr;
+  at::Tensor* dqkv_t = nullptr;
 };
+
+static void check_t_out(const char* name, int64_t T, int64_t features) {
+  DTG_CHECK(T % 8 == 0 && features % 8 == 0, name, ": the transposed output needs T and the feature count to be "
+            "multiples of 8, got T = ", T, ", features = ", features);
+}
 
 static void check_qkv(const at::Tensor& t, const char* name, int64_t heads, int64_t d) {
   DTG_CHECK_CUDA_BF16(t);
@@ -1142,6 +1216,10 @@
   }
   if (const char* why = fa::conflict(c)) DTG_CHECK(false, why);
   if (op.drop != nullptr) P.drop = *op.drop;
+  if (op.o_t != nullptr && fa::fwd_emits_t(c)) {
+    *op.o_t = at::empty({hq * D, T}, q.options());
+    P.o_t = bf16_mut(*op.o_t);
+  }
   D == 128 ? launch_fwd<128>(pl, P, stream()) : launch_fwd<64>(pl, P, stream());
   return {o, lse};
 }
@@ -1196,6 +1274,10 @@
   if (op.drop != nullptr) P.drop = *op.drop;
   const fa::DqPlan dqp = fa::plan_dq(c, tuning());
   const fa::KvPlan kvp = fa::plan_kv(c, tuning());
+  if (op.dqkv_t != nullptr && fa::bwd_emits_t(c, tuning())) {
+    *op.dqkv_t = at::empty({(hq + 2 * hkv) * D, T}, q.options());
+    P.dqkv_t = bf16_mut(*op.dqkv_t);
+  }
   D == 128 ? launch_bwd_dq<128>(dqp, P, stream()) : launch_bwd_dq<64>(dqp, P, stream());
   D == 128 ? launch_bwd_dkdv<128>(kvp, P, stream(), q.options()) : launch_bwd_dkdv<64>(kvp, P, stream(), q.options());
 }
@@ -1250,6 +1332,38 @@
                                    const at::Tensor& sin_t, const at::Tensor& pos, int64_t window) {
   return flash_attn_bwd_fused("flash_attn_bwd_qkv_rope", dout, qkv, nq, nkv, head_dim, o, lse, cu_seqlens, max_seqlen,
                               scale, causal, {.window = window, .rope_cos = &cos_t, .rope_sin = &sin_t, .rope_pos = &pos});
+}
+
+std::tuple<at::Tensor, at::Tensor, at::Tensor> flash_attn_fwd_t(const at::Tensor& q, const at::Tensor& k,
+                                                                const at::Tensor& v, const at::Tensor& cu_seqlens,
+                                                                int64_t max_seqlen, double scale, bool causal,
+                                                                int64_t window) {
+  DTG_CHECK(q.dim() == 3, "flash_attn_fwd_t: q must be [T, H, D]");
+  check_t_out("flash_attn_fwd_t", q.size(0), q.size(1) * q.size(2));
+  at::Tensor o_t;
+  auto [o, lse] = flash_attn_fwd_impl(q, k, v, cu_seqlens, max_seqlen, scale, causal, {.window = window, .o_t = &o_t});
+  return {o, lse, o_t};
+}
+
+std::tuple<at::Tensor, at::Tensor> flash_attn_bwd_qkv_t(
+    const at::Tensor& dout, const at::Tensor& qkv, int64_t nq, int64_t nkv, int64_t head_dim, const at::Tensor& o,
+    const at::Tensor& lse, const at::Tensor& cu_seqlens, int64_t max_seqlen, double scale, bool causal,
+    const std::optional<at::Tensor>& cos_t, const std::optional<at::Tensor>& sin_t,
+    const std::optional<at::Tensor>& pos, int64_t window) {
+  const bool rope = cos_t.has_value();
+  DTG_CHECK(sin_t.has_value() == rope && pos.has_value() == rope, "flash_attn_bwd_qkv_t: pass cos, sin and pos, or none");
+  DTG_CHECK(qkv.dim() == 2, "flash_attn_bwd_qkv_t: qkv must be [T, (nq + 2 nkv) * D]");
+  check_t_out("flash_attn_bwd_qkv_t", qkv.size(0), qkv.size(1));
+  at::Tensor dqkv_t;
+  AttnOpts op{.window = window, .dqkv_t = &dqkv_t};
+  if (rope) {
+    op.rope_cos = &*cos_t;
+    op.rope_sin = &*sin_t;
+    op.rope_pos = &*pos;
+  }
+  auto dqkv = flash_attn_bwd_fused("flash_attn_bwd_qkv_t", dout, qkv, nq, nkv, head_dim, o, lse, cu_seqlens, max_seqlen,
+                                   scale, causal, op);
+  return {dqkv, dqkv_t};
 }
 
 std::tuple<at::Tensor, at::Tensor> flash_attn_varlen_fwd(
@@ -1339,6 +1453,8 @@
   m.impl("flash_attn_bwd_qkv", &flash_attn_bwd_qkv);
   m.impl("flash_attn_bwd_qkv_rope", &flash_attn_bwd_qkv_rope);
   m.impl("flash_attn_tuning", &flash_attn_tuning);
-}
-
-}
+  m.impl("flash_attn_fwd_t", &flash_attn_fwd_t);
+  m.impl("flash_attn_bwd_qkv_t", &flash_attn_bwd_qkv_t);
+}
+
+}
diff --git a/csrc/kernels/flash_attn_plan.h b/csrc/kernels/flash_attn_plan.h
--- a/csrc/kernels/flash_attn_plan.h
+++ b/csrc/kernels/flash_attn_plan.h
@@ -80,5 +80,12 @@
   return {{var, c.causal, {(unsigned)c.hkv, (unsigned)c.nseq, nkb * nsplit}, kv_lds_bytes(c.D, qb)}, pf, qb, nsplit};
 }
 
+inline bool fwd_emits_t(const Call& c) { return variant(c) == Variant::PLAIN && !c.key_ranges; }
+inline bool bwd_emits_t(const Call& c, const Tuning& t) {
+  if (variant(c) != Variant::PLAIN || c.key_ranges) return false;
+  const KvPlan kv = plan_kv(c, t);
+  return kv.pf == 1 && kv.nsplit == 1 && plan_dq(c, t).occ == (c.D == 64 ? 2 : 1);
+}
+
 }
 }
diff --git a/lambda-labs_distributed-training-guide_amd/models/llama.py b/lambda-labs_distributed-training-guide_amd/models/llama.py
--- a/lambda-labs_distributed-training-guide_amd/models/llama.py
+++ b/lambda-labs_distributed-training-guide_amd/models/llama.py
@@ -59,6 +59,7 @@
         self.nq = cfg.num_attention_heads // tp.size
         self.nkv = cfg.num_key_value_heads // tp.size
         self.d = cfg.head_dim
+        self.tp_region = tp.enabled
         h = cfg.hidden_size
         self.qkv_proj = Weight((self.nq + 2 * self.nkv) * self.d, h, device=device, dtype=dtype)
         if cfg.attention_bias:
@@ -95,8 +96,15 @@
                                grad_inplace=True)
         return ops.attention(qkv, self.nq, self.nkv, d, rc.cu_seqlens, rc.max_seqlen, window=self.window)
 
+    def _plain(self, rc: RunCtx, b, out):
+        return (b is None and out is None and not self.qk_norm and not self.window and rc.cp_group is None
+                and rc.sp_group is None and rc.cos is not None and not self.tp_region)
+
     def forward(self, x, rc: RunCtx, out=None):
         b = getattr(self.qkv_proj, "bias", None)
+        if self._plain(rc, b, out) and ops.attention_block_ok(x, self.qkv_proj.weight, self.o_proj.weight, self.d):
+            return ops.attention_block(x, self.qkv_proj.weight, self.o_proj.weight, self.nq, self.nkv, self.d,
+                                       rc.cu_seqlens, rc.max_seqlen, rc.cos, rc.sin, rc.pos)
         qkv = ops.linear(x, self.qkv_proj.weight, None if b is None else b.view(-1))
         if self.qk_norm:
             return ops.linear(self._forward_qk_norm(qkv, rc), self.o_proj.weight, out=out)
diff --git a/lambda-labs_distributed-training-guide_amd/ops/__init__.py b/lambda-labs_distributed-training-guide_amd/ops/__init__.py
--- a/lambda-labs_distributed-training-guide_amd/ops/__init__.py
+++ b/lambda-labs_distributed-training-guide_amd/ops/__init__.py
@@ -10,6 +10,8 @@
 from .functional import (
     add_rms_norm,
     attention,
+    attention_block,
+    attention_block_ok,
     check_sample_scalar,
     decode_attention,
     dropout_add_layer_norm,
@@ -50,5 +52,5 @@
     "add_rms_norm", "attention", "rope", "embedding", "fused_linear_cross_entropy", "linear", "rms_norm",
     "rope_tables", "swiglu", "swiglu_mlp", "vocab_parallel_fused_linear_cross_entropy", "route_param_grad", "adamw_step",
     "fa_tuning", "layer_norm", "dropout_add_layer_norm", "gelu_mlp", "qk_norm_rope", "kv_cache_append", "decode_attention",
-    "sample_logits", "skinny_linear",
+    "sample_logits", "skinny_linear", "attention_block", "attention_block_ok",
 ]
diff --git a/lambda-labs_distributed-training-guide_amd/ops/_cpu.py b/lambda-labs_distributed-training-guide_amd/ops/_cpu.py
--- a/lambda-labs_distributed-training-guide_amd/ops/_cpu.py
+++ b/lambda-labs_distributed-training-guide_amd/ops/_cpu.py
@@ -618,6 +618,35 @@
     return dqkv
 
 
+def _check_t_out(name, T, features):
+    if T % 8 or features % 8:
+        raise RuntimeError(f"dtg: {name}: the transposed output needs T and the feature count to be multiples of 8, "
+                           f"got T = {T}, features = {features}")
+
+
+def flash_attn_fwd_t(q, k, v, cu_seqlens, max_seqlen, scale, causal, window=0):
+    if q.dim() != 3:
+        raise RuntimeError("dtg: flash_attn_fwd_t: q must be [T, H, D]")
+    _check_t_out("flash_attn_fwd_t", q.shape[0], q.shape[1] * q.shape[2])
+    o, lse = flash_attn_fwd(q, k, v, cu_seqlens, max_seqlen, scale, causal, window)
+    return o, lse, o.reshape(o.shape[0], -1).t().contiguous()
+
+
+def flash_attn_bwd_qkv_t(dout, qkv, nq, nkv, head_dim, o, lse, cu_seqlens, max_seqlen, scale, causal, cos, sin, pos,
+                         window=0):
+    if (cos is None) != (sin is None) or (cos is None) != (pos is None):
+        raise RuntimeError("dtg: flash_attn_bwd_qkv_t: pass cos, sin and pos, or none")
+    if qkv.dim() != 2:
+        raise RuntimeError("dtg: flash_attn_bwd_qkv_t: qkv must be [T, (nq + 2 nkv) * D]")
+    _check_t_out("flash_attn_bwd_qkv_t", qkv.shape[0], qkv.shape[1])
+    if cos is None:
+        dqkv = flash_attn_bwd_qkv(dout, qkv, nq, nkv, head_dim, o, lse, cu_seqlens, max_seqlen, scale, causal, window)
+    else:
+        dqkv = flash_attn_bwd_qkv_rope(dout, qkv, nq, nkv, head_dim, o, lse, cu_seqlens, max_seqlen, scale, causal, cos,
+                                       sin, pos, window)
+    return dqkv, dqkv.t().contiguous()
+
+
 def swiglu_bwd_t(dh, gu):
     if not (gu.dim() == 2 and gu.stride(1) == 1 and gu.stride(0) % 8 == 0 and gu.shape[1] % 16 == 0):
         raise RuntimeError("dtg: swiglu_bwd_t: the pre-activation must be [T, 2 * I] with unit inner stride, "
@@ -734,6 +763,6 @@
         "flash_attn_varlen_bwd", "flash_attn_fwd_drop", "flash_attn_bwd_drop", "flash_attn_bwd_qkv_drop", "philox_rng",
         "flash_attn_bwd_qkv_rope", "flash_attn_tuning", "layernorm_fwd", "dropout_add_layernorm_fwd", "layernorm_bwd",
         "gelu_fwd", "gelu_bwd", "gelu_bwd_t", "qk_norm_rope_fwd_", "qk_norm_rope_bwd_", "kv_cache_append_", "decode_attn",
-        "sample_logits", "skinny_linear",
+        "sample_logits", "skinny_linear", "flash_attn_fwd_t", "flash_attn_bwd_qkv_t",
     ):
         LIB.impl(_name, _fn, "CPU")
diff --git a/lambda-labs_distributed-training-guide_amd/ops/_schema.py b/lambda-labs_distributed-training-guide_amd/ops/_schema.py
--- a/lambda-labs_distributed-training-guide_amd/ops/_schema.py
+++ b/lambda-labs_distributed-training-guide_amd/ops/_schema.py
@@ -48,6 +48,11 @@
     "flash_attn_bwd_qkv_rope(Tensor dout, Tensor qkv, int nq, int nkv, int head_dim, Tensor o, Tensor lse, "
     "Tensor cu_seqlens, int max_seqlen, float scale, bool causal, Tensor cos, Tensor sin, Tensor pos, "
     "int window=0) -> Tensor",
+    "flash_attn_fwd_t(Tensor q, Tensor k, Tensor v, Tensor cu_seqlens, int max_seqlen, float scale, bool causal, "
+    "int window=0) -> (Tensor, Tensor, Tensor)",
+    "flash_attn_bwd_qkv_t(Tensor dout, Tensor qkv, int nq, int nkv, int head_dim, Tensor o, Tensor lse, "
+    "Tensor cu_seqlens, int max_seqlen, float scale, bool causal, Tensor? cos, Tensor? sin, Tensor? pos, "
+    "int window=0) -> (Tensor, Tensor)",
     "flash_attn_fwd_drop(Tensor q, Tensor k, Tensor v, Tensor cu_seqlens, int max_seqlen, float scale, bool causal, "
     "float p, Tensor rng) -> (Tensor, Tensor)",
     "flash_attn_bwd_drop(Tensor dout, Tensor q, Tensor k, Tensor v, Tensor o, Tensor lse, Tensor cu_seqlens, "
diff --git a/lambda-labs_distributed-training-guide_amd/ops/functional.py b/lambda-labs_distributed-training-guide_amd/ops/functional.py
--- a/lambda-labs_distributed-training-guide_amd/ops/functional.py
+++ b/lambda-labs_distributed-training-guide_amd/ops/functional.py
@@ -403,6 +403,74 @@
         pos = torch.empty(0, dtype=torch.long, device=qkv.device)
     return _AttentionQKV.apply(qkv, cos, sin, pos, cu_seqlens, int(max_seqlen), nq, nkv, head_dim, float(scale), causal, rope,
                                int(window or 0))
+
+
+_FA_EMIT_T = os.environ.get("DTG_FA_EMIT_T", "1")
+_FA_EMIT_O_T = _FA_EMIT_T in ("1", "fwd")
+_FA_EMIT_DQKV_T = _FA_EMIT_T in ("1", "bwd")
+
+
+class _AttentionBlock(torch.autograd.Function):
+
+    @staticmethod
+    def forward(ctx, x, w_qkv, w_o, cos, sin, pos, cu_seqlens, max_seqlen, nq, nkv, head_dim, scale, causal, emit):
+        T, d = x.shape[0], head_dim
+        qkv = torch.mm(x, w_qkv.t())
+        ops.rope_(qkv, cos, sin, pos, nq + nkv, d, False)
+        q, k, v = _qkv_head_views(qkv, nq, nkv, d)
+        o_t = None
+        if emit[0]:
+            o, lse, o_t = ops.flash_attn_fwd_t(q, k, v, cu_seqlens, max_seqlen, scale, causal, 0)
+        else:
+            o, lse = ops.flash_attn_fwd(q, k, v, cu_seqlens, max_seqlen, scale, causal, 0)
+        ctx.save_for_backward(x, w_qkv, w_o, qkv, o, lse, cu_seqlens, cos, sin, pos, *(() if o_t is None else (o_t,)))
+        ctx.meta = (max_seqlen, nq, nkv, d, scale, causal, emit[1])
+        return torch.mm(o.view(T, nq * d), w_o.t())
+
+    @staticmethod
+    def backward(ctx, dy):
+        x, w_qkv, w_o, qkv, o, lse, cu, cos, sin, pos, *o_t = ctx.saved_tensors
+        max_seqlen, nq, nkv, d, scale, causal, emit_dqkv_t = ctx.meta
+        T = x.shape[0]
+        o2 = o.view(T, nq * d)
+        dx_tn, dw_tn = _bwd_layout(o2, w_o)
+        do = _dx_mm(dy, w_o, dx_tn)
+        dw_o = _dw_mm(w_o, dy, o2, dw_tn, x_t=o_t[0] if o_t else None) if ctx.needs_input_grad[2] else None
+        del o_t
+        dx_tn, dw_tn = _bwd_layout(x, w_qkv)
+        dqkv_t = None
+        if emit_dqkv_t and _FA_ROPE_FUSED and ctx.needs_input_grad[1]:
+            dqkv, dqkv_t = ops.flash_attn_bwd_qkv_t(do.view(T, nq, d), qkv, nq, nkv, d, o, lse, cu, max_seqlen, scale,
+                                                    causal, cos, sin, pos, 0)
+        elif _FA_ROPE_FUSED:
+            dqkv = ops.flash_attn_bwd_qkv_rope(do.view(T, nq, d), qkv, nq, nkv, d, o, lse, cu, max_seqlen, scale, causal,
+                                               cos, sin, pos, 0)
+        else:
+            dqkv = ops.flash_attn_bwd_qkv(do.view(T, nq, d), qkv, nq, nkv, d, o, lse, cu, max_seqlen, scale, causal, 0)
+            ops.rope_(dqkv, cos, sin, pos, nq + nkv, d, True)
+        del do
+        dx = _dx_mm(dqkv, w_qkv, dx_tn) if ctx.needs_input_grad[0] else None
+        dw_qkv = _dw_mm(w_qkv, dqkv, x, dw_tn, dy_t=dqkv_t) if ctx.needs_input_grad[1] else None
+        del dqkv_t
+        return (dx, dw_qkv, dw_o) + (None,) * 11
+
+
+def attention_block_ok(x, w_qkv, w_o, head_dim):
+    if not (_FA_EMIT_O_T or _FA_EMIT_DQKV_T) or not torch.is_grad_enabled() or head_dim not in FA_HEAD_DIMS:
+        return False
+    if x.dim() != 2 or w_o.shape[1] % 8 or w_o.dtype != x.dtype:
+        return False
+    return _bwd_layout(x, w_qkv) == (True, True) and _bwd_layout(x, w_o) == (True, True)
+
+
+def attention_block(x, w_qkv, w_o, nq, nkv, head_dim, cu_seqlens, max_seqlen, cos, sin, pos, causal=True, scale=None,
+                    emit=None):
+    if scale is None:
+        scale = 1.0 / math.sqrt(head_dim)
+    if emit is None:
+        emit = (_FA_EMIT_O_T, _FA_EMIT_DQKV_T)
+    return _AttentionBlock.apply(x, w_qkv, w_o, cos, sin, pos, cu_seqlens, int(max_seqlen), int(nq), int(nkv),
+                                 int(head_dim), float(scale), bool(causal), (bool(emit[0]), bool(emit[1])))
 
 
 _DECODE_FUSED = os.environ.get("DTG_DECODE_FUSED", "1") == "1"
```
